# olsonanl/signature_kmers

Hardware: AMD Instinct MI355X
Metric: k-mers/sec (extract+hash+count) at 1/2/4/8 GPUs; achieved HBM GB/s % (higher is better)
Workload: dtype u8

## Files before the change

signature_kmers_amd/__init__.py:

```python
from __future__ import annotations

import ctypes as C
import os
from dataclasses import dataclass

import numpy as np

__all__ = [
    "SkmError", "lib", "K", "UNDEFINED_FUNCTION", "STORED_DTYPE", "CALL_DTYPE",
    "SignatureBuilder", "KeptKmers", "CmphKmerDb", "FunctionCaller", "mph_build",
    "kmer_to_str", "str_to_kmer", "keys_from_strings", "device_count", "MatrixDistance", "SeqIdMap",
    "matrix_tile_rows", "KeptKmerDb", "DeviceKeptKmerDb", "kept_db_plan", "kept_slot",
]

K = 8
UNDEFINED_FUNCTION = 0xFFFF
_HERE = os.path.dirname(os.path.abspath(__file__))
LIB_PATH = os.environ.get("SKM_LIB_PATH") or os.path.join(_HERE, "libskm.so")

STORED_DTYPE = np.dtype([("avg_from_end", "<u2"), ("function_index", "<u2"), ("mean", "<u2"),
                         ("median", "<u2"), ("var", "<u2")])
CALL_DTYPE = np.dtype([("start", "<u4"), ("end", "<u4"), ("count", "<i4"), ("function_index", "<u2"),
                       ("pad", "<u2"), ("protein_length_median", "<u4"),
                       ("protein_length_med_avg_dev", "<f4")])
# ... 159 lines not shown

def debug_chain_bench(n: int, njobs: int, mode: int = 0) -> float:
    ms = C.c_float()
    _check(lib().skm_debug_chain_bench(n, njobs, mode, C.byref(ms)))
    return ms.value


def debug_chain_eval(samples, mode: int):
    x = np.ascontiguousarray(samples, dtype=np.uint32)
    med, var = C.c_double(), C.c_double()
    _check(lib().skm_debug_chain_eval(_ptr(x), len(x), mode, C.byref(med), C.byref(var)))
    return med.value, var.value


def debug_div_check(nm: int, per: int) -> int:
    v = C.c_uint64(0)
    _check(lib().skm_debug_div_check(nm, per, C.byref(v)))
    return v.value


def device_count() -> int:
    n = C.c_int(0)
    _check(lib().skm_device_count(C.byref(n)))
    return n.value


def device_mem_info(device: int = 0) -> tuple:
    fr, tot = C.c_uint64(), C.c_uint64()
    _check(lib().skm_device_mem_info(device, C.byref(fr), C.byref(tot)))
    return fr.value, tot.value


def warm_device(device: int = 0) -> None:
    SignatureBuilder(1, device=device).close()


def kmer_to_str(key: int) -> str:
    return int(key).to_bytes(8, "little").decode("latin-1")


def str_to_kmer(s: str) -> int:
    b = s.encode("latin-1")
    assert len(b) == K
    return int.from_bytes(b, "little")


def keys_from_strings(strs) -> np.ndarray:
    return np.array([str_to_kmer(s) for s in strs], dtype=np.uint64)


@dataclass
class KeptKmers:
    keys: np.ndarray
    data: np.ndarray
    distinct_functions: np.ndarray
    seqs_with_func: np.ndarray
    n_seqs_with_signature: int
    distinct_signatures: int
    n_windows: int

    def stats_lines(self) -> str:
        return (f"Kept {len(self.keys)} kmers\ndistinct_signatures={self.distinct_signatures}\n"
                f"num_seqs_with_a_signature={self.n_seqs_with_signature}\n")

    def final_kmers_lines(self):
        for k, d in zip(self.keys, self.data):
            yield f"{kmer_to_str(k)}\t{int(d['avg_from_end'])}\t{int(d['function_index'])}\t\n"


class _KeptOwner:

    def __init__(self, k):
        self.k = k

    def __del__(self):
        try:
            lib().skm_kept_free(C.byref(self.k))
        except Exception:
            pass


class SignatureBuilder:

    def __init__(self, n_functions: int, max_seqs_per_file: int = 100000, device: int = 0, rank: int = 0,
                 world_size: int = 1):
        self._h = C.c_void_p()
        opts = _BuildOpts(8, max_seqs_per_file, n_functions, 1, rank, world_size)
        self.rank, self.world_size = rank, world_size
        dev = (C.c_int * 1)(device)
        _check(lib().skm_build_create(C.byref(self._h), dev, 1, C.byref(opts)))
        self.n_functions = n_functions
        self.device = device

    def add_batch(self, residues, seq_off, seq_len, seq_func, seq_id=None):
        residues = np.ascontiguousarray(residues, dtype=np.uint8)
        seq_off = np.ascontiguousarray(seq_off, dtype=np.uint64)
        seq_len = np.ascontiguousarray(seq_len, dtype=np.uint32)
        seq_func = np.ascontiguousarray(seq_func, dtype=np.uint16)
        n = len(seq_len)
        assert len(seq_off) == n and len(seq_func) == n
        if n:
            end = seq_off.astype(np.int64) + seq_len.astype(np.int64)
            if end.max() > len(residues):
                raise SkmError("seq_off/seq_len exceed the residue buffer")
        sid = None if seq_id is None else np.ascontiguousarray(seq_id, dtype=np.uint32)
        _check(lib().skm_build_add_batch(self._h, _ptr(residues), _ptr(seq_off), _ptr(seq_len), _ptr(seq_func),
                                         _ptr(sid) if sid is not None else None, n))

    def reserve(self, n_residues: int, n_seqs: int):
        _check(lib().skm_build_reserve(self._h, int(n_residues), int(n_seqs)))

    def set_transport(self, transport: "GlooTransport"):
        self._transport = transport
        _check(lib().skm_build_set_transport(self._h, transport.ptr))

    def set_comm(self, unique_id: bytes):
        buf = (C.c_uint8 * 128).from_buffer_copy(bytes(unique_id))
        _check(lib().skm_build_set_comm(self._h, buf))

    def prepare(self):
        _check(lib().skm_build_prepare(self._h))

    def run(self):
        _check(lib().skm_build_run(self._h))

    def timings(self) -> dict:
        ms = (C.c_float * 15)()
        n = lib().skm_build_last_timings(self._h, ms, 15)
        names = ["extract_count", "scan", "extract_scatter", "bucket_process", "overflow", "chains", "stats", "total",
                 "exchange", "partition", "bucket_kernel", "big_groups", "chain_tail", "giant_start", "giant_end"]
        return {names[i]: float(ms[i]) for i in range(n)}

    def set_kernel_timing(self, enable: bool, only: str | None = None):
        _check(lib().skm_build_set_kernel_timing(self._h, 1 if enable else 0, only.encode() if only else None))

    def kernel_timings(self) -> dict:
        n = lib().skm_build_kernel_timings(self._h, None, 0, None, None, 0)
        if n <= 0:
            return {}
        ms = (C.c_float * n)()
        cnt = (C.c_uint64 * n)()
        buf = C.create_string_buffer(64 * n + 64)
        lib().skm_build_kernel_timings(self._h, buf, len(buf), ms, cnt, n)
        names = buf.value.decode().split("\n")[:n]
        return {names[i]: (float(ms[i]), int(cnt[i])) for i in range(n)}

    def set_option(self, name: str, value: int):
        _check(lib().skm_build_set_option(self._h, name.encode(), int(value)))

    def passes(self) -> int:
        return self.counters()["passes"]

    def counters(self) -> dict:
        v = (C.c_uint64 * 48)()
        n = lib().skm_build_counters(self._h, v, 48)
        names = ["windows", "kept", "overflow_subbuckets", "chain_jobs", "chain_samples", "sequences", "grouped",
                 "overflow_elements", "overflow_kept", "big_groups", "big_kept", "passes", "valid", "giant_chains",
                 "giant_max", "redone", "cap_overflow_scratch", "cap_split", "cap_long_samples", "cap_long_jobs",
                 "demand_overflow_scratch", "demand_split", "demand_long_samples", "demand_long_jobs",
                 "long_samples", "routed", "add_batch_us", "prepare_upload_us", "prepare_plan_us", "prepare_rest_us",
                 "pass_groups", "add_pack_us", "add_dma_wait_us", "finish_us", "finish_wait_us", "finish_copy_us",
                 "finish_chunks", "finish_select_dev_us", "finish_sort_dev_us", "finish_gather_dev_us",
                 "finish_d2h_dev_us", "finish_max_chunk", "finish_wide_index", "kept_cap",
                 "free_after_prepare", "recs_rot", "overflow_light_subbuckets", "overflow_light_elements"]
        return {names[i]: int(v[i]) for i in range(n)}

    def debug_jobs(self, k: int = 64) -> list:
        v = (C.c_uint32 * k)()
        _check(lib().skm_build_debug_jobs(self._h, v, k))
        return [int(x) for x in v]

    def debug_overflow(self, k: int = 4096) -> list:
        v = (C.c_uint32 * k)()
        n = lib().skm_build_debug_overflow(self._h, v, k)
        return [int(x) for x in v[:min(max(n, 0), k)]]

    def debug_stamps(self, enable: bool) -> list:
        v = (C.c_uint64 * 32)()
        _check(lib().skm_build_debug_stamps(self._h, 1 if enable else 0, v, 32))
        return [int(x) for x in v]

    def finish(self) -> KeptKmers:
        k = _Kept()
        _check(lib().skm_build_finish(self._h, C.byref(k)))
        return self._kept(k)

    def finish_slice(self, slice_bits: int, slice_: int) -> KeptKmers:
        k = _Kept()
        _check(lib().skm_build_finish_slice(self._h, int(slice_bits), int(slice_), C.byref(k)))
        return self._kept(k)

    def signature_flags(self) -> np.ndarray:
        n = self.counters()["sequences"]
        out = np.zeros(max(n, 1), np.uint8)
        _check(lib().skm_build_signature_flags(self._h, _ptr(out), n))
        return out[:n]

    def kept_db(self, load_pct: int = 0, slots: int = 0, release_work: bool = False) -> "DeviceKeptKmerDb":
        opts = _KeptDbOpts(int(load_pct), 1 if release_work else 0, int(slots))
        h = C.c_void_p()
        _check(lib().skm_build_kept_db(self._h, C.byref(opts), C.byref(h)))
        return DeviceKeptKmerDb(h, self.device)

    @staticmethod
    def _kept(k) -> KeptKmers:
        owner = _KeptOwner(k)
        n = int(k.n)
        if n:
            kb = (C.c_char * (8 * n)).from_address(C.cast(k.keys, C.c_void_p).value)
            db = (C.c_char * (10 * n)).from_address(C.cast(k.data, C.c_void_p).value)
            kb._owner = db._owner = owner
            keys = np.frombuffer(kb, np.uint64)
            data = np.frombuffer(db, STORED_DTYPE)
        else:
            keys, data = np.zeros(0, np.uint64), np.zeros(0, STORED_DTYPE)
        nf = int(k.n_functions)
        df = np.ctypeslib.as_array(k.distinct_functions, shape=(max(nf, 1),))[:nf].copy()
        sw = np.ctypeslib.as_array(k.seqs_with_func, shape=(max(nf, 1),))[:nf].copy()
        return KeptKmers(keys, data, df, sw, int(k.n_seqs_with_signature), int(k.distinct_signatures),
                         int(k.n_windows))

    def close(self):
        if self._h:
            lib().skm_build_destroy(self._h)
            self._h = C.c_void_p()

    def __del__(self):
        try:
            self.close()
        except Exception:
            pass


class GlooTransport:

    def __init__(self):
        import torch.distributed as dist
        self.dist = dist
        self.rank, self.world = dist.get_rank(), dist.get_world_size()
        self._cbs = (_A2A_T(self._a2a), _RED_T(self._red), _AGV_T(self._agv))
        self.struct = _Transport(None, *self._cbs)
        self.ptr = C.pointer(self.struct)

    @staticmethod
    def _buf(addr, n):
        import torch
        if n == 0:
            return torch.zeros(0, dtype=torch.uint8)
        return torch.frombuffer((C.c_uint8 * n).from_address(addr), dtype=torch.uint8)

    def _a2a(self, ctx, send, scnt, soff, recv, rcnt, roff):
        try:
            W, me = self.world, self.rank
            sc = [int(scnt[i]) for i in range(W)]
            so = [int(soff[i]) for i in range(W)]
            rc = [int(rcnt[i]) for i in range(W)]
            ro = [int(roff[i]) for i in range(W)]
            if sc[me]:
                C.memmove(recv + ro[me], send + so[me], sc[me])
            reqs = []
            for q in range(W):
                if q == me:
                    continue
                if sc[q]:
                    reqs.append(self.dist.isend(self._buf(send + so[q], sc[q]).clone(), q))
                if rc[q]:
                    reqs.append(self.dist.irecv(self._buf(recv + ro[q], rc[q]), q))
            for r in reqs:
                r.wait()
            return 0
        except Exception:
            import traceback
            traceback.print_exc()
            return -1

    def _red(self, ctx, data, count, op):
        try:
            import torch
            n = int(count)
            if op == 0:
                a = np.ctypeslib.as_array(C.cast(data, C.POINTER(C.c_uint32)), shape=(n,))
                t = torch.from_numpy(a.astype(np.int64))
                self.dist.all_reduce(t, op=self.dist.ReduceOp.SUM)
                a[:] = (t.numpy() & 0xFFFFFFFF).astype(np.uint32)
            else:
                a = np.ctypeslib.as_array(C.cast(data, C.POINTER(C.c_uint8)), shape=(n,))
                t = torch.from_numpy(a.astype(np.int32))
                self.dist.all_reduce(t, op=self.dist.ReduceOp.MAX)
                a[:] = t.numpy().astype(np.uint8)
            return 0
        except Exception:
            import traceback
            traceback.print_exc()
            return -1

    def _agv(self, ctx, send, recv, bytes_per_rank):
        try:
            import torch
            W = self.world
            nb = [int(bytes_per_rank[i]) for i in range(W)]
            m = max(1, max(nb))
            mine = torch.zeros(m, dtype=torch.uint8)
            if nb[self.rank]:
                mine[:nb[self.rank]] = self._buf(send, nb[self.rank])
            outs = [torch.zeros(m, dtype=torch.uint8) for _ in range(W)]
            self.dist.all_gather(outs, mine)
            o = 0
            for r in range(W):
                if nb[r]:
                    self._buf(recv + o, nb[r])[:] = outs[r][:nb[r]]
                o += nb[r]
            return 0
        except Exception:
            import traceback
            traceback.print_exc()
            return -1

# ... 456 lines not shown
```

signature_kmers_amd/csrc/skm_build.hip:

```cpp
#include <hip/hip_runtime.h>

#include <algorithm>
#include <type_traits>
#include <chrono>
#include <cmath>
#include <cstdio>
#include <cstdlib>
#include <cstring>
#include <deque>
#include <memory>
#include <numeric>
#include <string>
#include <thread>
#include <vector>

#include "skm_common.h"
#include "skm_keptdb.h"
#include "skm_pool.h"
#include "skm_output.h"
#include "skm_util.h"

#if defined(SKM_WITH_RCCL)
#include <rccl/rccl.h>
#endif
// ... 460 lines not shown
            const int q = __ffsll((long long)m) - 1;
            m &= m - 1;
            const uint32_t pos = base + (uint32_t)q;
            const uint32_t len = pos - run_s;
            if (len > best_c) {
                best_c = len;
                best_f = run_f;
                rb = run_s;
            }
            run_s = pos;
            run_f = (uint32_t)__shfl((int)f, q, 64);
        }
    }
    {
        const uint32_t len = c - run_s;
        if (len > best_c) {
            best_c = len;
            best_f = run_f;
            rb = run_s;
        }
    }
    if ((float)best_c < float(c) * 0.8f) return r;
    r.kept = true;
    r.best_f = best_f;
    r.cbest = best_c;
    r.rb = rb;
    uint32_t vmin = 0xFFFFu, vmax = 0;
    for (uint32_t t = lane; t < c; t += 64) {
        const uint32_t o = (uint32_t)(v.lov(a + t) & 0xFFFFu);
        vmin = min(vmin, o);
        vmax = max(vmax, o);
    }
    vmin = wave_min(vmin);
    vmax = wave_max(vmax);
    const uint32_t k = c / 2;
    while (vmin < vmax) {
        const uint32_t mid = (vmin + vmax) >> 1;
        uint32_t cnt = 0;
        for (uint32_t t = lane; t < c; t += 64) cnt += (uint32_t)(v.lov(a + t) & 0xFFFFu) <= mid;
        cnt = wave_sum(cnt);
        if (cnt >= k + 1)
            vmax = mid;
        else
            vmin = mid + 1;
    }
    r.avg = vmin;
    uint32_t sum = 0;
    for (uint32_t t = lane; t < c; t += 64) {
        const uint32_t s = (uint32_t)(v.lov(a + t) >> 36);
        mark_seq(flags, s);
        if (t >= rb && t < rb + best_c) sum += glen[s];
    }
    sum = wave_sum(sum);
    r.mean = d2u16((double)(uint16_t)sum / (double)best_c);
    r.median = 0;
    r.var = 0;
    return r;
}

__device__ __forceinline__ uint32_t wg_sum(uint32_t x, uint32_t* s_wave) {
    const uint32_t lane = threadIdx.x & 63u, wave = threadIdx.x >> 6, nw = blockDim.x >> 6;
    x = wave_sum(x);
    if (lane == 0) s_wave[wave] = x;
    __syncthreads();
    uint32_t t = 0;
    for (uint32_t w = 0; w < nw; ++w) t += s_wave[w];
    __syncthreads();
    return t;
}

__device__ __forceinline__ uint32_t wg_max(uint32_t x, uint32_t* s_wave) {
    const uint32_t lane = threadIdx.x & 63u, wave = threadIdx.x >> 6, nw = blockDim.x >> 6;
    x = wave_max(x);
    if (lane == 0) s_wave[wave] = x;
    __syncthreads();
    uint32_t t = 0;
    for (uint32_t w = 0; w < nw; ++w) t = max(t, s_wave[w]);
    __syncthreads();
    return t;
}

__device__ __forceinline__ uint32_t wg_min(uint32_t x, uint32_t* s_wave) {
    const uint32_t lane = threadIdx.x & 63u, wave = threadIdx.x >> 6, nw = blockDim.x >> 6;
    x = wave_min(x);
    if (lane == 0) s_wave[wave] = x;
    __syncthreads();
    uint32_t t = 0xFFFFFFFFu;
    for (uint32_t w = 0; w < nw; ++w) t = min(t, s_wave[w]);
    __syncthreads();
    return t;
}

template <class V>
__device__ bool group_block(const V& v, uint64_t a, uint32_t c, const uint32_t* __restrict__ glen,
                            uint32_t* __restrict__ flags, uint32_t* heads, uint32_t hcap, uint32_t* s_wave, GRes& r) {
    const uint32_t tid = threadIdx.x, nt = blockDim.x;
    r.kept = false;
    uint32_t H = 0;
    for (uint32_t t0 = 0; t0 < c; t0 += nt) {
        const uint32_t t = t0 + tid;
        const bool head = t < c && (t == 0 || v.func(a + t) != v.func(a + t - 1));
        uint32_t tot;
        const uint32_t pos = wg_exclusive_scan(head ? 1u : 0u, s_wave, tot);
        if (head && H + pos < hcap) heads[H + pos] = t;
        H += tot;
    }
    if (H > hcap) return false;
    __syncthreads();
    uint32_t lmax = 0;
    for (uint32_t j = tid; j < H; j += nt) lmax = max(lmax, (j + 1 < H ? heads[j + 1] : c) - heads[j]);
    const uint32_t best_c = wg_max(lmax, s_wave);
    uint32_t fmin = 0xFFFFFFFFu;
    for (uint32_t j = tid; j < H; j += nt)
        if ((j + 1 < H ? heads[j + 1] : c) - heads[j] == best_c) fmin = min(fmin, (v.func(a + heads[j]) << 16) | j);
    const uint32_t fj = wg_min(fmin, s_wave);
    if ((float)best_c < float(c) * 0.8f) return true;
    const uint32_t rb = heads[fj & 0xFFFFu];
    r.kept = true;
    r.best_f = fj >> 16;
    r.cbest = best_c;
    r.rb = rb;
    uint32_t k = c / 2, pre = 0;
    for (int b = 15; b >= 0; --b) {
        uint32_t n0 = 0;
        for (uint32_t t = tid; t < c; t += nt) {
            const uint32_t o = (uint32_t)(v.lov(a + t) & 0xFFFFu);
            n0 += (o >> b) == (pre >> b);
        }
        n0 = wg_sum(n0, s_wave);
        if (k >= n0) {
            k -= n0;
            pre |= 1u << b;
        }
    }
    r.avg = pre;
    uint32_t sum = 0;
    for (uint32_t t = tid; t < c; t += nt) {
        const uint32_t s = (uint32_t)(v.lov(a + t) >> 36);
        mark_seq(flags, s);
        if (t >= rb && t < rb + best_c) sum += glen[s];
    }
    sum = wg_sum(sum, s_wave);
    r.mean = d2u16((double)(uint16_t)sum / (double)best_c);
    r.median = 0;
    r.var = 0;
    return true;
}

enum : uint32_t {
    RUN_FLAGS = 0,
    RUN_LONG_CUR = 1,
    RUN_LONG_N = 2,
    RUN_LONG_FLUSHED = 3,
    RUN_SNAP = 28,
    RUN_DEM_TOT = 8,
    RUN_DEM_SPLIT = 9,
    RUN_DEM_LONG = 10,
    RUN_DEM_LJOBS = 11,
    RUN_LONG_WANT = 12,
    RUN_LONG_WANTJ = 13,
    RUN_ACC_LIGHT_SUB = 14,
    RUN_ACC_LIGHT_ELEMS = 15,
    RUN_ACC_NOVF = 16,
    RUN_ACC_JOBS = 17,
    RUN_ACC_LENS = 18,
    RUN_ACC_OVF_ELEMS = 19,
    RUN_ACC_OVF_KEPT = 20,
    RUN_ACC_BIG = 21,
    RUN_ACC_BIG_KEPT = 22,
    RUN_ACC_GROUPED = 23,
    RUN_LAST_NOVF = 24,
    RUN_LAST_JOBS = 25,
    RUN_NLOC = 26,
    RUN_SLOTS = 64
};
constexpr unsigned long long RUN_F_ARENA = 1;
constexpr unsigned long long RUN_F_RERUN = 2;
constexpr unsigned long long RUN_F_CAP = 4;
enum : uint32_t {
    PLAN_NOVF = 0,
    PLAN_NSPLIT = 1,
    PLAN_NHEAVY = 2,
    PLAN_SKIP = 3,
    PLAN_Q_SPLIT = 4,
    PLAN_Q_HEAVY = 5,
    PLAN_Q_REST = 6,
    PLAN_Q_LIGHT = 7,
    PLAN_SLOTS = 8
};

constexpr int JOB_CLASSES = 32;
constexpr int JOB_WG = 256;

__device__ __forceinline__ uint32_t job_class(uint32_t n) { return 31u - (uint32_t)__clz(n | 1u); }

__device__ __forceinline__ void job_chunk(const unsigned long long* nj_p, uint64_t cap, uint64_t& a, uint64_t& e) {
    const uint64_t nj = min((uint64_t)*nj_p, cap);
    const uint64_t chunk = (nj + gridDim.x - 1) / gridDim.x;
    a = min(nj, (uint64_t)blockIdx.x * chunk);
    e = min(nj, a + chunk);
}

__global__ __launch_bounds__(JOB_WG) void k_job_count(const Job* __restrict__ jobs, const unsigned long long* nj_p,
                                                      uint64_t cap, uint32_t* __restrict__ hist) {
    __shared__ uint32_t h[JOB_CLASSES];
    if (threadIdx.x < JOB_CLASSES) h[threadIdx.x] = 0;
    __syncthreads();
    uint64_t a, e;
    job_chunk(nj_p, cap, a, e);
    for (uint64_t j = a + threadIdx.x; j < e; j += blockDim.x) atomicAdd(&h[job_class(jobs[j].n)], 1u);
    __syncthreads();
    if (threadIdx.x < JOB_CLASSES) hist[blockIdx.x * JOB_CLASSES + threadIdx.x] = h[threadIdx.x];
}

constexpr uint32_t LONG_CLASS = 14;

__global__ void k_job_scan(const uint32_t* __restrict__ hist, uint32_t nwg, uint64_t* __restrict__ offs,
                           uint32_t long_class) {
    __shared__ uint64_t tot[JOB_CLASSES];
    const uint32_t c = threadIdx.x;
    if (c < JOB_CLASSES) {
        uint64_t t = 0;
        for (uint32_t w = 0; w < nwg; ++w) t += hist[w * JOB_CLASSES + c];
        tot[c] = t;
    }
    __syncthreads();
    if (c == 0) {
        uint64_t nl = 0;
        for (uint32_t cc = long_class; cc < JOB_CLASSES; ++cc) nl += tot[cc];
        offs[(uint64_t)nwg * JOB_CLASSES] = nl;
    }
    if (c < JOB_CLASSES) {
        uint64_t base = 0;
        for (uint32_t cc = JOB_CLASSES - 1; cc > c; --cc) base += tot[cc];
        for (uint32_t w = 0; w < nwg; ++w) {
            offs[w * JOB_CLASSES + c] = base;
            base += hist[w * JOB_CLASSES + c];
        }
    }
}

__global__ __launch_bounds__(JOB_WG) void k_job_scatter(const Job* __restrict__ jobs, const unsigned long long* nj_p,
                                                        uint64_t cap, const uint64_t* __restrict__ offs,
                                                        Job* __restrict__ sorted) {
    __shared__ unsigned long long cur[JOB_CLASSES];
    if (threadIdx.x < JOB_CLASSES) cur[threadIdx.x] = offs[blockIdx.x * JOB_CLASSES + threadIdx.x];
    __syncthreads();
    uint64_t a, e;
    job_chunk(nj_p, cap, a, e);
    for (uint64_t j = a + threadIdx.x; j < e; j += blockDim.x) {
        const Job jb = jobs[j];
        sorted[atomicAdd(&cur[job_class(jb.n)], 1ull)] = jb;
    }
}

__global__ __launch_bounds__(1024) void k_long_plan(const Job* __restrict__ jobs, const uint64_t* __restrict__ nlong_p,
                                                    uint64_t* __restrict__ off, unsigned long long* __restrict__ run,
                                                    uint64_t arena_cap, uint64_t jobs_cap) {
    __shared__ uint32_t s_wave[17];
    __shared__ unsigned long long s_run;
    const uint64_t nlong = *nlong_p;
    if (threadIdx.x == 0) s_run = 0;
    __syncthreads();
    for (uint64_t b = 0; b < nlong; b += blockDim.x) {
        const uint64_t j = b + threadIdx.x;
        const uint32_t n = j < nlong ? jobs[j].n : 0u;
        uint32_t tot;
        const uint32_t ex = wg_exclusive_scan(n, s_wave, tot);
        const unsigned long long run_ = s_run;
        if (j < nlong) off[j] = run_ + ex;
        __syncthreads();
        if (threadIdx.x == 0) s_run = run_ + tot;
        __syncthreads();
    }
    if (threadIdx.x == 0) {
        const uint64_t total = s_run;
        off[nlong] = total;
        off[nlong + 1] = nlong;
        if (run) {
            uint64_t base = 0, jbase = 0;
            bool ok = true;
            if (nlong) {
                const unsigned long long want = atomicAdd(&run[RUN_LONG_WANT], (unsigned long long)total) + total;
                const unsigned long long wantj = atomicAdd(&run[RUN_LONG_WANTJ], (unsigned long long)nlong) + nlong;
                auto reserve = [&](unsigned long long* c, uint64_t n, uint64_t cap, uint64_t& at) {
                    unsigned long long cur = *(volatile unsigned long long*)c;
                    while (true) {
                        if (cur + n > cap) return false;
                        const unsigned long long seen = atomicCAS(c, cur, cur + n);
                        if (seen == cur) {
                            at = cur;
                            return true;
                        }
                        cur = seen;
                    }
                };
                ok = reserve(&run[RUN_LONG_CUR], total, arena_cap, base);
                ok = ok && reserve(&run[RUN_LONG_N], nlong, jobs_cap, jbase);
                if (!ok) {
                    atomicMax(&run[RUN_DEM_LONG], want);
                    atomicMax(&run[RUN_DEM_LJOBS], wantj);
                    atomicOr(&run[RUN_FLAGS], (unsigned long long)RUN_F_RERUN);
                }
            }
            off[nlong + 2] = base;
            off[nlong + 3] = jbase;
// ... 1766 lines not shown
    SKM_STAMP(6);
    {
        const uint32_t ntask = tstart[6];
        const uint32_t nbig = cstart[7] - cstart[6];
        const uint64_t bbase = *reinterpret_cast<const unsigned long long*>(L.wave + 44);
        const uint32_t wave = tid >> 6, nwaves = nt >> 6, lane = tid & 63u;
        uint64_t* slots = reinterpret_cast<uint64_t*>(L.lens32);
        uint64_t* slots_lo = const_cast<uint64_t*>(src_lo);
        (void)wave;
        (void)nwaves;
        for (;;) {
            uint32_t t = 0;
            if (lane == 0) t = atomicAdd(&ccnt[7], 1u);
            t = (uint32_t)__builtin_amdgcn_readfirstlane((int)t);
            if (t >= nbig + ntask) break;
            if (t < nbig) {
                const uint32_t g = L.big[cstart[6] + t];
                const uint32_t rep = L.glist[g];
                const uint32_t a = L.goff[rep];
                const uint32_t c = g + 1 < G ? L.goff[L.glist[g + 1]] - a : M - a;
                for (uint32_t u = lane; u < c; u += 64) {
                    const uint32_t j = L.order[a + u];
                    const uint64_t hj = L.hi[j], lj = L.lo[j];
                    slots[a + u] = ((hj & 0xFFFFull) << 48) | (lj >> 16);
                    slots_lo[a + u] = elem_len(hj, lj, A.glen);
                }
                const uint64_t q = bbase + t;
                if (lane == 0 && q < A.big_cap) {
                    A.big_desc[2 * q] = key_h43(hprefix, (L.hi[rep] >> 16) & REM_MASK, A.rem_bits, A.pshift) |
                                        ((uint64_t)c << KEY_BITS);
                    A.big_desc[2 * q + 1] = L.lens_sel + 2 * a;
                }
                continue;
            }
            const uint32_t ts = ntask - 1u - (t - nbig);
            uint32_t k = 0;
            while (k < 5 && ts >= tstart[k + 1]) ++k;
            const uint32_t per = 64u >> (k + 1);
            const uint32_t q0 = cstart[k] + (ts - tstart[k]) * per, qe = cstart[k + 1];
            switch (k) {
                case 0: seg_groups<2>(L, q0, qe, G, M, A, hprefix, jobinfo, fmean); break;
                case 1: seg_groups<4>(L, q0, qe, G, M, A, hprefix, jobinfo, fmean); break;
                case 2: seg_groups<8>(L, q0, qe, G, M, A, hprefix, jobinfo, fmean); break;
                case 3: seg_groups<16>(L, q0, qe, G, M, A, hprefix, jobinfo, fmean); break;
                case 4: seg_groups<32>(L, q0, qe, G, M, A, hprefix, jobinfo, fmean); break;
                default: seg_groups<64>(L, q0, qe, G, M, A, hprefix, jobinfo, fmean); break;
            }
        }
    }
    __syncthreads();
    SKM_STAMP(11);
    SKM_STAMP(7);
    constexpr uint32_t EMIT_PER = CAP / BPK_THREADS;
    unsigned long long* s_base = reinterpret_cast<unsigned long long*>(L.wave + 36);
    const uint32_t j0 = tid * EMIT_PER;
    uint32_t cnt = 0;
#pragma unroll
    for (uint32_t u = 0; u < EMIT_PER; ++u) {
        const uint32_t j = j0 + u;
        const uint32_t jb = j < n ? jobinfo[j] : 0u;
        cnt += ((jb & JOB_KEPT) ? 1u : 0u) | ((jb & JOB_COUNT_MASK) ? 0x10000u : 0u);
    }
    uint32_t tot;
    const uint32_t pos = wg_exclusive_scan1(cnt, L.wave, tot);
    unsigned long long rsv = 0;
    if (tid == 0 && (tot & 0xFFFFu)) rsv = atomicAdd(A.kept_ctr, (unsigned long long)(tot & 0xFFFFu));
    if (tid == 64 && (tot >> 16)) rsv = atomicAdd(&A.ctr[3], (unsigned long long)(tot >> 16));
    {
        uint32_t pk = pos & 0xFFFFu, pj = pos >> 16;
#pragma unroll
        for (uint32_t u = 0; u < EMIT_PER; ++u) {
            const uint32_t jb = j0 + u < n ? jobinfo[j0 + u] : 0u;
            if (!(jb & JOB_KEPT)) continue;
            L.slot[pk] = (uint16_t)(j0 + u);
            if (jb & JOB_COUNT_MASK) {
                L.order[pj++] = (uint16_t)(j0 + u);
                L.rank[j0 + u] = (uint16_t)pk;
            }
            ++pk;
        }
    }
    if (tid == 0 || tid == 64) s_base[tid >> 6] = rsv;
    __syncthreads();
    const uint32_t nkept = tot & 0xFFFFu, njob = tot >> 16;
    if (nkept) {
        const uint64_t ob = s_base[0];
#pragma unroll 1
        for (uint32_t t = tid; t < nkept; t += nt) {
            const uint32_t j = L.slot[t];
            const uint32_t jb = jobinfo[j];
            uint64_t lo;
            if (jb & JOB_COUNT_MASK) {
                const uint32_t fm = fmean[j];
                lo = kept_lo(fm & 0xFFFFu, fm >> 16, 0, 0);
            } else {
                lo = L.lo[j];
            }
            write_kept(A, ob + t, L.hi[j], lo);
        }
        const uint64_t jbase = njob ? s_base[1] : 0;
#pragma unroll 1
        for (uint32_t t = tid; t < njob; t += nt) {
            const uint32_t j = L.order[t];
            const uint32_t jb = jobinfo[j];
            Job jbr;
            jbr.lens_off = L.lens_sel + 2 * (jb >> 16);
            jbr.n = jb & JOB_COUNT_MASK;
            jbr.out_idx = (uint32_t)(ob + L.rank[j]);
            A.jobs[jbase + t] = jbr;
        }
    }
    __syncthreads();
    SKM_STAMP(8);
    return nkept;
}

struct SubMem {
    uint64_t hi[CAP];
    uint64_t lo[CAP];
    uint32_t tab[TAB];
    __align__(16) uint16_t slot[CAP];
    __align__(16) uint16_t rank[CAP];
    __align__(16) uint16_t goff[CAP];
    __align__(16) uint16_t glist[CAP];
    __align__(16) uint16_t order[CAP];
    __align__(16) uint16_t big[CAP / 2];
    __align__(16) uint32_t wave[48];
    uint32_t nbig;
    uint64_t tlast;
    uint32_t ccnt[24];
};

__device__ __forceinline__ SubLds sub_lds(SubMem& m) {
    SubLds L;
    L.ccnt = m.ccnt;
    L.tlast = &m.tlast;
    if (threadIdx.x == 0) m.tlast = __builtin_amdgcn_s_memtime();
    L.hi = m.hi;
    L.lo = m.lo;
    L.tab = m.tab;
    L.slot = m.slot;
    L.rank = m.rank;
    L.goff = m.goff;
    L.glist = m.glist;
    L.order = m.order;
    L.big = m.big;
    L.wave = m.wave;
    L.nbig = &m.nbig;
    L.lens32 = nullptr;
    L.lens_sel = 0;
    return L;
}

__global__ __launch_bounds__(BPK_THREADS, BPK_WAVES_EU) void k_bucket_process(BucketArgs A) {
    static_assert(CAP % BPK_THREADS == 0, "emit assigns CAP / BPK_THREADS elements per thread");
    __shared__ SubMem s_mem;
    __shared__ uint32_t s_sub[(1 << MAX_B2) + 1];
    if (A.skip && *A.skip) return;
    SubLds L = sub_lds(s_mem);

    const uint32_t bucket = blockIdx.x;
    if (bucket >= A.nbuckets) return;
    const uint64_t r0 = A.bstart[bucket], r1 = A.bstart[bucket + 1];
    const uint64_t n = r1 - r0;
    if (n == 0) return;
    const uint64_t hprefix = (uint64_t)(A.bucket_base + bucket) << A.rem_bits;
    if (A.prio == 1) __builtin_amdgcn_s_setprio(1);
    if (A.prio == 2) __builtin_amdgcn_s_setprio(2);
    if (A.prio >= 3) __builtin_amdgcn_s_setprio(3);

    const bool direct = n <= (uint64_t)CAP && A.nsrc == 1;
    uint32_t nsub = 1;
    if (!direct) {
        const uint32_t* tab = A.sub_tab + (uint64_t)bucket * SUB_TAB;
        nsub = tab[0];
        for (uint32_t d = threadIdx.x; d <= nsub; d += blockDim.x) s_sub[d] = tab[1 + d];
        __syncthreads();
        SKM_STAMP(9);
    }
    struct Batch {
        uint32_t a, cnt;
    };
    auto next_batch = [&](uint32_t& d) -> Batch {
        if (direct) {
            if (d >= 1) return Batch{0, 0};
            d = 1;
            return Batch{0, (uint32_t)n};
        }
        while (d < nsub) {
            const uint32_t a = s_sub[d];
            if (s_sub[d + 1] - a == 0 || s_sub[d + 1] - a > (uint32_t)CAP) {
                ++d;
                continue;
            }
            uint32_t d2 = d + 1;
            while (d2 < nsub && s_sub[d2 + 1] - a <= (uint32_t)CAP) ++d2;
            d = d2;
            return Batch{a, s_sub[d2] - a};
        }
        return Batch{0, 0};
    };
    const uint64_t* base_hi = direct ? A.recs_hi + r0 : A.tmp_hi + r0;
    const uint64_t* base_lo = direct ? A.recs_lo + r0 : A.tmp_lo + r0;
    const uint64_t sel = direct ? LENS_IN_RECS : LENS_IN_TMP;
    uint32_t d = 0;
    for (Batch cur = next_batch(d); cur.cnt; cur = next_batch(d)) {
        L.lens_sel = (sel << LENS_SEL_SHIFT) | (2 * (r0 + cur.a));
        L.lens32 = reinterpret_cast<uint32_t*>(const_cast<uint64_t*>(base_hi + cur.a));
        process_sub(base_hi + cur.a, base_lo + cur.a, cur.cnt, A, hprefix, L);
        __syncthreads();
        SKM_STAMP(10);
    }
}

struct BigOut {
    uint64_t h43;
    uint64_t lens_off;
    uint32_t n;
    uint16_t avg, func, mean, pad0;
    uint32_t pad1;
};
static_assert(sizeof(BigOut) == 32, "BigOut layout");

struct BigArgs {
    const uint64_t* desc;
    const unsigned long long* ndesc;
    uint32_t cap;
    const uint64_t* recs_hi;
    const uint64_t* tmp_hi;
    const uint64_t* recs_lo;
    const uint64_t* tmp_lo;
    uint32_t* flags;
    BigOut* out;
};

template <int E>
__device__ __forceinline__ uint32_t ballot_count(const bool (&p)[E]) {
    uint32_t n = 0;
#pragma unroll
    for (int e = 0; e < E; ++e) n += (uint32_t)__popcll(__ballot(p[e]));
    return n;
}

template <int E, int D>
__device__ __forceinline__ void bitonic_cross(uint64_t (&ky)[E], bool take_min) {
#pragma unroll
    for (int e = 0; e < E; ++e) {
        const uint64_t o = xshfl64<D>(ky[e]);
        ky[e] = take_min ? (o < ky[e] ? o : ky[e]) : (o > ky[e] ? o : ky[e]);
    }
}

template <int E>
__device__ __forceinline__ void big_group(const BigArgs& B, uint64_t g, uint64_t* mem, const uint64_t* mlen,
                                          uint32_t c, uint64_t h43, uint64_t lens_off) {
    const uint32_t lane = threadIdx.x & 63u;
    uint32_t fo[E];
    uint64_t ky[E];
#pragma unroll
    for (int e = 0; e < E; ++e) {
        const uint32_t t = lane * E + (uint32_t)e;
        fo[e] = 0xFFFFFFFFu;
        ky[e] = ~0ull;
        if (t < c) {
            const uint64_t v = mem[t];
            const uint32_t len = (uint32_t)mlen[t];
            const uint32_t i = (uint32_t)v & ((1u << ELEM_I_BITS) - 1u);
            fo[e] = ((uint32_t)(v >> 48) << 16) | ((len - i) & 0xFFFFu);
            ky[e] = (v << 16) | t;
        }
    }
    uint32_t cand = 0xFFFFFFFFu, cc = 0;
#pragma unroll
    for (int e = 0; e < E; ++e) {
        if (fo[e] != 0xFFFFFFFFu) {
            const uint32_t f = fo[e] >> 16;
            if (cc == 0) {
                cand = f;
                cc = 1;
            } else if (f == cand) {
                ++cc;
            } else {
                --cc;
            }
        }
    }
    bm_combine(cand, cc);
    bool p[E];
#pragma unroll
    for (int e = 0; e < E; ++e) p[e] = (fo[e] >> 16) == cand;
    const uint32_t nb = ballot_count<E>(p);
    BigOut o;
    o.h43 = h43;
    o.lens_off = lens_off;
    o.n = 0;
    o.avg = o.func = o.mean = 0;
    o.pad0 = 0;
    o.pad1 = 0;
    if ((float)nb < float(c) * 0.8f) {
        if (lane == 0) B.out[g] = o;
        return;
    }
    constexpr int MC = E < 8 ? E : 8;
#pragma unroll
    for (int e0 = 0; e0 < E; e0 += MC) {
        uint32_t ms[MC];
#pragma unroll
        for (int u = 0; u < MC; ++u)
            ms[u] = fo[e0 + u] != 0xFFFFFFFFu ? (uint32_t)(ky[e0 + u] >> (16 + ELEM_I_BITS)) : 0xFFFFFFFFu;
        if constexpr (E > 16) {
            Seq8 q;
#pragma unroll
            for (int u = 0; u < 8; ++u) q.s[u] = ms[u];
            mark_seqs8(B.flags, q);
        } else {
            mark_seqs<MC>(B.flags, ms);
        }
    }
    uint32_t sum = 0;
#pragma unroll
    for (int e = 0; e < E; ++e) {
        if (fo[e] != 0xFFFFFFFFu && p[e]) sum += (uint32_t)mlen[ky[e] & 0xFFFFu];
        if (!p[e]) ky[e] = ~0ull;
    }
    sum = wave_sum(sum);
    uint32_t k = c / 2, pre = 0;
#pragma unroll 1
    for (int b = 15; b >= 0; --b) {
#pragma unroll
        for (int e = 0; e < E; ++e) {
            const uint32_t v = fo[e] == 0xFFFFFFFFu ? 0x10000u : (fo[e] & 0xFFFFu);
            p[e] = ((v >> b) ^ (pre >> b)) == 0u;
        }
        const uint32_t n0 = ballot_count<E>(p);
        if (k >= n0) {
            k -= n0;
            pre |= 1u << b;
        }
    }
#pragma unroll 1
    for (uint32_t kk = 2; kk <= 64u * E; kk <<= 1) {
        const bool asc_lane = ((lane * (uint32_t)E) & kk) == 0;
#pragma unroll 1
        for (uint32_t jj = kk >> 1; jj >= (uint32_t)E; jj >>= 1) {
            const uint32_t d = jj / (uint32_t)E;
            const bool take_min = ((lane & d) == 0) == asc_lane;
            switch (d) {
                case 1: bitonic_cross<E, 1>(ky, take_min); break;
                case 2: bitonic_cross<E, 2>(ky, take_min); break;
                case 4: bitonic_cross<E, 4>(ky, take_min); break;
                case 8: bitonic_cross<E, 8>(ky, take_min); break;
                case 16: bitonic_cross<E, 16>(ky, take_min); break;
                default: bitonic_cross<E, 32>(ky, take_min); break;
            }
        }
#pragma unroll
        for (int jj = E / 2; jj > 0; jj >>= 1) {
            if ((uint32_t)jj < kk) {
#pragma unroll
                for (int e = 0; e < E; ++e) {
                    const int l = e ^ jj;
                    if (l > e) {
                        const bool asc = (((lane * (uint32_t)E) + (uint32_t)e) & kk) == 0;
                        const uint64_t x = ky[e], y = ky[l];
                        const bool sw = asc ? (y < x) : (x < y);
                        ky[e] = sw ? y : x;
                        ky[l] = sw ? x : y;
                    }
                }
            }
        }
    }
    uint32_t* lens = reinterpret_cast<uint32_t*>(mem);
#pragma unroll
    for (int e = 0; e < E; ++e) {
        const uint32_t t = lane * E + (uint32_t)e;
        if (t < nb) lens[nb - 1 - t] = (uint32_t)mlen[ky[e] & 0xFFFFu];
    }
    o.n = nb;
    o.avg = (uint16_t)pre;
    o.func = (uint16_t)cand;
    o.mean = d2u16((double)(uint16_t)sum / (double)nb);
    if (lane == 0) B.out[g] = o;
}

constexpr int BIG_WG = 256;

template <bool LARGE>
__global__ __launch_bounds__(BIG_WG, LARGE ? 3 : 4) void k_big_groups(BigArgs B) {
    const uint64_t nd = min((uint64_t)*B.ndesc, (uint64_t)B.cap);
    const uint64_t nw = (uint64_t)gridDim.x * (BIG_WG / 64);
    for (uint64_t g = (uint64_t)blockIdx.x * (BIG_WG / 64) + (threadIdx.x >> 6); g < nd; g += nw) {
        const uint64_t d0 = B.desc[2 * g], d1 = B.desc[2 * g + 1];
        const uint32_t c = (uint32_t)(d0 >> KEY_BITS);
        if (LARGE != (c > 1024u)) continue;
        const uint64_t h43 = d0 & KEY_MASK;
        const uint64_t sel = d1 >> LENS_SEL_SHIFT, off = d1 & LENS_OFF_MASK;
        uint64_t* mem = const_cast<uint64_t*>(sel == LENS_IN_RECS ? B.recs_hi : B.tmp_hi) + off / 2;
        const uint64_t* mlen = (sel == LENS_IN_RECS ? B.recs_lo : B.tmp_lo) + off / 2;
        if constexpr (LARGE) {
            big_group<32>(B, g, mem, mlen, c, h43, d1);
        } else {
            if (c <= 128u) big_group<2>(B, g, mem, mlen, c, h43, d1);
            else if (c <= 256u) big_group<4>(B, g, mem, mlen, c, h43, d1);
            else if (c <= 512u) big_group<8>(B, g, mem, mlen, c, h43, d1);
            else big_group<16>(B, g, mem, mlen, c, h43, d1);
        }
    }
}

__global__ __launch_bounds__(BIG_WG) void k_big_append(const BigOut* __restrict__ out, BigArgs B, BucketArgs A) {
    __shared__ __align__(16) uint32_t s_wave[48];
    __shared__ unsigned long long s_base[2];
    const uint64_t nd = min((uint64_t)*B.ndesc, (uint64_t)B.cap);
    const uint64_t per = (nd + gridDim.x - 1) / gridDim.x;
    const uint64_t g0 = (uint64_t)blockIdx.x * per, g1 = min(nd, g0 + per);
    for (uint64_t r = g0; r < g1; r += BIG_WG) {
        const uint64_t g = r + threadIdx.x;
        const bool kept = g < g1 && out[g].n != 0;
        uint32_t tot;
        const uint32_t pos = wg_exclusive_scan(kept ? 1u : 0u, s_wave, tot);
        if (tot == 0) continue;
        if (threadIdx.x == 0) {
            s_base[0] = atomicAdd(A.kept_ctr, (unsigned long long)tot);
            s_base[1] = atomicAdd(&A.ctr[3], (unsigned long long)tot);
            atomicAdd(&A.ctr[6], (unsigned long long)tot);
        }
        __syncthreads();
        if (kept) {
            const BigOut o = out[g];
            const uint64_t w = s_base[0] + pos;
            write_kept(A, w, kept_hi(o.h43, o.avg), kept_lo(o.func, o.mean, 0, 0));
            Job jb;
            jb.lens_off = o.lens_off;
            jb.n = o.n;
            jb.out_idx = (uint32_t)w;
            A.jobs[s_base[1] + pos] = jb;
        }
        __syncthreads();
    }
}

__global__ __launch_bounds__(1024) void k_part_order(const uint64_t* __restrict__ bstart, uint32_t nb,
                                                     uint32_t* __restrict__ order) {
    __shared__ uint32_t s_wave[48];
    const uint64_t total = bstart[nb] - bstart[0];
    const uint64_t thr = 2 * (total / max(nb, 1u));
    const uint32_t per = (nb + blockDim.x - 1) / blockDim.x;
    const uint32_t b0 = min(nb, threadIdx.x * per), b1 = min(nb, b0 + per);
    uint32_t loc = 0;
    for (uint32_t b = b0; b < b1; ++b) loc += bstart[b + 1] - bstart[b] > thr ? 1u : 0u;
    uint32_t nbig;
    uint32_t pos = wg_exclusive_scan(loc, s_wave, nbig);
    uint32_t sp = b0 - pos;
    for (uint32_t b = b0; b < b1; ++b) {
        if (bstart[b + 1] - bstart[b] > thr)
            order[pos++] = b;
        else
            order[nbig + sp++] = b;
    }
    if (threadIdx.x == 0) order[nb] = nbig;
}

constexpr uint32_t PT_ROUND = 2048, PT_THREADS = BP_THREADS;

__global__ __launch_bounds__(PT_THREADS, 3) void k_partition(BucketArgs A) {
    __shared__ uint32_t s_cur[(1 << MAX_B2) + 1];
    __shared__ uint32_t s_rc[1 << MAX_B2];
    __shared__ uint16_t s_ro[(1 << MAX_B2) + 1];
    __shared__ uint64_t s_sh[PT_ROUND];
    __shared__ uint64_t s_sl[PT_ROUND];
    __shared__ __align__(16) uint32_t s_wave[48];
    if (blockIdx.x >= A.nbuckets) return;
    const uint32_t bucket = A.order ? A.order[blockIdx.x] : blockIdx.x;
    const uint64_t r0 = A.bstart[bucket], r1 = A.bstart[bucket + 1];
    const uint64_t n = r1 - r0;
    uint32_t* tab = A.sub_tab + (uint64_t)bucket * SUB_TAB;
    if (n == 0 || (n <= (uint64_t)CAP && A.nsrc == 1)) {
        if (threadIdx.x == 0) tab[0] = 0;
        return;
    }
    const uint64_t rem_mask = (1ull << A.rem_bits) - 1;
    int b2 = 0;
    const uint64_t target = A.sub_target ? A.sub_target : (uint32_t)SUB_TARGET;
    while (b2 < MAX_B2 && (n >> b2) > target) ++b2;
    const uint32_t nsub = 1u << b2;
    const int shift = A.rem_bits - b2;
    for (uint32_t d = threadIdx.x; d <= nsub; d += blockDim.x) s_cur[d] = 0;
    __syncthreads();
    const uint32_t nseg = A.nsrc;
    auto seg = [&](uint32_t p, uint64_t& base, uint64_t& len) {
        if (nseg == 1) {
            base = r0;
            len = n;
        } else {
            base = A.seg_start[(uint64_t)p * A.nbuckets + bucket];
            len = A.seg_len[(uint64_t)p * A.nbuckets + bucket];
        }
    };
    for (uint32_t p = 0; p < nseg; ++p) {
        uint64_t base, len;
        seg(p, base, len);
        for (uint64_t j0 = 0; j0 < len; j0 += blockDim.x) {
            const uint64_t j = j0 + threadIdx.x;
            const bool v = j < len;
            const uint64_t h = v ? A.recs_hi[base + j] : 0ull;
            agg_count(s_cur, (uint32_t)(((h >> 16) & rem_mask) >> shift), v);
        }
    }
    __syncthreads();
    {
        const uint32_t per = (nsub + blockDim.x - 1) / blockDim.x;
        const uint32_t d0 = threadIdx.x * per;
        uint32_t local = 0;
        for (uint32_t d = d0; d < min(nsub, d0 + per); ++d) local += s_cur[d];
        uint32_t tot;
        uint32_t run = wg_exclusive_scan(local, s_wave, tot);
        for (uint32_t d = d0; d < min(nsub, d0 + per); ++d) {
            const uint32_t t = s_cur[d];
            s_cur[d] = run;
            run += t;
        }
        __syncthreads();
        if (threadIdx.x == 0) s_cur[nsub] = tot;
        __syncthreads();
    }
    if (threadIdx.x == 0) tab[0] = nsub;
    for (uint32_t d = threadIdx.x; d <= nsub; d += blockDim.x) tab[1 + d] = s_cur[d];
    __syncthreads();
    constexpr uint32_t PER = PT_ROUND / PT_THREADS;
    for (uint32_t p = 0; p < nseg; ++p) {
        uint64_t base, len;
        seg(p, base, len);
        uint64_t nh[PER], nl[PER];
#pragma unroll
        for (uint32_t u = 0; u < PER; ++u) {
            const uint64_t j = threadIdx.x + (uint64_t)u * PT_THREADS;
            if (j < len) {
                nh[u] = A.recs_hi[base + j];
                nl[u] = A.recs_lo[base + j];
            }
        }
        for (uint64_t rb = 0; rb < len; rb += PT_ROUND) {
            for (uint32_t d = threadIdx.x; d < nsub; d += blockDim.x) s_rc[d] = 0;
            uint64_t eh[PER], el[PER];
            uint32_t sb[PER], rk[PER];
#pragma unroll
            for (uint32_t u = 0; u < PER; ++u) {
                sb[u] = 0xFFFFFFFFu;
                eh[u] = nh[u];
                el[u] = nl[u];
                const uint64_t j = rb + PT_ROUND + threadIdx.x + (uint64_t)u * PT_THREADS;
                if (j < len) {
                    nh[u] = A.recs_hi[base + j];
                    nl[u] = A.recs_lo[base + j];
                }
            }
            __syncthreads();
#pragma unroll
            for (uint32_t u = 0; u < PER; ++u) {
                const uint64_t j = rb + threadIdx.x + (uint64_t)u * PT_THREADS;
                const bool v = j < len;
                if (v) sb[u] = (uint32_t)(((eh[u] >> 16) & rem_mask) >> shift);
                rk[u] = agg_rank(s_rc, v ? sb[u] : 0u, v);
            }
            __syncthreads();
            {
                const uint32_t per = (nsub + blockDim.x - 1) / blockDim.x;
                const uint32_t d0 = threadIdx.x * per;
                uint32_t local = 0;
                for (uint32_t d = d0; d < min(nsub, d0 + per); ++d) local += s_rc[d];
                uint32_t tot;
                uint32_t run = wg_exclusive_scan(local, s_wave, tot);
                for (uint32_t d = d0; d < min(nsub, d0 + per); ++d) {
                    s_ro[d] = (uint16_t)run;
                    run += s_rc[d];
                }
                if (threadIdx.x == 0) s_ro[nsub] = (uint16_t)tot;
                __syncthreads();
            }
#pragma unroll
            for (uint32_t u = 0; u < PER; ++u)
                if (sb[u] != 0xFFFFFFFFu) {
                    const uint32_t slot = s_ro[sb[u]] + rk[u];
                    s_sh[slot] = eh[u];
                    s_sl[slot] = el[u];
                }
            __syncthreads();
            const uint32_t tot = s_ro[nsub];
            for (uint32_t k = threadIdx.x; k < tot; k += blockDim.x) {
                const uint64_t h = s_sh[k];
                const uint32_t d = (uint32_t)(((h >> 16) & rem_mask) >> shift);
                const uint64_t o = r0 + s_cur[d] + (k - s_ro[d]);
                A.tmp_hi[o] = h;
                A.tmp_lo[o] = s_sl[k];
            }
            __syncthreads();
            for (uint32_t d = threadIdx.x; d < nsub; d += blockDim.x) s_cur[d] += s_rc[d];
            __syncthreads();
        }
    }
    for (uint32_t d = threadIdx.x; d < nsub; d += blockDim.x) {
        const uint32_t beg = d ? s_cur[d - 1] : 0u;
        const uint32_t cnt = s_cur[d] - beg;
        if (cnt > (uint32_t)CAP) {
            const unsigned int en = atomicAdd(reinterpret_cast<unsigned int*>(&A.ctr[1]), 1u);
            if (en < A.ovf_cap) {
                OvfEntry o;
                o.off = r0 + beg;
                o.n = cnt;
                o.bucket = bucket;
                o.scratch = 0;
                o.npad = 0;
                o.src = 1;
                A.ovf[en] = o;
            }
        }
    }
}

struct OvfScratch {
    uint64_t* hi;
    uint64_t* lo;
    uint32_t* heads;
    uint64_t* jobinfo;
    uint32_t* fmean;
};

constexpr uint32_t OVF_INLINE_CAP = 32;
constexpr uint32_t OVF_BLOCK_GROUP = 1024;

__global__ __launch_bounds__(BP_THREADS) void k_overflow(BucketArgs A, OvfScratch S, uint32_t* plan, int lo_slot,
// ... 974 lines not shown
                        mark_seq(A.flags, sv[u]);
                    }
                }
            }
        }
        if (tid == 0) {
            const uint64_t h43 = key_h43((uint64_t)(A.bucket_base + K.bucket) << A.rem_bits, K.rem, A.rem_bits, A.pshift);
            write_kept(A, o, kept_hi(h43, pre), kept_lo(best_f, mean, 0, 0));
            Job jbr;
            jbr.n = cb;
            jbr.out_idx = o;
            if (giant) {
                jbr.lens_off = reinterpret_cast<uint64_t>(H.gsamples + loff);
                H.gjobs[jb] = jbr;
            } else {
                jbr.lens_off = loff;
                A.jobs[jb] = jbr;
            }
        }
        __syncthreads();
    }
}

struct PlanArgs {
    const OvfEntry* in;
    OvfEntry* out;
    const unsigned long long* ctr;
    const unsigned long long* kept;
    const unsigned long long* nloc;
    unsigned long long* run;
    uint32_t* plan;
    uint32_t ovf_cap, split_min, heavy_min;
    uint64_t kept_cap, tot_cap, split_cap;
};

constexpr uint32_t PLAN_BINS = 3 * 32;

__device__ __forceinline__ uint32_t plan_bin(uint32_t n, uint32_t split_min, uint32_t heavy_min) {
    const uint32_t tier = (n >= split_min ? 1u : 0u) + (n >= heavy_min ? 1u : 0u);
    return PLAN_BINS - 1u - (tier * 32u + (31u - (uint32_t)__clz(n | 1u)));
}

__global__ __launch_bounds__(1024) void k_ovf_plan(PlanArgs P) {
    __shared__ uint32_t s_cnt[PLAN_BINS];
    __shared__ unsigned long long s_part[1024];
    __shared__ unsigned long long s_tot, s_elems, s_split;
    __shared__ uint32_t s_nsplit, s_nheavy;
    const uint32_t tid = threadIdx.x, nt = blockDim.x;
    const uint64_t raw = P.ctr[1] & 0xFFFFFFFFull;
    const uint32_t n = (uint32_t)min<uint64_t>(raw, P.ovf_cap);
    for (uint32_t i = tid; i < PLAN_BINS; i += nt) s_cnt[i] = 0;
    if (tid == 0) {
        s_tot = s_elems = s_split = 0;
        s_nsplit = s_nheavy = 0;
    }
    __syncthreads();
    for (uint32_t i = tid; i < n; i += nt) atomicAdd(&s_cnt[plan_bin(P.in[i].n, P.split_min, P.heavy_min)], 1u);
    __syncthreads();
    if (tid == 0) {
        uint32_t r = 0;
        for (uint32_t b = 0; b < PLAN_BINS; ++b) {
            const uint32_t c = s_cnt[b];
            s_cnt[b] = r;
            r += c;
        }
    }
    __syncthreads();
    unsigned long long lt = 0, le = 0, ls = 0;
    uint32_t lns = 0, lnh = 0;
    for (uint32_t i = tid; i < n; i += nt) {
        OvfEntry e = P.in[i];
        const uint32_t pos = atomicAdd(&s_cnt[plan_bin(e.n, P.split_min, P.heavy_min)], 1u);
        uint64_t np = 1;
        while (np < e.n) np <<= 1;
        e.npad = (uint32_t)np;
        P.out[pos] = e;
        lt += np;
        le += e.n;
        if (e.n >= P.split_min) {
            ls += e.n;
            ++lns;
        }
        if (e.n >= P.heavy_min) ++lnh;
    }
    atomicAdd(&s_tot, lt);
    atomicAdd(&s_elems, le);
    atomicAdd(&s_split, ls);
    atomicAdd(&s_nsplit, lns);
    atomicAdd(&s_nheavy, lnh);
    __threadfence_block();
    __syncthreads();
    const uint32_t per = (n + nt - 1) / nt;
    const uint32_t a = min(n, tid * per), e_ = min(n, a + per);
    unsigned long long sum = 0;
    for (uint32_t i = a; i < e_; ++i) sum += P.out[i].npad;
    s_part[tid] = sum;
    __syncthreads();
    if (tid == 0) {
        unsigned long long r = 0;
        for (uint32_t t = 0; t < nt; ++t) {
            const unsigned long long v = s_part[t];
            s_part[t] = r;
            r += v;
        }
    }
    __syncthreads();
    unsigned long long o = s_part[tid];
    for (uint32_t i = a; i < e_; ++i) {
        P.out[i].scratch = o;
        o += P.out[i].npad;
    }
    if (tid == 0) {
        unsigned long long* R = P.run;
        const uint64_t tot = s_tot, split = s_split, nl = *P.nloc;
        atomicMax(&R[RUN_DEM_TOT], (unsigned long long)tot);
        atomicMax(&R[RUN_DEM_SPLIT], (unsigned long long)split);
        if (raw > P.ovf_cap) atomicOr(&R[RUN_FLAGS], RUN_F_CAP);
        const bool over = tot > P.tot_cap || split > P.split_cap;
        if (over) atomicOr(&R[RUN_FLAGS], RUN_F_RERUN);
        if (P.kept[0] + nl > P.kept_cap) atomicOr(&R[RUN_FLAGS], RUN_F_ARENA);
        const bool skip = over || (atomicAdd(&R[RUN_FLAGS], 0ull) & (RUN_F_ARENA | RUN_F_CAP)) != 0;
        P.plan[PLAN_NOVF] = skip ? 0u : n;
        P.plan[PLAN_NSPLIT] = skip ? 0u : s_nsplit;
        P.plan[PLAN_NHEAVY] = skip ? 0u : s_nheavy;
        P.plan[PLAN_SKIP] = skip ? 1u : 0u;
        P.plan[PLAN_Q_SPLIT] = 0;
        P.plan[PLAN_Q_HEAVY] = 0;
        P.plan[PLAN_Q_REST] = 0;
        P.plan[PLAN_Q_LIGHT] = 0;
        R[RUN_ACC_NOVF] += n;
        R[RUN_ACC_OVF_ELEMS] += s_elems;
        R[RUN_ACC_GROUPED] += nl;
        R[RUN_LAST_NOVF] = n;
    }
}

__global__ void k_poison_jobs(Job* __restrict__ jobs, uint64_t n, uint64_t samples, uint32_t idx,
                             skm_stored_kmer_data* __restrict__ out) {
    const uint64_t t = (uint64_t)blockIdx.x * blockDim.x + threadIdx.x;
    for (uint64_t j = t; j < n; j += (uint64_t)gridDim.x * blockDim.x) jobs[j] = Job{samples, 8u, idx};
    if (t == 0) out[idx] = skm_stored_kmer_data{0xC0DE, 0xC0DE, 0xC0DE, 0xC0DE, 0xC0DE};
}

__global__ void k_pass_account(const unsigned long long* __restrict__ ctr, unsigned long long* __restrict__ run,
                               uint64_t jobs_cap, uint64_t jobs2_cap, uint64_t big_cap, uint64_t lens_cap) {
    const unsigned long long j = ctr[3] + ctr[8 + 3];
    run[RUN_ACC_JOBS] += j;
    run[RUN_ACC_LENS] += ctr[8 + 4];
    run[RUN_ACC_OVF_KEPT] += ctr[8];
    run[RUN_ACC_BIG] += ctr[5];
    run[RUN_ACC_BIG_KEPT] += ctr[6];
    run[RUN_ACC_LIGHT_SUB] += ctr[21];
    run[RUN_ACC_LIGHT_ELEMS] += ctr[22];
    run[RUN_LAST_JOBS] = j;
    if (ctr[3] > jobs_cap || ctr[8 + 3] > jobs2_cap || ctr[5] > big_cap || ctr[8 + 4] > lens_cap)
        atomicOr(&run[RUN_FLAGS], RUN_F_CAP);
}

__global__ void k_kept_finalize(uint64_t* __restrict__ keys, const skm_stored_kmer_data* __restrict__ data,
                                const unsigned long long* __restrict__ n_p, uint32_t nf, uint32_t* __restrict__ dfunc) {
    extern __shared__ uint32_t s_h[];
    const uint64_t n = *n_p;
    const bool lds = nf <= 16384;
    if (lds)
        for (uint32_t f = threadIdx.x; f < nf; f += blockDim.x) s_h[f] = 0;
    __syncthreads();
    for (uint64_t i = (uint64_t)blockIdx.x * blockDim.x + threadIdx.x; i < n; i += (uint64_t)gridDim.x * blockDim.x) {
        keys[i] = decode_key(unmix43(keys[i]));
        uint32_t f = data[i].function_index;
        if (f < nf) {
            if (lds)
                atomicAdd(&s_h[f], 1u);
            else
                atomicAdd(&dfunc[f], 1u);
        }
    }
    __syncthreads();
    if (lds)
        for (uint32_t f = threadIdx.x; f < nf; f += blockDim.x)
            if (s_h[f]) atomicAdd(&dfunc[f], s_h[f]);
}

__global__ void k_func_hist_seqs(const SeqMeta* __restrict__ meta, uint32_t nseq, uint32_t nf, uint32_t* __restrict__ swf) {
    extern __shared__ uint32_t s_h[];
    const bool lds = nf <= 16384;
    if (lds)
        for (uint32_t f = threadIdx.x; f < nf; f += blockDim.x) s_h[f] = 0;
    __syncthreads();
    for (uint32_t s = blockIdx.x * blockDim.x + threadIdx.x; s < nseq; s += gridDim.x * blockDim.x) {
        uint32_t f = meta[s].func;
        if (f < nf) {
            if (lds)
                atomicAdd(&s_h[f], 1u);
            else
                atomicAdd(&swf[f], 1u);
        }
    }
    __syncthreads();
    if (lds)
        for (uint32_t f = threadIdx.x; f < nf; f += blockDim.x)
            if (s_h[f]) atomicAdd(&swf[f], s_h[f]);
}

__global__ void k_flags_from_bits(const uint32_t* __restrict__ bits, uint32_t nseq, uint8_t* __restrict__ flags) {
    for (uint32_t w = blockIdx.x * blockDim.x + threadIdx.x; w < (nseq + 31) / 32; w += gridDim.x * blockDim.x) {
        const uint32_t v = bits[w];
        const uint32_t n = min(32u, nseq - 32 * w);
        uint8_t* o = flags + 32 * (uint64_t)w;
        for (uint32_t t = 0; t < n; ++t) o[t] = (uint8_t)((v >> t) & 1u);
    }
}

__global__ void k_count_flags(const uint8_t* __restrict__ flags, uint32_t nseq, unsigned long long* __restrict__ out) {
    uint32_t local = 0;
    for (uint32_t s = blockIdx.x * blockDim.x + threadIdx.x; s < nseq; s += gridDim.x * blockDim.x) local += flags[s] ? 1u : 0u;
#pragma unroll
    for (int d = 32; d > 0; d >>= 1) local += __shfl_down(local, d, 64);
    if ((threadIdx.x & 63) == 0 && local) atomicAdd(out, (unsigned long long)local);
}

__global__ void k_send_counts(const uint64_t* __restrict__ bstart, uint32_t NB, uint32_t NB1, uint32_t W,
                              const unsigned long long* __restrict__ expect, unsigned long long* __restrict__ run,
                              uint32_t* __restrict__ out) {
    const uint32_t t = blockIdx.x * blockDim.x + threadIdx.x;
    if (t < NB) out[t] = (uint32_t)(bstart[t + 1] - bstart[t]);
    if (t < W && bstart[(uint64_t)(t + 1) * NB1] - bstart[(uint64_t)t * NB1] != expect[t])
        atomicOr(&run[RUN_FLAGS], (unsigned long long)RUN_F_CAP);
}

__global__ __launch_bounds__(1024) void k_recv_plan(const uint32_t* __restrict__ cnt, uint32_t W, uint32_t NB1,
                                                    const unsigned long long* __restrict__ expect,
                                                    unsigned long long* __restrict__ run,
                                                    uint64_t* __restrict__ seg_start, uint32_t* __restrict__ seg_len,
                                                    uint64_t* __restrict__ vstart) {
    __shared__ uint32_t s_wave[17];
    __shared__ unsigned long long s_tot[64];
    const uint32_t tid = threadIdx.x, nt = blockDim.x;
    const uint32_t N = W * NB1;
    {
        const uint32_t per = (N + nt - 1) / nt, a = min(N, tid * per), e = min(N, a + per);
        uint32_t loc = 0;
        for (uint32_t i = a; i < e; ++i) loc += cnt[i];
        uint32_t tot;
        uint64_t run_ = wg_exclusive_scan(loc, s_wave, tot);
        for (uint32_t i = a; i < e; ++i) {
            seg_start[i] = run_;
            seg_len[i] = cnt[i];
            run_ += cnt[i];
        }
    }
    if (tid < 64) s_tot[tid] = 0;
    __syncthreads();
    for (uint32_t i = tid; i < N; i += nt) atomicAdd(&s_tot[i / NB1], (unsigned long long)cnt[i]);
    __syncthreads();
    if (tid < W && s_tot[tid] != expect[tid]) atomicOr(&run[RUN_FLAGS], (unsigned long long)RUN_F_CAP);
    {
        const uint32_t per = (NB1 + nt - 1) / nt, a = min(NB1, tid * per), e = min(NB1, a + per);
        uint32_t loc = 0;
        for (uint32_t k = a; k < e; ++k)
            for (uint32_t p = 0; p < W; ++p) loc += cnt[(uint64_t)p * NB1 + k];
        uint32_t tot;
        uint64_t run_ = wg_exclusive_scan(loc, s_wave, tot);
        for (uint32_t k = a; k < e; ++k) {
            vstart[k] = run_;
            for (uint32_t p = 0; p < W; ++p) run_ += cnt[(uint64_t)p * NB1 + k];
        }
        if (tid == 0) vstart[NB1] = tot;
    }
}

__global__ __launch_bounds__(256) void k_slice_select(const uint64_t* __restrict__ keys,
                                                      const skm_stored_kmer_data* __restrict__ data, uint64_t n,
                                                      int bits, uint64_t slice, unsigned long long* __restrict__ cursor,
                                                      uint64_t* __restrict__ out_keys,
                                                      skm_stored_kmer_data* __restrict__ out_data) {
    const uint32_t lane = threadIdx.x & 63u;
    const uint64_t stride = (uint64_t)gridDim.x * blockDim.x;
    for (uint64_t b0 = (uint64_t)blockIdx.x * blockDim.x; b0 < n; b0 += stride) {
        const uint64_t j = b0 + threadIdx.x;
        const uint64_t k = j < n ? keys[j] : 0ull;
        const bool in = j < n && (bits == 0 || (slice_hash(k) >> (64 - bits)) == slice);
        const uint64_t m = __ballot(in);
        if (!m) continue;
        unsigned long long base = 0;
        if (lane == 0) base = atomicAdd(cursor, (unsigned long long)__popcll(m));
        base = __shfl(base, 0, 64);
        if (in && out_keys) {
            const uint64_t o = base + (uint64_t)__popcll(m & ((1ull << lane) - 1ull));
            out_keys[o] = k;
            out_data[o] = data[j];
        }
    }
}

struct Tune {
    int passes = 0;
    int64_t mem_budget_mb = 0;
    int ovf_heavy = 8192;
    int ovf_inline_min = 0x7FFFFFFF;
    int inline_prio = 3;
    int ovf_long_class = 14;
    int main_long_class = 14;
    int ovf_chain_wgs = 0;
    int chain_prio = 0;
    int bucket_prio = 0;
    int chain_lds_kb = 0;
    int host_timing = 0;
    int heavy_min = (int)HEAVY_MIN;
    int split_min = (int)SPLIT_MIN;
    int ovf_light = 1;
    int giant_class = -1;
    int giant_passes = 0;
    int prefetch = 1;
    int heavy_grid = (int)HEAVY_GRID;
    int ovf_grid = 1024;
    int split_grid = 512;
    int chain_grid = 4096;
    int stream_prio = 0;
    int chain_batches = 2;
    int chain_streams = 1;
    int poison_jobs = 0;
    int route_vacate = 0;
    int tail_async = 1;
    int big_grid = 2048;
    int big_grid_large = 512;
    int big_split = 0;
    int part_order = 1;
    int emit_group = 0;
    int route_first = -1;
    int route_first_min = 1 << 17;
    int route_heavy_min = 1 << 14;
    int chain_cus = 0;
    int side_cus = 0;
    int serial_overflow = 0;
    int stage_round = 1;
    int lane_long = 1 << 20;
    int lane_grid = 256;
    int lane_streams = 1;
    int lane_tail = 1 << 16;
    int sub_target = 0;
    int heavy_lsd = 0;
    int handoff_index_limit = 0;
    int handoff_max_chunk = 0;
};

}

using namespace skm;

struct ChainSet {
    DevBuf hist, offs, sorted, long_off;
};

struct skm_build {
    skm_build_opts opts{};
    int device = 0;
    hipStream_t stream = nullptr;
    struct EvSet {
        hipEvent_t ev[13] = {}, o[3] = {}, o3[3] = {};
    };
    std::deque<EvSet> evsets;
    hipEvent_t* ev = nullptr;
    hipEvent_t* ev_o = nullptr;
    hipEvent_t* ev_o3 = nullptr;
    float last_ms[15] = {};
    uint64_t ovf_elems = 0, ovf_kept = 0, ovf_light_sub = 0, ovf_light_elems = 0;

    uint8_t* st_pin[2] = {};
    size_t st_fill[2] = {};
    hipEvent_t st_ev[2] = {};
    bool st_busy[2] = {};
    int st_cur = 0;
    uint64_t rp_total = 0;
    uint64_t rp_dev = 0;
    uint64_t res_cap = 0;
    std::vector<SeqMeta> h_meta;
    std::vector<uint32_t> h_seqid;
    std::unique_ptr<HostPool> pool;
    HandoffStats handoff;
    std::vector<uint32_t> h_keep;
    std::vector<uint64_t> h_cum;
    double add_s = 0, add_pack_s = 0, add_wait_s = 0, prep_upload_s = 0, prep_plan_s = 0, prep_rest_s = 0;
    uint64_t n_windows = 0;
    bool seqid_strict = true;
    bool prepared = false, ran = false;
    bool work_released = false;

    DevBuf d_res, d_meta, d_blk2seq, d_glen;
    uint64_t rp = 0;
    uint32_t nseq = 0;
    int world = 1, rank = 0;
    int owner_bits = 0, b1_bits = 12;
    uint32_t s_base = 0;
    uint32_t n_total = 0;
    std::vector<uint32_t> g_seqid;
    bool g_strict = true;
    DevBuf d_hist, d_offs, d_partial, d_rbbase, d_bstart32, d_bstart, d_owner_start;
    DevBuf d_recs_hi, d_recs_lo, d_tmp_hi, d_tmp_lo;
    DevBuf d_stg_hi, d_stg_lo;
    DevBuf d_part_order;
    DevBuf d_cur0, d_cur1, d_slices;
    DevBuf d_flagbits;
    DevBuf d_keys, d_data, d_ctr, d_flags, d_dfunc, d_swf, d_ovf, d_ovf_hi, d_ovf_lo, d_ovf_heads, d_ovf_job, d_ovf_fm;
    DevBuf d_jobs, d_lens, d_stamps, d_big_desc, d_big_out;
    uint64_t big_cap = 0, n_big = 0, big_kept = 0;
    bool stamps = false;
    uint64_t jobs_cap = 0, lens_cap = 0, n_jobs = 0, n_lens = 0;
    uint32_t n_overflow = 0, n_overflow_last = 0;
    uint32_t nwg = 0;
    uint64_t span = 0;
    uint64_t n_kept = 0;
    uint64_t ovf_cap = 0;

    DevBuf d_rhi, d_rlo;
    DevBuf d_cnt_send, d_cnt_recv;
    DevBuf d_seg_start, d_seg_len, d_vstart;
    std::vector<uint64_t> xs_send, xs_recv;
    DevBuf d_xs;
    uint64_t n_local_max = 0;
    uint64_t n_local = 0;
    uint64_t cap_local = 0;

#if defined(SKM_WITH_RCCL)
    ncclComm_t comm = nullptr;
#endif
    std::vector<skm_build*> group;
    skm_transport tp{};

    hipStream_t stream2 = nullptr, stream3 = nullptr;
    hipStream_t stream_tail = nullptr;
    hipStream_t stream_tail2 = nullptr;
    hipEvent_t ev_tail_bp = nullptr, ev_tail_done = nullptr, ev_tail2 = nullptr;
    bool tail_pending = false;
    uint64_t free_after_prepare = 0;
    hipEvent_t ev_part = nullptr, ev_split = nullptr, ev_light = nullptr;
    DevBuf d_hv_keys, d_hv_rec, d_hv_len, d_hv_s0, d_hv_s1;
    DevBuf d_sub_tab, d_jobs2, d_jobs3;

    unsigned long long* h_pin = nullptr;
    OvfEntry* h_ovf = nullptr;
    size_t h_ovf_cap = 0;
    unsigned long long* pinned_ctr() {
        if (!h_pin) SKM_HIP(hipHostMalloc(reinterpret_cast<void**>(&h_pin), 128 * 8, hipHostMallocDefault));
        return h_pin;
    }
    OvfEntry* pinned_ovf(size_t n) {
        if (n > h_ovf_cap) {
            if (h_ovf) SKM_HIP(hipHostFree(h_ovf));
            h_ovf = nullptr;
            h_ovf_cap = std::max<size_t>(n, 1024);
            SKM_HIP(hipHostMalloc(reinterpret_cast<void**>(&h_ovf), sizeof(OvfEntry) * h_ovf_cap, hipHostMallocDefault));
        }
        return h_ovf;
    }

    uint64_t jobs2_cap = 0;
    ChainSet cs_main, cs_ovf, cs_ovf3;
    uint32_t n_ovf_heavy = 0;

    int pass_bits = 0;
    uint64_t pass_max = 0;
    uint64_t valid_total = 0;
    DevBuf d_ids;
    DevBuf d_bloom;
    std::vector<uint64_t> cnt64;
    bool route = false;
    bool route_first = false;
    uint64_t routed = 0;
    DevBuf d_posg, d_histg, d_npos;
    uint32_t emit_g = 1;
    DevBuf d_selrows, d_seloff;
    uint64_t sel_span = 0;
    uint32_t sel_wg = SEL_WG;
    hipStream_t stx = nullptr;
    hipEvent_t ev_staged = nullptr, ev_emit = nullptr;
    int64_t emit_q = -1;
    uint32_t pf_nwg = 1;
    uint64_t pf_span = 0;
    uint64_t kept_cap = 0;
    hipEvent_t ev_start = nullptr;
    struct Acc {
        uint64_t novf, jobs, lens, ovf_elems, ovf_kept, big, big_kept, grouped;
    } acc{};
    float pass_ms[12] = {};
    skm::Tune tune;
    hipStream_t chain_st = nullptr;
    hipEvent_t chain_ev[3] = {};
    static constexpr int LANE_ST = 4;
    hipStream_t lane_st[LANE_ST] = {};
    hipEvent_t lane_ev[LANE_ST] = {};
    bool lane_used[LANE_ST] = {};
    static constexpr int GSLOTS = 3;
    hipStream_t gst[GSLOTS] = {};
    hipEvent_t gev_ready[GSLOTS] = {}, gev_done[GSLOTS] = {};
    std::deque<DevBuf> gsamples, gjobs, gcount;
    bool gused[GSLOTS] = {};
    bool chain_used[GSLOTS + 1] = {};
    DevBuf d_gstat;
    uint64_t giant_jobs = 0, giant_max = 0;
    DevBuf d_long_arena;
    DevBuf d_long_jobs;
    uint64_t long_jobs_cap = 0;
    DevBuf d_ovf2, d_plan, d_run;
    uint64_t tot_cap = 0, split_cap = 0, long_cap = 0;
    uint64_t run_flags = 0, demand[4] = {}, n_jobs_last = 0, n_redo = 0;
    uint64_t long_samples = 0;
    int kt_mode = 0;
    std::string kt_only;
    std::vector<hipEvent_t> kt_pool;
    size_t kt_used = 0;
    struct KtRec {
        const char* name;
        size_t e0;
    };
    std::vector<KtRec> kt_recs;
    std::vector<std::string> kt_names;
    std::vector<double> kt_ms;
    std::vector<uint64_t> kt_n;
    hipEvent_t ev_tail[2] = {};
    hipEvent_t ev_giant[2] = {};
    bool giant_timed = false;
};

namespace {

int kt_begin(skm_build* b, const char* name, hipStream_t st) {
    if (!b->kt_mode || (!b->kt_only.empty() && b->kt_only != name)) return -1;
    while (b->kt_pool.size() < b->kt_used + 2) {
        hipEvent_t e;
        SKM_HIP(hipEventCreate(&e));
        b->kt_pool.push_back(e);
    }
    const size_t e0 = b->kt_used;
    b->kt_used += 2;
    SKM_HIP(hipEventRecord(b->kt_pool[e0], st));
    b->kt_recs.push_back({name, e0});
    return (int)e0;
}
void kt_end(skm_build* b, int e0, hipStream_t st) {
    if (e0 >= 0) SKM_HIP(hipEventRecord(b->kt_pool[(size_t)e0 + 1], st));
}
#define SKM_LAUNCH(B, K, G, BL, LDS, ST, ...)                   \
    do {                                                        \
        const int _kt = kt_begin((B), #K, (ST));                \
        hipLaunchKernelGGL(K, G, BL, LDS, ST, __VA_ARGS__);     \
        kt_end((B), _kt, (ST));                                 \
    } while (0)
#define SKM_LAUNCH_AS(B, NAME, K, G, BL, LDS, ST, ...)          \
    do {                                                        \
        const int _kt = kt_begin((B), NAME, (ST));              \
        hipLaunchKernelGGL(K, G, BL, LDS, ST, __VA_ARGS__);     \
        kt_end((B), _kt, (ST));                                 \
    } while (0)

void kt_collect(skm_build* b) {
    b->kt_names.clear();
    b->kt_ms.clear();
    b->kt_n.clear();
    for (const auto& r : b->kt_recs) {
// ... 154 lines not shown
}

enum class Red { SumU32, MaxU8 };

void allreduce(const Ranks& bs, const std::vector<void*>& ptr, size_t count, Red op) {
    if (count == 0) return;
    if (has_tp(bs)) {
        skm_build* b = bs[0];
        const size_t es = op == Red::SumU32 ? 4 : 1;
        std::vector<uint8_t> h(count * es);
        SKM_HIP(hipStreamSynchronize(b->stream));
        SKM_HIP(hipMemcpy(h.data(), ptr[0], count * es, hipMemcpyDeviceToHost));
        tp_check(b->tp.allreduce(b->tp.ctx, h.data(), count, op == Red::SumU32 ? 0 : 1), "allreduce");
        SKM_HIP(hipMemcpy(ptr[0], h.data(), count * es, hipMemcpyHostToDevice));
        return;
    }
    if (is_group(bs)) {
        sync_all(bs);
        const size_t es = op == Red::SumU32 ? 4 : 1;
        std::vector<uint8_t> acc(count * es, 0), tmp(count * es);
        for (size_t r = 0; r < bs.size(); ++r) {
            SKM_HIP(hipMemcpy(tmp.data(), ptr[r], count * es, hipMemcpyDeviceToHost));
            if (op == Red::SumU32) {
                auto* a = reinterpret_cast<uint32_t*>(acc.data());
                auto* t = reinterpret_cast<const uint32_t*>(tmp.data());
                for (size_t i = 0; i < count; ++i) a[i] += t[i];
            } else {
                for (size_t i = 0; i < count; ++i) acc[i] = std::max(acc[i], tmp[i]);
            }
        }
        for (size_t r = 0; r < bs.size(); ++r) SKM_HIP(hipMemcpy(ptr[r], acc.data(), count * es, hipMemcpyHostToDevice));
        return;
    }
#if defined(SKM_WITH_RCCL)
    skm_build* b = bs[0];
    if (op == Red::SumU32)
        SKM_NCCL(ncclAllReduce(ptr[0], ptr[0], count, ncclUint32, ncclSum, b->comm, b->stream));
    else
        SKM_NCCL(ncclAllReduce(ptr[0], ptr[0], count, ncclUint8, ncclMax, b->comm, b->stream));
#else
    throw Error(SKM_E_COMM, "libskm was built without RCCL");
#endif
}

std::vector<uint64_t> allgather_u64(const Ranks& bs, const std::vector<uint64_t>& mine) {
    if (has_tp(bs)) {
        skm_build* b = bs[0];
        std::vector<uint64_t> out(b->world), bytes(b->world, 8);
        tp_check(b->tp.allgatherv(b->tp.ctx, &mine[0], out.data(), bytes.data()), "allgatherv");
        return out;
    }
    if (is_group(bs)) return mine;
#if defined(SKM_WITH_RCCL)
    skm_build* b = bs[0];
    DevBuf d;
    d.ensure(8 * (b->world + 1));
    SKM_HIP(hipMemcpyAsync(d.as<uint64_t>() + b->rank, &mine[0], 8, hipMemcpyHostToDevice, b->stream));
    SKM_NCCL(ncclAllGather(d.as<uint64_t>() + b->rank, d.p, 1, ncclUint64, b->comm, b->stream));
    std::vector<uint64_t> out(b->world);
    SKM_HIP(hipMemcpyAsync(out.data(), d.p, 8 * b->world, hipMemcpyDeviceToHost, b->stream));
    SKM_HIP(hipStreamSynchronize(b->stream));
    return out;
#else
    throw Error(SKM_E_COMM, "libskm was built without RCCL");
#endif
}

void allgatherv(const Ranks& bs, const std::vector<const void*>& src, const std::vector<void*>& dst,
                const std::vector<uint64_t>& bytes_per_rank) {
    const size_t W = bytes_per_rank.size();
    std::vector<uint64_t> off(W + 1, 0);
    for (size_t r = 0; r < W; ++r) off[r + 1] = off[r] + bytes_per_rank[r];
    if (has_tp(bs)) {
        skm_build* b = bs[0];
        std::vector<uint8_t> hs(std::max<uint64_t>(bytes_per_rank[b->rank], 1)), hr(std::max<uint64_t>(off[W], 1));
        SKM_HIP(hipStreamSynchronize(b->stream));
        if (bytes_per_rank[b->rank])
            SKM_HIP(hipMemcpy(hs.data(), src[0], bytes_per_rank[b->rank], hipMemcpyDeviceToHost));
        tp_check(b->tp.allgatherv(b->tp.ctx, hs.data(), hr.data(), bytes_per_rank.data()), "allgatherv");
        if (off[W]) SKM_HIP(hipMemcpy(dst[0], hr.data(), off[W], hipMemcpyHostToDevice));
        return;
    }
    if (is_group(bs)) {
        sync_all(bs);
        for (size_t q = 0; q < bs.size(); ++q)
            for (size_t r = 0; r < W; ++r)
                if (bytes_per_rank[r])
                    SKM_HIP(hipMemcpy(static_cast<uint8_t*>(dst[q]) + off[r], src[r], bytes_per_rank[r],
                                      hipMemcpyDeviceToDevice));
        return;
    }
#if defined(SKM_WITH_RCCL)
    skm_build* b = bs[0];
    SKM_NCCL(ncclGroupStart());
    for (int r = 0; r < b->world; ++r)
        if (bytes_per_rank[r])
            SKM_NCCL(ncclBroadcast(r == b->rank ? src[0] : nullptr, static_cast<uint8_t*>(dst[0]) + off[r],
                                   bytes_per_rank[r], ncclUint8, r, b->comm, b->stream));
    SKM_NCCL(ncclGroupEnd());
#else
    throw Error(SKM_E_COMM, "libskm was built without RCCL");
#endif
}

void set_geometry(skm_build* b) {
    b->world = std::max(1, b->opts.world_size);
    b->rank = b->opts.rank;
    int ob = 0;
    while ((1 << ob) < b->world) ++ob;
    b->owner_bits = ob;
    const int total = 12 + (ob >= 2 ? 1 : 0);
    b->b1_bits = total - ob;
}

constexpr size_t STAGE_BYTES = 64ull << 20;

void res_reserve(skm_build* b, uint64_t need) {
    if (need <= b->res_cap && b->d_res.p) return;
    const uint64_t cap = std::max<uint64_t>({need, b->res_cap + b->res_cap / 2, STAGE_BYTES});
    void* np = nullptr;
    SKM_HIP(hipMalloc(&np, cap));
    if (b->rp_dev) SKM_HIP(hipMemcpyAsync(np, b->d_res.p, b->rp_dev, hipMemcpyDeviceToDevice, b->stream));
    SKM_HIP(hipStreamSynchronize(b->stream));
    if (b->d_res.p) SKM_HIP(hipFree(b->d_res.p));
    b->d_res.p = np;
    b->d_res.bytes = cap;
    b->res_cap = cap;
}

void stage_flush(skm_build* b) {
    const int c = b->st_cur;
    if (b->st_fill[c]) {
        res_reserve(b, b->rp_dev + b->st_fill[c] + 64);
        SKM_HIP(hipMemcpyAsync(b->d_res.as<uint8_t>() + b->rp_dev, b->st_pin[c], b->st_fill[c], hipMemcpyHostToDevice,
                               b->stream));
        SKM_HIP(hipEventRecord(b->st_ev[c], b->stream));
        b->st_busy[c] = true;
        b->rp_dev += b->st_fill[c];
        b->st_fill[c] = 0;
    }
    b->st_cur ^= 1;
    const int n = b->st_cur;
    if (b->st_busy[n]) {
        const auto t0 = std::chrono::steady_clock::now();
        SKM_HIP(hipEventSynchronize(b->st_ev[n]));
        b->add_wait_s += std::chrono::duration<double>(std::chrono::steady_clock::now() - t0).count();
        b->st_busy[n] = false;
    }
    b->st_fill[n] = 0;
}

void prepare_local(skm_build* b) {
    SKM_HIP(hipSetDevice(b->device));
    set_geometry(b);
    stage_flush(b);
    const uint64_t rp = b->rp_total;
    b->rp = rp;
    b->nseq = (uint32_t)b->h_meta.size();
    SKM_CHECK(b->h_meta.size() < (1ull << ELEM_S_BITS), SKM_E_ARG, "too many sequences in one build shard");
    res_reserve(b, rp + 64);
    SKM_HIP(hipMemsetAsync(b->d_res.as<uint8_t>() + rp, 0, 64, b->stream));
    b->d_meta.ensure(sizeof(SeqMeta) * (b->nseq + 1));
    const SeqMeta sentinel{rp, 0, 0xFFFF, 0};
    if (b->nseq) SKM_HIP(hipMemcpy(b->d_meta.p, b->h_meta.data(), sizeof(SeqMeta) * b->nseq, hipMemcpyHostToDevice));
    SKM_HIP(hipMemcpy(b->d_meta.as<SeqMeta>() + b->nseq, &sentinel, sizeof(SeqMeta), hipMemcpyHostToDevice));
    const uint64_t nblk = (rp >> 6) + 1;
    b->d_blk2seq.ensure(sizeof(uint32_t) * nblk);
    SKM_HIP(hipMemsetAsync(b->d_blk2seq.p, 0, sizeof(uint32_t) * nblk, b->stream));
    if (b->nseq)
        hipLaunchKernelGGL(k_blk2seq, dim3((b->nseq + 255) / 256), dim3(256), 0, b->stream, b->d_meta.as<SeqMeta>(), b->nseq,
                           b->d_blk2seq.as<uint32_t>(), nblk);
    SKM_HIP(hipGetLastError());
    const uint32_t NB = 1u << (b->owner_bits + b->b1_bits);
    uint64_t step = (uint64_t)EX_THREADS * EX_POS_PER_THREAD;
    uint64_t nwg = std::max<uint64_t>(1, std::min<uint64_t>(EX_MAX_WG, ceil_div(rp ? rp : 1, step)));
    b->span = ceil_div(ceil_div(rp ? rp : 1, nwg), step) * step;
    b->nwg = (uint32_t)ceil_div(rp ? rp : 1, b->span);
    const uint32_t nrb = (uint32_t)ceil_div(b->nwg, SCAN_ROWS);
    b->d_hist.ensure(sizeof(uint32_t) * (uint64_t)b->nwg * NB);
    b->d_offs.ensure(sizeof(uint32_t) * (uint64_t)b->nwg * NB);
    b->d_partial.ensure(sizeof(uint32_t) * (uint64_t)nrb * NB);
    b->d_rbbase.ensure(sizeof(uint32_t) * (uint64_t)nrb * NB);
    b->d_bstart32.ensure(sizeof(uint32_t) * (NB + 1));
    b->d_bstart.ensure(sizeof(uint64_t) * (NB + 1));
    b->d_owner_start.ensure(sizeof(uint64_t) * 80);
    b->d_ctr.ensure(2 * 256);
    b->d_dfunc.ensure(sizeof(uint32_t) * std::max<uint32_t>(b->opts.n_functions, 1));
    b->d_swf.ensure(sizeof(uint32_t) * std::max<uint32_t>(b->opts.n_functions, 1));
}

constexpr uint64_t PASS_BYTES = 104;
inline uint64_t pass_work(uint64_t m, int pb, uint64_t rp, bool giant = false) {
    const uint64_t G = pb ? std::min<uint64_t>(1ull << pb, 4) : 0;
    const uint64_t gcap = std::min<uint64_t>(m / 16 * 5 + (1u << 15), 1ull << 28);
    const uint64_t gw = giant ? (1ull << pb) * (4 * gcap + sizeof(Job) * (gcap >> 10) + 4096) : 0;
    return m * (PASS_BYTES + 8 * G) + (pb ? rp : 0) + gw;
}
inline bool work_fits(uint64_t work, uint64_t budget) { return work <= budget / 8 * 5; }
void size_passes(skm_build* b, int forced_pb = -1) {
    DevBuf d_cnt;
    d_cnt.ensure(8 * 64);
    SKM_HIP(hipMemsetAsync(d_cnt.p, 0, 8 * 64, b->stream));
    if (b->rp)
        hipLaunchKernelGGL(k_pass_ids, dim3(1024), dim3(256), 4u * 64, b->stream, b->d_res.as<uint8_t>(), b->rp, 0, 0,
                           nullptr, d_cnt.as<unsigned long long>(), nullptr, 64u);
    SKM_HIP(hipGetLastError());
    uint64_t cnt[64];
    SKM_HIP(hipMemcpyAsync(cnt, d_cnt.p, sizeof(cnt), hipMemcpyDeviceToHost, b->stream));
    SKM_HIP(hipStreamSynchronize(b->stream));
    b->valid_total = 0;
    for (int i = 0; i < 64; ++i) b->valid_total += cnt[i];
    auto pass_max = [&](int pb) {
        uint64_t m = 0;
        const int per = 64 >> pb;
        for (int p = 0; p < (1 << pb); ++p) {
            uint64_t t = 0;
            for (int i = 0; i < per; ++i) t += cnt[p * per + i];
            m = std::max(m, t);
        }
        return m;
    };
    size_t fr = 0, tot = 0;
    SKM_HIP(hipMemGetInfo(&fr, &tot));
    const uint64_t budget = b->tune.mem_budget_mb > 0 ? (uint64_t)b->tune.mem_budget_mb << 20 : (uint64_t)fr;
    int pb = 0;
    if (forced_pb >= 0) {
        pb = forced_pb;
    } else if (b->tune.passes > 0) {
        while ((1 << pb) < b->tune.passes) ++pb;
    } else {
        while (pb < 6) {
            const uint64_t m = pass_max(pb);
            const bool giant = b->tune.giant_class > 0 || (b->tune.giant_class < 0 && (pb == 0 || b->world > 1));
            if (m < (1ull << 32) - (1ull << 28) && work_fits(pass_work(m, pb, b->rp, giant), budget)) break;
            ++pb;
        }
    }
    SKM_CHECK(pb <= 6, SKM_E_ARG, "key_range_passes must be a power of two <= 64");
    b->pass_bits = pb;
    b->pass_max = pass_max(pb);
    b->route = false;
    b->routed = 0;
    b->cnt64.assign(cnt, cnt + 64);
    SKM_CHECK(b->pass_max < (1ull << 32), SKM_E_ARG, "more than 2^32 occurrences in one pass of one GPU shard");
}

bool tail_async_on(const skm_build* b) { return b->tune.tail_async && b->world == 1 && b->pass_bits; }

void ensure_local(skm_build* b, uint64_t n) {
    if (tail_async_on(b)) {
        const uint64_t cs = std::max<uint64_t>(n + n / 16, 1);
        b->d_stg_hi.ensure(8 * cs);
        b->d_stg_lo.ensure(8 * cs);
    }
    if (n <= b->cap_local && b->cap_local) return;
    const uint64_t c = std::max<uint64_t>(n + n / 16, 1);
    if (b->world > 1) {
        b->d_rhi.ensure(8 * c);
        b->d_rlo.ensure(8 * c);
    }
    b->d_tmp_hi.ensure(8 * c);
    b->d_tmp_lo.ensure(8 * c);
    if (b->pass_bits == 0) {
        b->d_keys.ensure(8 * c);
        b->d_data.ensure(sizeof(skm_stored_kmer_data) * c + 16);
        b->kept_cap = c;
    }
    const uint32_t NB1 = 1u << b->b1_bits;
    b->ovf_cap = c / CAP + NB1 + 16;
    b->jobs_cap = c / 3 + 16;
    b->lens_cap = c + 16;
    b->d_jobs.ensure(sizeof(Job) * b->jobs_cap);
    b->d_lens.ensure(sizeof(uint32_t) * b->lens_cap);
    b->d_ovf.ensure(sizeof(OvfEntry) * b->ovf_cap);
    b->big_cap = c / 65 + 64;
    b->d_big_desc.ensure(16 * b->big_cap);
    b->d_big_out.ensure(sizeof(BigOut) * b->big_cap);
    b->cap_local = c;
}

void size_local(skm_build* b) {
    const uint64_t W = std::max<uint64_t>(b->pass_max, 1);
    b->d_recs_hi.ensure(8 * W);
    b->d_recs_lo.ensure(8 * W);
    if (b->pass_bits > 0) {
        const uint32_t NB = 1u << (b->owner_bits + b->b1_bits);
        const uint32_t P = 1u << b->pass_bits;
        const uint32_t eg = b->tune.emit_group > 0 ? (uint32_t)b->tune.emit_group : 4u;
        b->emit_g = std::max<uint32_t>(1, std::min<uint32_t>(P, eg));
        b->d_posg.ensure(8 * W * b->emit_g);
        b->d_ids.ensure(((b->rp + 15) & ~15ull) + 64);
        SKM_HIP(hipMemsetAsync(b->d_ids.p, 0xFF, ((b->rp + 15) & ~15ull) + 64, b->stream));
        b->d_histg.ensure(sizeof(uint32_t) * (uint64_t)NB * b->emit_g);
        b->d_npos.ensure(8ull * P);
        const uint64_t rmax = (1ull << REL_BITS) - 16;
        b->sel_wg = (uint32_t)std::max<uint64_t>(SEL_WG, ceil_div(std::max<uint64_t>(b->rp, 1), rmax));
        b->d_selrows.ensure(4ull * b->sel_wg * P);
        b->d_seloff.ensure(8ull * P * (b->sel_wg + 1));
        b->sel_span = ceil_div(ceil_div(std::max<uint64_t>(b->rp, 1), b->sel_wg), 16) * 16;
        SKM_CHECK(b->sel_span < (1ull << REL_BITS), SKM_E_STATE, "pass entry row span exceeds REL_BITS");
        const uint64_t stage_wg = b->tune.stage_round == 1 ? 4ull * EX_MAX_WG : EX_MAX_WG;
        uint32_t nwg = (uint32_t)std::max<uint64_t>(1, std::min<uint64_t>(stage_wg, ceil_div(W, (uint64_t)SC_ROUND * 4)));
        b->pf_span = ceil_div(ceil_div(W, nwg), (uint64_t)SC_ROUND) * SC_ROUND;
        b->pf_nwg = (uint32_t)std::max<uint64_t>(1, ceil_div(W, b->pf_span));
        b->d_hist.ensure(sizeof(uint32_t) * (uint64_t)EX_MAX_WG * NB);
        b->d_offs.ensure(sizeof(uint32_t) * (uint64_t)EX_MAX_WG * NB);
        b->d_partial.ensure(sizeof(uint32_t) * (uint64_t)ceil_div(EX_MAX_WG, SCAN_ROWS) * NB);
        b->d_rbbase.ensure(sizeof(uint32_t) * (uint64_t)ceil_div(EX_MAX_WG, SCAN_ROWS) * NB);
    }
}

void size_arena(skm_build* b) {
    if (b->pass_bits == 0) return;
    size_t fr = 0, tot = 0;
    SKM_HIP(hipMemGetInfo(&fr, &tot));
    const uint64_t reserve = b->pass_max * 32 + (1ull << 30);
    const uint64_t held = (uint64_t)b->d_keys.bytes + (uint64_t)b->d_data.bytes;
    const uint64_t avail = fr + held > reserve ? fr + held - reserve : 0;
    uint64_t cap = std::min<uint64_t>(b->valid_total + 16, avail / (8 + sizeof(skm_stored_kmer_data)));
    if (b->tune.mem_budget_mb > 0) {
        const uint64_t budget = (uint64_t)b->tune.mem_budget_mb << 20;
        const bool giant = b->tune.giant_class > 0 || (b->tune.giant_class < 0 && (b->pass_bits == 0 || b->world > 1));
        const uint64_t used = pass_work(b->pass_max, b->pass_bits, b->rp, giant);
        cap = std::min<uint64_t>(cap, budget > used ? (budget - used) / 18 : 0);
    }
    cap = std::max<uint64_t>(cap, b->pass_max + 16);
    b->d_keys.ensure(8 * cap);
    b->d_data.ensure(sizeof(skm_stored_kmer_data) * cap + 16);
    b->kept_cap = cap;
}

void alloc_caps(skm_build* b);
void pass_peer_counts(const Ranks& bs);

bool route_first_on(const skm_build* b) {
    return b->tune.route_first > 0 || (b->tune.route_first < 0 && b->world > 1);
}
uint32_t route_arg(const skm_build* b) {
    return b->route_first ? ROUTE_FIRST : (uint32_t)std::max(0, b->tune.route_vacate);
}

void route_plan(const Ranks& bs) {
    skm_build* b0 = bs[0];
    int pb = b0->pass_bits;
    const int W = b0->world;
    for (auto* b : bs) {
        b->route = false;
        b->route_first = false;
        b->routed = 0;
    }
    auto wish = [&](const skm_build* b) -> uint64_t {
        const bool first = route_first_on(b);
        if (b->tune.route_heavy_min <= 0 || pb < (first ? (W > 1 ? 1 : 0) : (W > 1 ? 1 : 2))) return 0u;
        return first ? 3u : 1u;
    };
    uint64_t want = 3u;
    {
        std::vector<uint64_t> mine(bs.size());
        for (size_t k = 0; k < bs.size(); ++k) mine[k] = wish(bs[k]);
        const std::vector<uint64_t> all = W > 1 ? allgather_u64(bs, mine) : mine;
        for (auto v : all) want &= v;
    }
    if (!(want & 1u)) return;
    const bool first = (want & 2u) != 0;
    const size_t ncms = 2ull << CMS_BITS, nbl = 1ull << BLOOM_BITS;
    std::vector<DevBuf> cms(bs.size()), bl8(bs.size());
    std::vector<void*> pc, pb8;
    for (size_t k = 0; k < bs.size(); ++k) {
        skm_build* b = bs[k];
        cms[k].ensure(4 * ncms);
        bl8[k].ensure(nbl);
        SKM_HIP(hipMemsetAsync(cms[k].p, 0, 4 * ncms, b->stream));
        SKM_HIP(hipMemsetAsync(bl8[k].p, 0, nbl, b->stream));
        if (b->rp)
            hipLaunchKernelGGL(k_route_sketch, dim3(2048), dim3(256), 0, b->stream, b->d_res.as<uint8_t>(), b->rp,
                               cms[k].as<uint32_t>(), 0u, nullptr);
        SKM_HIP(hipGetLastError());
        pc.push_back(cms[k].p);
        pb8.push_back(bl8[k].p);
    }
    if (W > 1) allreduce(bs, pc, ncms, Red::SumU32);
    for (size_t k = 0; k < bs.size(); ++k) {
        skm_build* b = bs[k];
        const uint64_t hmin = first ? (uint64_t)std::max(1, b->tune.route_first_min) : (uint64_t)b->tune.route_heavy_min;
        const uint32_t thresh = std::max<uint32_t>(8, (uint32_t)((hmin >> ROUTE_SAMPLE) * 85 / 100));
        if (b->rp)
            hipLaunchKernelGGL(k_route_sketch, dim3(2048), dim3(256), 0, b->stream, b->d_res.as<uint8_t>(), b->rp,
                               cms[k].as<uint32_t>(), thresh, bl8[k].as<uint8_t>());
        SKM_HIP(hipGetLastError());
    }
    if (W > 1) allreduce(bs, pb8, nbl, Red::MaxU8);
    for (size_t k = 0; k < bs.size(); ++k) {
        skm_build* b = bs[k];
        b->route_first = first;
        b->d_bloom.ensure(nbl / 8);
        hipLaunchKernelGGL(k_bloom_pack, dim3((uint32_t)(nbl / 32 + 255) / 256), dim3(256), 0, b->stream,
                           bl8[k].as<uint8_t>(), b->d_bloom.as<uint32_t>());
        SKM_HIP(hipGetLastError());
    }
    std::vector<uint64_t> ok(bs.size(), 1), heavy(bs.size(), 0);
    std::vector<uint64_t> routed_m(bs.size()), routed_n(bs.size());
    auto count_routed = [&]() {
        for (size_t k = 0; k < bs.size(); ++k) {
            skm_build* b = bs[k];
            const uint32_t P = 1u << pb;
            DevBuf d_cnt;
            d_cnt.ensure(8 * 64);
            SKM_HIP(hipMemsetAsync(d_cnt.p, 0, 8 * 64, b->stream));
            if (b->rp)
                hipLaunchKernelGGL(k_pass_ids, dim3(1024), dim3(256), 4u * 64 + (uint32_t)(nbl / 8), b->stream,
                                   b->d_res.as<uint8_t>(), b->rp, pb, 0, nullptr, d_cnt.as<unsigned long long>(),
                                   b->d_bloom.as<uint32_t>(), 64u, nullptr, 0, route_arg(b));
            SKM_HIP(hipGetLastError());
            uint64_t cnt[64];
            SKM_HIP(hipMemcpyAsync(cnt, d_cnt.p, sizeof(cnt), hipMemcpyDeviceToHost, b->stream));
            SKM_HIP(hipStreamSynchronize(b->stream));
            const int R = b->tune.route_vacate > 0 ? std::min(b->tune.route_vacate, (int)P - 1) : (int)(P >> 1);
            uint64_t natural_late = 0, late = 0, m = 0;
            if (first) {
                natural_late = cnt[0];
            } else {
                for (int p = (int)P - R; p < (int)P; ++p) {
                    for (int i = 0; i < (64 >> pb); ++i) natural_late += b->cnt64[p * (64 >> pb) + i];
                    late += cnt[p];
                }
            }
            for (uint32_t p = 0; p < P; ++p) m = std::max<uint64_t>(m, cnt[p]);
            size_t fr = 0, tot = 0;
            SKM_HIP(hipMemGetInfo(&fr, &tot));
            const uint64_t budget = b->tune.mem_budget_mb > 0 ? (uint64_t)b->tune.mem_budget_mb << 20 : (uint64_t)fr;
            const bool forced = b->tune.passes > 0;
            const bool giant = b->tune.giant_class > 0 || (b->tune.giant_class < 0 && (pb == 0 || b->world > 1));
            ok[k] = m < (1ull << 32) - (1ull << 28) &&
                    (forced || m <= b->pass_max || work_fits(pass_work(m, pb, b->rp, giant), budget));
            routed_m[k] = m;
            routed_n[k] = natural_late - late;
            heavy[k] = first ? cnt[0] : 0;
        }
    };
    auto turn_off = [&]() {
        for (auto* b : bs) b->route_first = false;
    };
    count_routed();
    if (first) {
        const std::vector<uint64_t> all = W > 1 ? allgather_u64(bs, heavy) : heavy;
        uint64_t any = 0;
        for (auto v : all) any |= v;
        if (!any) return turn_off();
        if (pb < 2 && b0->tune.passes <= 0 && pb < 6) {
            ++pb;
            for (auto* b : bs) {
                size_passes(b, pb);
                b->route_first = true;
            }
            count_routed();
        }
        if (pb == 0) return turn_off();
    }
    {
        const std::vector<uint64_t> all = W > 1 ? allgather_u64(bs, ok) : ok;
        for (auto v : all)
            if (!v) return turn_off();
    }
    for (size_t k = 0; k < bs.size(); ++k) {
        bs[k]->pass_max = routed_m[k];
        bs[k]->routed = routed_n[k];
        bs[k]->route = true;
    }
}

void check_not_released(const Ranks& bs) {
    for (auto* b : bs)
        SKM_CHECK(!b->work_released, SKM_E_STATE,
                  "the build's work buffers were released (skm_build_kept_db release_work): the handle can only be "
                  "read out and destroyed");
}

void prepare(const Ranks& bs) {
    check_not_released(bs);
    bool need = false;
    for (auto* b : bs) need |= !b->prepared;
    if (!need) return;
    using clk = std::chrono::steady_clock;
    const auto t0 = clk::now();
    for (auto* b : bs) prepare_local(b);
    for (auto* b : bs) SKM_HIP(hipStreamSynchronize(b->stream));
    const auto t1 = clk::now();
    for (auto* b : bs) size_passes(b);
    {
        std::vector<uint64_t> mine;
        for (auto* b : bs) mine.push_back((uint64_t)b->pass_bits);
        const std::vector<uint64_t> all = bs[0]->world > 1 ? allgather_u64(bs, mine) : mine;
        uint64_t pb = 0;
        for (auto v : all) pb = std::max(pb, v);
        for (auto* b : bs)
            if ((uint64_t)b->pass_bits != pb) size_passes(b, (int)pb);
        route_plan(bs);
        for (auto* b : bs) SKM_HIP(hipStreamSynchronize(b->stream));
    }
    const auto t2 = clk::now();
    for (auto* b : bs) {
        b->prep_upload_s = std::chrono::duration<double>(t1 - t0).count();
        b->prep_plan_s = std::chrono::duration<double>(t2 - t1).count();
    }
    for (auto* b : bs) size_local(b);
    skm_build* b0 = bs[0];
    if (b0->world == 1) {
        b0->s_base = 0;
        b0->n_total = b0->nseq;
        b0->d_glen.ensure(4 * (b0->nseq + 1));
        std::vector<uint32_t> len(b0->nseq);
        for (uint32_t s = 0; s < b0->nseq; ++s) len[s] = b0->h_meta[s].len;
        if (b0->nseq) SKM_HIP(hipMemcpyAsync(b0->d_glen.p, len.data(), 4 * b0->nseq, hipMemcpyHostToDevice, b0->stream));
        ensure_local(b0, b0->pass_max);
    } else {
        std::vector<uint64_t> mine;
        for (auto* b : bs) mine.push_back(b->nseq);
        const std::vector<uint64_t> ns = allgather_u64(bs, mine);
        uint64_t tot = 0;
        for (auto v : ns) tot += v;
        SKM_CHECK(tot < (1ull << ELEM_S_BITS), SKM_E_ARG, "too many sequences in one build");
        std::vector<uint64_t> bytes(ns.size());
        for (size_t r = 0; r < ns.size(); ++r) bytes[r] = 4 * ns[r];
        std::vector<DevBuf> lens_src(bs.size()), ids_src(bs.size()), ids_all(bs.size());
        std::vector<const void*> src_l, src_i;
        std::vector<void*> dst_l, dst_i;
        for (size_t k = 0; k < bs.size(); ++k) {
            skm_build* b = bs[k];
            uint64_t base = 0;
            for (int r = 0; r < b->rank; ++r) base += ns[r];
            b->s_base = (uint32_t)base;
            b->n_total = (uint32_t)tot;
            std::vector<uint32_t> len(b->nseq);
            for (uint32_t s = 0; s < b->nseq; ++s) len[s] = b->h_meta[s].len;
            lens_src[k].ensure(4 * (b->nseq + 1));
            ids_src[k].ensure(4 * (b->nseq + 1));
            ids_all[k].ensure(4 * (tot + 1));
            b->d_glen.ensure(4 * (tot + 1));
            SKM_HIP(hipMemcpy(lens_src[k].p, len.data(), 4 * b->nseq, hipMemcpyHostToDevice));
            SKM_HIP(hipMemcpy(ids_src[k].p, b->h_seqid.data(), 4 * b->nseq, hipMemcpyHostToDevice));
            src_l.push_back(lens_src[k].p);
            src_i.push_back(ids_src[k].p);
            dst_l.push_back(b->d_glen.p);
            dst_i.push_back(ids_all[k].p);
        }
        if (is_group(bs)) {
            allgatherv(bs, src_l, dst_l, bytes);
            allgatherv(bs, src_i, dst_i, bytes);
        } else {
            allgatherv(bs, {src_l[0]}, {dst_l[0]}, bytes);
            allgatherv(bs, {src_i[0]}, {dst_i[0]}, bytes);
        }
        sync_all(bs);
        pass_peer_counts(bs);
        for (size_t k = 0; k < bs.size(); ++k) {
            skm_build* b = bs[k];
            b->g_seqid.resize(tot);
            if (tot) SKM_HIP(hipMemcpy(b->g_seqid.data(), ids_all[k].p, 4 * tot, hipMemcpyDeviceToHost));
            b->g_strict = true;
            for (uint64_t s = 1; s < tot; ++s)
                if (b->g_seqid[s] <= b->g_seqid[s - 1]) b->g_strict = false;
            ensure_local(b, std::max(b->pass_max, b->n_local_max));
        }
    }
    for (auto* b : bs) {
        if (!b->tot_cap) {
            b->tot_cap = b->cap_local / 8 * 5 + (1u << 16);
            b->split_cap = b->tot_cap / 2;
            b->long_cap = b->pass_bits ? b->valid_total / 8 + (1u << 16) : 0;
        }
        alloc_caps(b);
        size_arena(b);
        b->d_flags.ensure(std::max<uint64_t>(b->n_total, 1));
        b->d_flagbits.ensure(4 * ((b->n_total + 31) / 32 + 1));
        {
            size_t fr = 0, tot = 0;
            SKM_HIP(hipMemGetInfo(&fr, &tot));
            b->free_after_prepare = fr;
        }
        SKM_HIP(hipStreamSynchronize(b->stream));
        b->prepared = true;
        b->ran = false;
    }
    for (auto* b : bs) b->prep_rest_s = std::chrono::duration<double>(clk::now() - t2).count();
}

void emit_group(skm_build* b, uint32_t g, hipStream_t st) {
    const uint32_t G = b->emit_g;
    const uint32_t NB = 1u << (b->owner_bits + b->b1_bits);
    const int rem_bits = KEY_BITS - b->pass_bits - b->owner_bits - b->b1_bits;
    const uint64_t cap = std::max<uint64_t>(b->pass_max, 1);
#define SKM_EMIT(GG)                                                                                                    \
    SKM_LAUNCH_AS(b, "k_pass_emit", k_pass_emit<GG>, dim3(b->sel_wg), dim3(EMIT_THREADS), 0, st, b->d_res.as<uint8_t>(), \
                  b->d_ids.as<uint8_t>(), b->rp, g * G, b->sel_span, b->d_seloff.as<uint64_t>(), b->sel_wg, \
                  b->d_posg.as<uint64_t>(), cap)
    if (G == 16)
        SKM_EMIT(16);
    else if (G == 8)
        SKM_EMIT(8);
    else if (G == 4)
        SKM_EMIT(4);
    else if (G == 2)
        SKM_EMIT(2);
    else
        SKM_EMIT(1);
#undef SKM_EMIT
    SKM_HIP(hipMemsetAsync(b->d_histg.p, 0, sizeof(uint32_t) * NB * G, st));
    SKM_LAUNCH(b, k_pass_hist, dim3(256, G), dim3(PH_THREADS), 4u * NB, st, b->d_posg.as<uint64_t>(), cap,
               b->d_npos.as<unsigned long long>() + (uint64_t)g * G, NB, rem_bits, b->d_histg.as<uint32_t>());
    SKM_HIP(hipGetLastError());
    if (st != b->stream) SKM_HIP(hipEventRecord(b->ev_emit, st));
}

inline unsigned long long* pass_ctr(skm_build* b) { return b->d_ctr.as<unsigned long long>() + 32; }

void join_tail(skm_build* b) {
    if (!b->tail_pending) return;
    SKM_HIP(hipStreamWaitEvent(b->stream, b->ev_tail_done, 0));
    b->tail_pending = false;
}

void phase_extract(skm_build* b, uint32_t pass) {
    hipStream_t st = b->stream;
    const int nbits = b->owner_bits + b->b1_bits;
    const uint32_t NB = 1u << nbits;
    const uint32_t nowners = 1u << b->owner_bits;
    SKM_HIP(hipEventRecord(b->ev[0], st));
    const size_t lds_cnt = sizeof(uint32_t) * NB;
    ExtractArgs X;
    X.res = b->d_res.as<uint8_t>();
    X.rp = b->rp;
    X.span = b->span;
    X.owner_bits = b->owner_bits;
    X.b1_bits = b->b1_bits;
    X.pass_bits = b->pass_bits;
    X.pass_id = pass;
    X.pos_cap = b->pass_max;
    X.ids = nullptr;
    X.hist = b->d_hist.as<uint32_t>();
    X.offs = b->d_offs.as<uint32_t>();
    X.owner_start = b->d_owner_start.as<uint64_t>();
    X.blk2seq = b->d_blk2seq.as<uint32_t>();
    X.meta = b->d_meta.as<SeqMeta>();
    X.s_base = b->s_base;
    X.out_hi = b->d_recs_hi.as<uint64_t>();
    X.out_lo = b->d_recs_lo.as<uint64_t>();
    uint32_t nwg = b->nwg, hist_rows = b->nwg;
    if (b->pass_bits) {
        const uint32_t G = b->emit_g, q = pass % G;
        if (q == 0) {
            if (b->emit_q == (int64_t)(pass / G))
                SKM_HIP(hipStreamWaitEvent(st, b->ev_emit, 0));
            else
                emit_group(b, pass / G, st);
            b->emit_q = -1;
        }
        X.hist = b->d_histg.as<uint32_t>() + (uint64_t)q * NB;
        X.span = b->pf_span;
        nwg = b->pf_nwg;
        hist_rows = 1;
        (void)lds_cnt;
    } else {
        SKM_LAUNCH(b, k_extract, dim3(nwg), dim3(EX_THREADS), lds_cnt, st, X);
    }
    SKM_HIP(hipGetLastError());
    SKM_HIP(hipEventRecord(b->ev[1], st));
    const uint32_t nrb = (uint32_t)ceil_div(hist_rows, SCAN_ROWS);
    dim3 gsc((NB + 255) / 256, nrb);
    SKM_LAUNCH(b, k_colsum, gsc, dim3(256), 0, st, X.hist, hist_rows, NB, b->d_partial.as<uint32_t>());
    SKM_LAUNCH(b, k_bstart, dim3(1), dim3(1024), 0, st, b->d_partial.as<uint32_t>(), nrb, NB, b->b1_bits,
                       b->d_rbbase.as<uint32_t>(), b->d_bstart32.as<uint32_t>(), b->d_owner_start.as<uint64_t>(), nowners);
    SKM_LAUNCH(b, k_coloffs, gsc, dim3(256), 0, st, X.hist, b->d_rbbase.as<uint32_t>(), hist_rows,
                       NB, b->d_offs.as<uint32_t>());
    SKM_LAUNCH(b, k_abs_starts, dim3((NB + 1 + 255) / 256), dim3(256), 0, st, b->d_bstart32.as<uint32_t>(),
                       b->d_owner_start.as<uint64_t>(), NB, b->b1_bits, nowners, b->d_bstart.as<uint64_t>());
    SKM_HIP(hipGetLastError());
    SKM_HIP(hipEventRecord(b->ev[2], st));
    const int l0_shift = nbits - SC_L0_BITS;
    b->d_cur0.ensure(8ull * 64 * CUR_STRIDE);
    b->d_cur1.ensure(8ull * NB * CUR_STRIDE);
    b->d_slices.ensure(4 * 80);
    SKM_LAUNCH(b, k_stage_init, dim3((NB + 255) / 256), dim3(256), 0, st, b->d_bstart.as<uint64_t>(), NB, l0_shift,
                       b->d_cur0.as<unsigned long long>(), b->d_cur1.as<unsigned long long>(), b->d_slices.as<uint32_t>());
    const bool sep = tail_async_on(b);
    uint64_t* stg_hi = (sep ? b->d_stg_hi : b->d_tmp_hi).as<uint64_t>();
    uint64_t* stg_lo = (sep ? b->d_stg_lo : b->d_tmp_lo).as<uint64_t>();
    if (!sep) join_tail(b);
    if (b->pass_bits && b->tune.stage_round == 1)
        SKM_LAUNCH_AS(b, "k_extract_stage_pos", (k_extract_stage_pos<SC_ROUND_HALF, 4>), dim3(nwg), dim3(EX_THREADS), 0, st, X,
                   b->d_posg.as<uint64_t>() + (uint64_t)(pass % b->emit_g) * std::max<uint64_t>(b->pass_max, 1),
                   b->d_npos.as<unsigned long long>() + pass,
                   b->d_seloff.as<uint64_t>() + (uint64_t)pass * (b->sel_wg + 1), b->sel_wg, b->sel_span,
                   b->d_cur0.as<unsigned long long>(), stg_hi, stg_lo);
    else if (b->pass_bits)
        SKM_LAUNCH_AS(b, "k_extract_stage_pos", (k_extract_stage_pos<SC_ROUND, 2>), dim3(nwg), dim3(EX_THREADS), 0, st, X,
                   b->d_posg.as<uint64_t>() + (uint64_t)(pass % b->emit_g) * std::max<uint64_t>(b->pass_max, 1),
                   b->d_npos.as<unsigned long long>() + pass,
                   b->d_seloff.as<uint64_t>() + (uint64_t)pass * (b->sel_wg + 1), b->sel_wg, b->sel_span,
                   b->d_cur0.as<unsigned long long>(), stg_hi, stg_lo);
    else
        SKM_LAUNCH(b, k_extract_stage, dim3(nwg), dim3(EX_THREADS), 0, st, X, b->d_cur0.as<unsigned long long>(),
                           stg_hi, stg_lo);
    join_tail(b);
    const uint32_t nsl = (uint32_t)(ceil_div(b->pass_max, SC_SLICE) + (1u << SC_L0_BITS));
    SKM_LAUNCH(b, k_split_stage, dim3(nsl), dim3(EX_THREADS), 0, st, stg_hi,
                       stg_lo, b->d_bstart.as<uint64_t>(), nbits, b->d_slices.as<uint32_t>(),
                       b->d_cur1.as<unsigned long long>(), b->d_recs_hi.as<uint64_t>(), b->d_recs_lo.as<uint64_t>());
    SKM_HIP(hipGetLastError());
    SKM_HIP(hipEventRecord(b->ev[3], st));
}

void exchange(const Ranks& bs, uint32_t pass) {
    const int W = bs[0]->world;
    const uint32_t NB1 = 1u << bs[0]->b1_bits;
    const uint32_t NB = NB1 * (uint32_t)W;
    A2A cx, ex_hi, ex_lo;
    for (auto* b : bs) {
        b->d_cnt_send.ensure(4ull * NB);
        b->d_cnt_recv.ensure(4ull * NB);
        SKM_LAUNCH(b, k_send_counts, dim3((NB + 255) / 256), dim3(256), 0, b->stream, b->d_bstart.as<uint64_t>(), NB, NB1,
                   (uint32_t)W, b->d_xs.as<unsigned long long>() + (uint64_t)pass * W, b->d_run.as<unsigned long long>(),
                   b->d_cnt_send.as<uint32_t>());
        cx.send.push_back(b->d_cnt_send.as<uint8_t>());
        cx.recv.push_back(b->d_cnt_recv.as<uint8_t>());
        std::vector<uint64_t> off(W), c(W, 4ull * NB1);
        for (int q = 0; q < W; ++q) off[q] = 4ull * NB1 * q;
        cx.soff.push_back(off);
        cx.scnt.push_back(c);
        cx.roff.push_back(off);
        cx.rcnt.push_back(c);
        std::vector<uint64_t> so(W), sc(W), ro(W), rcn(W);
        uint64_t s0 = 0, r0 = 0;
        for (int q = 0; q < W; ++q) {
            const uint64_t ns = b->xs_send[(uint64_t)pass * W + q], nr = b->xs_recv[(uint64_t)pass * W + q];
            so[q] = 8 * s0;
            sc[q] = 8 * ns;
            ro[q] = 8 * r0;
            rcn[q] = 8 * nr;
            s0 += ns;
            r0 += nr;
        }
        ex_hi.send.push_back(b->d_recs_hi.as<uint8_t>());
        ex_hi.recv.push_back(b->d_rhi.as<uint8_t>());
        ex_lo.send.push_back(b->d_recs_lo.as<uint8_t>());
        ex_lo.recv.push_back(b->d_rlo.as<uint8_t>());
        for (A2A* e : {&ex_hi, &ex_lo}) {
            e->soff.push_back(so);
            e->scnt.push_back(sc);
            e->roff.push_back(ro);
            e->rcnt.push_back(rcn);
        }
    }
    alltoallv(bs, cx);
    alltoallv(bs, ex_hi);
    alltoallv(bs, ex_lo);
    for (auto* b : bs) {
        b->d_seg_start.ensure(8ull * NB);
        b->d_seg_len.ensure(4ull * NB);
        b->d_vstart.ensure(8ull * (NB1 + 1));
        SKM_LAUNCH(b, k_recv_plan, dim3(1), dim3(1024), 0, b->stream, b->d_cnt_recv.as<uint32_t>(), (uint32_t)W, NB1,
                   b->d_xs.as<unsigned long long>() + (uint64_t)(b->xs_recv.size() / W + pass) * W,
                   b->d_run.as<unsigned long long>(), b->d_seg_start.as<uint64_t>(), b->d_seg_len.as<uint32_t>(),
                   b->d_vstart.as<uint64_t>());
        SKM_HIP(hipGetLastError());
    }
}

void pass_peer_counts(const Ranks& bs) {
    const int W = bs[0]->world;
    const uint32_t P = 1u << bs[0]->pass_bits;
    A2A x;
    std::vector<DevBuf> snd(bs.size()), rcv(bs.size());
    for (size_t k = 0; k < bs.size(); ++k) {
        skm_build* b = bs[k];
        DevBuf cnt;
        cnt.ensure(8ull * P * W);
        SKM_HIP(hipMemsetAsync(cnt.p, 0, 8ull * P * W, b->stream));
        if (b->rp)
            hipLaunchKernelGGL(k_pass_ids, dim3(1024), dim3(256), 4u * P * W + (b->route ? (1u << BLOOM_BITS) / 8 : 0u),
                               b->stream, b->d_res.as<uint8_t>(), b->rp, b->pass_bits, b->owner_bits, nullptr,
                               cnt.as<unsigned long long>(), b->route ? b->d_bloom.as<uint32_t>() : nullptr, P * W,
                               nullptr, 0, route_arg(b));
        SKM_HIP(hipGetLastError());
        std::vector<uint64_t> c(P * W), t(P * W);
        SKM_HIP(hipMemcpyAsync(c.data(), cnt.p, 8ull * P * W, hipMemcpyDeviceToHost, b->stream));
        SKM_HIP(hipStreamSynchronize(b->stream));
        b->xs_send = c;
        for (uint32_t p = 0; p < P; ++p)
            for (int q = 0; q < W; ++q) t[(uint64_t)q * P + p] = c[(uint64_t)p * W + q];
        snd[k].ensure(8ull * P * W);
        rcv[k].ensure(8ull * P * W);
        SKM_HIP(hipMemcpy(snd[k].p, t.data(), 8ull * P * W, hipMemcpyHostToDevice));
        x.send.push_back(snd[k].as<uint8_t>());
        x.recv.push_back(rcv[k].as<uint8_t>());
        std::vector<uint64_t> off(W), n(W, 8ull * P);
        for (int q = 0; q < W; ++q) off[q] = 8ull * P * q;
        x.soff.push_back(off);
        x.scnt.push_back(n);
        x.roff.push_back(off);
        x.rcnt.push_back(n);
    }
    alltoallv(bs, x);
    sync_all(bs);
    for (size_t k = 0; k < bs.size(); ++k) {
        skm_build* b = bs[k];
        std::vector<uint64_t> t(P * W);
        SKM_HIP(hipMemcpy(t.data(), rcv[k].p, 8ull * P * W, hipMemcpyDeviceToHost));
        b->xs_recv.assign((uint64_t)P * W, 0);
        uint64_t most = 0;
        for (uint32_t p = 0; p < P; ++p) {
            uint64_t tot = 0;
            for (int q = 0; q < W; ++q) {
                b->xs_recv[(uint64_t)p * W + q] = t[(uint64_t)q * P + p];
                tot += t[(uint64_t)q * P + p];
            }
            most = std::max(most, tot);
        }
        SKM_CHECK(most < (1ull << 32) - (1ull << 28), SKM_E_ARG, "more than 2^32 occurrences in one pass of one GPU");
        b->n_local_max = most;
        b->d_xs.ensure(16ull * P * W);
        SKM_HIP(hipMemcpy(b->d_xs.p, b->xs_send.data(), 8ull * P * W, hipMemcpyHostToDevice));
        SKM_HIP(hipMemcpy(b->d_xs.as<uint64_t>() + (uint64_t)P * W, b->xs_recv.data(), 8ull * P * W, hipMemcpyHostToDevice));
    }
}

uint64_t giant_cap(const skm_build* b) { return std::min<uint64_t>(std::max<uint64_t>(b->split_cap, 1), 1ull << 28); }

int giant_class(const skm_build* b) {
    return b->tune.giant_class >= 0 ? b->tune.giant_class : (b->pass_bits == 0 || b->world > 1 ? 14 : 0);
}

constexpr uint32_t JOB_NWG = 256;
constexpr uint32_t LONG_GRID = 2048;

void launch_chains(skm_build* b, hipStream_t st, const Job* jobs, const unsigned long long* nj_d, uint64_t cap,
                   ChainSet& cs, const uint32_t* lens, const uint32_t* recs32, const uint32_t* tmp32,
                   const uint32_t* big32, skm_stored_kmer_data* out, uint32_t long_class,
                   hipStream_t st_short = nullptr, hipEvent_t ev_sorted = nullptr, uint32_t max_wgs = 0) {
    const Tune& tn = b->tune;
    SKM_LAUNCH(b, k_job_count, dim3(JOB_NWG), dim3(JOB_WG), 0, st, jobs, nj_d, cap, cs.hist.as<uint32_t>());
    SKM_LAUNCH(b, k_job_scan, dim3(1), dim3(64), 0, st, cs.hist.as<uint32_t>(), JOB_NWG, cs.offs.as<uint64_t>(),
                       long_class);
    SKM_LAUNCH(b, k_job_scatter, dim3(JOB_NWG), dim3(JOB_WG), 0, st, jobs, nj_d, cap, cs.offs.as<uint64_t>(),
                       cs.sorted.as<Job>());
    if (st_short && ev_sorted) SKM_HIP(hipEventRecord(ev_sorted, st));
    const uint64_t* nlong_d = cs.offs.as<uint64_t>() + (uint64_t)JOB_NWG * JOB_CLASSES;
    const auto* nlong_u = reinterpret_cast<const unsigned long long*>(nlong_d);
    if (b->pass_bits == 0) {
        const uint32_t lds = (uint32_t)tn.chain_lds_kb * 1024u;
        static bool attr = false;
        if (lds > 65536 && !attr) {
            SKM_HIP(hipFuncSetAttribute(reinterpret_cast<const void*>(k_chain_long),
                                        hipFuncAttributeMaxDynamicSharedMemorySize, (int)lds));
            attr = true;
        }
        SKM_LAUNCH(b, k_chain_long, dim3(LONG_GRID), dim3(128), lds, st, cs.sorted.as<Job>(), nullptr, nlong_u,
                   lens, recs32, tmp32, big32, out, tn.chain_prio);
    } else {
        SKM_LAUNCH(b, k_long_plan, dim3(1), dim3(1024), 0, st, cs.sorted.as<Job>(), nlong_d,
                           cs.long_off.as<uint64_t>(), b->d_run.as<unsigned long long>(), b->long_cap,
                           b->long_jobs_cap);
        SKM_LAUNCH(b, k_long_stash, dim3(LONG_GRID), dim3(256), 0, st, cs.sorted.as<Job>(), nlong_d,
                           cs.long_off.as<uint64_t>(), lens, recs32, tmp32, big32, b->d_long_arena.as<uint32_t>(),
                           b->d_long_jobs.as<Job>());
    }
    hipStream_t ss = st;
    if (st_short && ev_sorted) {
        SKM_HIP(hipStreamWaitEvent(st_short, ev_sorted, 0));
        ss = st_short;
    }
    SKM_LAUNCH(b, k_chains, dim3(max_wgs ? max_wgs : (uint32_t)std::max(1, tn.chain_grid)), dim3(256), 0, ss,
               cs.sorted.as<Job>(), nlong_u, nj_d, cap, lens, recs32, tmp32, big32, out, 0u);
    SKM_HIP(hipGetLastError());
}

void phase_group(skm_build* b, uint32_t pass) {
    hipStream_t st = b->stream, st2 = b->stream2, st3 = b->stream3;
    const bool multi = b->world > 1;
    const uint32_t NB1 = 1u << b->b1_bits;
    join_tail(b);
    SKM_HIP(hipEventRecord(b->ev[4], st));
    unsigned long long* ctr_d = pass_ctr(b);
    SKM_HIP(hipMemsetAsync(ctr_d, 0, 256, st));
    unsigned long long* run_d = b->d_run.as<unsigned long long>();
    uint32_t* plan_d = b->d_plan.as<uint32_t>();
    OvfEntry* ovf2_d = b->d_ovf2.as<OvfEntry>();
    BucketArgs A;
    A.recs_hi = (multi ? b->d_rhi : b->d_recs_hi).as<uint64_t>();
    A.recs_lo = (multi ? b->d_rlo : b->d_recs_lo).as<uint64_t>();
    A.tmp_hi = b->d_tmp_hi.as<uint64_t>();
    A.tmp_lo = b->d_tmp_lo.as<uint64_t>();
    A.bstart = multi ? b->d_vstart.as<uint64_t>() : b->d_bstart.as<uint64_t>();
    A.seg_start = multi ? b->d_seg_start.as<uint64_t>() : nullptr;
    A.seg_len = multi ? b->d_seg_len.as<uint32_t>() : nullptr;
    A.nsrc = multi ? (uint32_t)b->world : 1u;
    A.sub_tab = b->d_sub_tab.as<uint32_t>();
    A.kept_ctr = b->d_ctr.as<unsigned long long>();
    A.nbuckets = NB1;
    A.bucket_base = (pass << (b->owner_bits + b->b1_bits)) | ((uint32_t)b->rank << b->b1_bits);
    A.rem_bits = KEY_BITS - b->pass_bits - b->owner_bits - b->b1_bits;
    A.pshift = KEY_BITS - b->pass_bits;
    A.glen = b->d_glen.as<uint32_t>();
    A.flags = b->d_flagbits.as<uint32_t>();
    A.ctr = ctr_d;
    A.out_keys = b->d_keys.as<uint64_t>();
    A.out_data = b->d_data.as<skm_stored_kmer_data>();
    A.jobs = b->d_jobs.as<Job>();
    A.lens = b->d_lens.as<uint32_t>();
    A.ovf = b->d_ovf.as<OvfEntry>();
    A.ovf_cap = (uint32_t)b->ovf_cap;
    A.prio = b->tune.bucket_prio;
    A.stamps = nullptr;
    A.big_desc = b->d_big_desc.as<uint64_t>();
    A.big_cap = (uint32_t)std::min<uint64_t>(b->big_cap, 0xFFFFFFFFull);
    A.big_ctr = ctr_d + 5;
    A.skip = nullptr;
    A.sub_target = (uint32_t)std::max(0, b->tune.sub_target);
    if (b->stamps) {
        SKM_HIP(hipMemsetAsync(b->d_stamps.p, 0, 32 * 8, st));
        A.stamps = b->d_stamps.as<unsigned long long>();
    }
    A.order = nullptr;
    if (b->tune.part_order) {
        b->d_part_order.ensure(4ull * (NB1 + 1));
        SKM_LAUNCH(b, k_part_order, dim3(1), dim3(1024), 0, st, A.bstart, NB1, b->d_part_order.as<uint32_t>());
        A.order = b->d_part_order.as<uint32_t>();
    }
    SKM_LAUNCH(b, k_partition, dim3(NB1), dim3(BP_THREADS), 0, st, A);
    SKM_HIP(hipGetLastError());
    SKM_HIP(hipEventRecord(b->ev[10], st));
    if (b->pass_bits && pass % b->emit_g == b->emit_g - 1) SKM_HIP(hipEventRecord(b->ev_staged, st));
    const unsigned long long* nloc_d;
    if (multi) {
        nloc_d = reinterpret_cast<const unsigned long long*>(b->d_vstart.as<uint64_t>() + NB1);
    } else {
        nloc_d = reinterpret_cast<const unsigned long long*>(b->d_bstart.as<uint64_t>() + NB1);
    }
    const uint32_t split_min = (uint32_t)std::max(b->tune.split_min, CAP + 1);
    const uint32_t key_min = (uint32_t)std::max(b->tune.heavy_min, 2);
    PlanArgs P;
    P.in = b->d_ovf.as<OvfEntry>();
    P.out = ovf2_d;
    P.ctr = ctr_d;
    P.kept = b->d_ctr.as<unsigned long long>();
    P.nloc = nloc_d;
    P.run = run_d;
    P.plan = plan_d;
    P.ovf_cap = (uint32_t)b->ovf_cap;
    P.split_min = split_min;
    P.heavy_min = (uint32_t)b->tune.ovf_heavy;
    P.kept_cap = b->kept_cap;
    P.tot_cap = b->tot_cap;
    P.split_cap = b->split_cap;
    SKM_LAUNCH(b, k_ovf_plan, dim3(1), dim3(1024), 0, st, P);
    SKM_HIP(hipGetLastError());
    A.skip = plan_d + PLAN_SKIP;
    BucketArgs A2 = A, A3 = A;
    OvfScratch S;
    S.hi = b->d_ovf_hi.as<uint64_t>();
    S.lo = b->d_ovf_lo.as<uint64_t>();
    S.heads = b->d_ovf_heads.as<uint32_t>();
    S.jobinfo = b->d_ovf_job.as<uint64_t>();
    S.fmean = b->d_ovf_fm.as<uint32_t>();
    A2.ovf = ovf2_d;
    A2.ctr = ctr_d + 8;
    A2.jobs = b->d_jobs2.as<Job>();
    A2.lens = b->d_lens.as<uint32_t>();
    A3.ovf = A2.ovf;
    A3.ctr = A2.ctr;
    A3.jobs = A2.jobs;
    A3.lens = A2.lens;
    const uint32_t inline_min = (uint32_t)b->tune.ovf_inline_min;
    const int prio = b->tune.inline_prio;
    HeavyArgs H;
    H.keys = b->d_hv_keys.as<HeavyKey>();
    H.nkeys = ctr_d + 18;
    H.cursor = ctr_d + 19;
    H.queue = ctr_d + 20;
    H.rec = b->d_hv_rec.as<uint64_t>();
    H.len = b->d_hv_len.as<uint32_t>();
    H.s0 = b->d_hv_s0.as<uint32_t>();
    H.s1 = b->d_hv_s1.as<uint32_t>();
    H.fast = b->opts.n_functions <= HV_FT && !b->tune.heavy_lsd ? 1u : 0u;
    H.n_total = std::max<uint32_t>(b->n_total, 1);
    const int gs = (int)(pass % skm_build::GSLOTS);
    const uint32_t NP = 1u << b->pass_bits;
    const bool late = b->tune.giant_passes <= 0 || pass + (uint32_t)b->tune.giant_passes >= NP;
    const int gcls = giant_class(b);
    H.giant_min = gcls > 0 && late && pass < b->gsamples.size() ? 1u << gcls : 0u;
    H.gsamples = nullptr;
    H.gjobs = nullptr;
    H.gcount = nullptr;
    H.gcap = 0;
    H.gstat = nullptr;
    if (H.giant_min) {
        H.gsamples = b->gsamples[pass].as<uint32_t>();
        H.gjobs = b->gjobs[pass].as<Job>();
        H.gcount = b->gcount[pass].as<unsigned long long>();
        H.gcap = giant_cap(b);
        H.gstat = b->d_gstat.as<unsigned long long>();
    }
    const bool light = b->tune.ovf_light != 0;
    auto launch_overflow = [&]() {
    SKM_HIP(hipEventRecord(b->ev_part, st));
    SKM_HIP(hipStreamWaitEvent(st2, b->ev_part, 0));
    SKM_HIP(hipStreamWaitEvent(st3, b->ev_part, 0));
    SKM_HIP(hipEventRecord(b->ev_o[0], st2));
    SKM_HIP(hipEventRecord(b->ev_o3[0], st3));
    if (H.giant_min) SKM_HIP(hipMemsetAsync(b->gcount[pass].p, 0, 16, st2));
    SKM_LAUNCH(b, k_ovf_split, dim3((uint32_t)std::max(1, b->tune.split_grid)), dim3(BP_THREADS), 0, st2, A2, H, key_min, plan_d);
    SKM_HIP(hipEventRecord(b->ev_split, st2));
    SKM_HIP(hipStreamWaitEvent(st3, b->ev_split, 0));
    if (light) {
        SKM_LAUNCH(b, k_ovf_light, dim3(LIGHT_GRID), dim3(BPK_THREADS), 0, st3, A3, plan_d,
                   ctr_d + 21);
        SKM_HIP(hipEventRecord(b->ev_light, st3));
    }
    SKM_LAUNCH(b, k_heavy, dim3((uint32_t)std::max(1, b->tune.heavy_grid)), dim3(HEAVY_WG), 0, st2, A2, H);
    SKM_HIP(hipGetLastError());
    if (H.giant_min) {
        SKM_HIP(hipEventRecord(b->gev_ready[gs], st2));
        SKM_HIP(hipStreamWaitEvent(b->gst[gs], b->gev_ready[gs], 0));
        SKM_LAUNCH(b, k_giant_order, dim3(1), dim3(1024), 0, b->gst[gs], H.gjobs, H.gcount);
        if (!b->giant_timed) SKM_HIP(hipEventRecord(b->ev_giant[0], b->gst[gs]));
        SKM_LAUNCH(b, k_chain_dyn, dim3(1024), dim3(128), 0, b->gst[gs], H.gjobs, H.gcount, A.out_data,
                           b->tune.chain_prio);
        SKM_HIP(hipGetLastError());
        if (!b->giant_timed) SKM_HIP(hipEventRecord(b->ev_giant[1], b->gst[gs]));
        b->giant_timed = true;
        SKM_HIP(hipEventRecord(b->gev_done[gs], b->gst[gs]));
        b->gused[gs] = true;
    }
    if (light) SKM_HIP(hipStreamWaitEvent(st2, b->ev_light, 0));
    SKM_LAUNCH(b, k_overflow, dim3((uint32_t)std::max(1, b->tune.ovf_grid)), dim3(BP_THREADS), 0, st2, A2, S, plan_d, -1, (int)PLAN_NHEAVY,
                       (int)PLAN_Q_HEAVY, inline_min, prio);
    SKM_HIP(hipEventRecord(b->ev_o[1], st2));
    SKM_LAUNCH(b, k_overflow, dim3((uint32_t)std::max(1, b->tune.ovf_grid)), dim3(BP_THREADS), 0, st3, A3, S, plan_d, (int)PLAN_NHEAVY,
                       (int)PLAN_NOVF, (int)PLAN_Q_REST, inline_min, prio);
    SKM_HIP(hipGetLastError());
    };
    if (!b->tune.serial_overflow) launch_overflow();
    BigArgs BA;
    BA.desc = A.big_desc;
    BA.ndesc = ctr_d + 5;
    BA.cap = A.big_cap;
    BA.recs_hi = A.recs_hi;
    BA.tmp_hi = A.tmp_hi;
    BA.recs_lo = A.recs_lo;
    BA.tmp_lo = A.tmp_lo;
    BA.flags = A.flags;
    BA.out = b->d_big_out.as<BigOut>();
    SKM_HIP(hipEventRecord(b->ev[11], st));
    SKM_LAUNCH(b, k_bucket_process, dim3(NB1), dim3(BPK_THREADS), 0, st, A);
    SKM_HIP(hipGetLastError());
    SKM_HIP(hipEventRecord(b->ev[5], st));
    if (b->tune.serial_overflow) launch_overflow();
    if (b->pass_bits && pass + 1 < NP && (pass + 1) % b->emit_g == 0 && b->tune.prefetch) {
        SKM_HIP(hipStreamWaitEvent(b->stx, b->ev_staged, 0));
        emit_group(b, (pass + 1) / b->emit_g, b->stx);
        b->emit_q = (pass + 1) / b->emit_g;
    }
    const bool tail_async = tail_async_on(b);
    hipStream_t tt = tail_async ? b->stream_tail : st;
    if (tail_async) {
        SKM_HIP(hipEventRecord(b->ev_tail_bp, st));
        SKM_HIP(hipStreamWaitEvent(tt, b->ev_tail_bp, 0));
    }
    SKM_HIP(hipEventRecord(b->ev_o3[0], st3));
    SKM_HIP(hipStreamWaitEvent(st2, b->ev_o3[0], 0));
    launch_chains(b, st2, A2.jobs, ctr_d + 8 + 3, b->jobs2_cap, b->cs_ovf, A2.lens, reinterpret_cast<const uint32_t*>(A.recs_hi),
                  reinterpret_cast<const uint32_t*>(A.tmp_hi), nullptr, A.out_data, (uint32_t)b->tune.ovf_long_class, st3, b->ev_o3[2], (uint32_t)b->tune.ovf_chain_wgs);
    SKM_HIP(hipEventRecord(b->ev_o[2], st2));
    SKM_HIP(hipEventRecord(b->ev_o3[1], st3));
    if (light) SKM_HIP(hipStreamWaitEvent(tt, b->ev_light, 0));
    if (tail_async && b->tune.big_split) {
        SKM_HIP(hipStreamWaitEvent(b->stream_tail2, b->ev_tail_bp, 0));
        if (light) SKM_HIP(hipStreamWaitEvent(b->stream_tail2, b->ev_light, 0));
        SKM_LAUNCH(b, k_big_groups<true>, dim3((uint32_t)std::max(1, b->tune.big_grid_large)), dim3(BIG_WG), 0,
                   b->stream_tail2, BA);
        SKM_HIP(hipEventRecord(b->ev_tail2, b->stream_tail2));
        SKM_LAUNCH(b, k_big_groups<false>, dim3((uint32_t)std::max(1, b->tune.big_grid)), dim3(BIG_WG), 0, tt, BA);
        SKM_HIP(hipStreamWaitEvent(tt, b->ev_tail2, 0));
    } else {
        SKM_LAUNCH(b, k_big_groups<false>, dim3((uint32_t)std::max(1, b->tune.big_grid)), dim3(BIG_WG), 0, tt, BA);
        SKM_LAUNCH(b, k_big_groups<true>, dim3((uint32_t)std::max(1, b->tune.big_grid_large)), dim3(BIG_WG), 0, tt, BA);
    }
    SKM_LAUNCH(b, k_big_append, dim3(256), dim3(BIG_WG), 0, tt, BA.out, BA, A);
    SKM_HIP(hipGetLastError());
    SKM_HIP(hipEventRecord(b->ev[12], tt));
    launch_chains(b, tt, A.jobs, ctr_d + 3, b->jobs_cap, b->cs_main, A.lens, reinterpret_cast<const uint32_t*>(A.recs_hi),
                  reinterpret_cast<const uint32_t*>(A.tmp_hi), nullptr, A.out_data, (uint32_t)b->tune.main_long_class);
    SKM_HIP(hipStreamWaitEvent(tt, b->ev_o[2], 0));
    SKM_HIP(hipStreamWaitEvent(tt, b->ev_o3[1], 0));
    SKM_HIP(hipEventRecord(b->ev[6], tt));
    SKM_LAUNCH(b, k_pass_account, dim3(1), dim3(1), 0, tt, ctr_d, run_d, b->jobs_cap, b->jobs2_cap, b->big_cap,
                       b->lens_cap);
    SKM_HIP(hipGetLastError());
    SKM_HIP(hipEventRecord(b->ev[7], tt));
    if (tail_async) {
        SKM_HIP(hipEventRecord(b->ev_tail_done, tt));
        b->tail_pending = true;
    }
}

void alloc_caps(skm_build* b) {
    const uint64_t T = std::max<uint64_t>(b->tot_cap, 1), Sp = std::max<uint64_t>(b->split_cap, 1);
    b->d_ovf_hi.ensure(8 * T);
    b->d_ovf_lo.ensure(8 * T);
    b->d_ovf_heads.ensure(4 * T);
    b->d_ovf_job.ensure(8 * T);
    b->d_ovf_fm.ensure(4 * T);
    b->jobs2_cap = T / 3 + 16;
    b->d_jobs2.ensure(sizeof(Job) * b->jobs2_cap);
    const uint32_t key_min = (uint32_t)std::max(b->tune.heavy_min, 2);
    b->d_hv_keys.ensure(sizeof(HeavyKey) * (Sp / key_min + 16));
    b->d_hv_rec.ensure(8 * Sp);
    b->d_hv_len.ensure(4 * Sp);
    b->d_hv_s0.ensure(4 * Sp);
    b->d_hv_s1.ensure(4 * Sp);
    b->d_ovf2.ensure(sizeof(OvfEntry) * std::max<uint64_t>(b->ovf_cap, 1));
    b->d_plan.ensure(4 * PLAN_SLOTS);
    b->d_run.ensure(8 * RUN_SLOTS);
    b->d_sub_tab.ensure(4ull * (1u << b->b1_bits) * SUB_TAB);
    b->d_stamps.ensure(32 * 8);
    const int cls = std::max(1, std::min(b->tune.main_long_class, b->tune.ovf_long_class));
    struct {
        ChainSet* cs;
        uint64_t cap, elems;
    } sets[2] = {{&b->cs_main, b->jobs_cap, b->cap_local}, {&b->cs_ovf, b->jobs2_cap, T}};
    for (auto& c : sets) {
        c.cs->hist.ensure(4ull * JOB_NWG * JOB_CLASSES);
        c.cs->offs.ensure(8ull * JOB_NWG * JOB_CLASSES + 16);
        c.cs->sorted.ensure(sizeof(Job) * c.cap);
        c.cs->long_off.ensure(8ull * (std::min(c.cap, (c.elems >> cls) + 16) + 8));
    }
    if (b->pass_bits) {
        b->long_jobs_cap = std::max<uint64_t>(b->long_jobs_cap, b->world * (b->valid_total >> cls) + 4096);
        b->d_long_jobs.ensure(sizeof(Job) * b->long_jobs_cap);
        b->d_long_arena.ensure(4 * std::max<uint64_t>(b->long_cap, 1));
    }
    const uint32_t NP = 1u << b->pass_bits;
    if (giant_class(b) > 0) {
        while (b->gsamples.size() < NP) {
            b->gsamples.emplace_back();
            b->gjobs.emplace_back();
            b->gcount.emplace_back();
        }
        for (uint32_t p = 0; p < NP; ++p) {
            b->gsamples[p].ensure(4 * giant_cap(b));
            b->gjobs[p].ensure(sizeof(Job) * (giant_cap(b) / (1u << giant_class(b)) + 16));
            b->gcount[p].ensure(16);
        }
    }
}

void begin_run(skm_build* b) {
    hipStream_t st = b->stream;
    alloc_caps(b);
    b->emit_q = -1;
    b->giant_timed = false;
    b->tail_pending = false;
    SKM_HIP(hipEventRecord(b->ev_start, st));
    SKM_HIP(hipMemsetAsync(b->d_ctr.p, 0, 2 * 256, st));
    SKM_HIP(hipMemsetAsync(b->d_run.p, 0, 8 * RUN_SLOTS, st));
    SKM_HIP(hipMemsetAsync(b->d_flags.p, 0, b->n_total ? b->n_total : 1, st));
    SKM_HIP(hipMemsetAsync(b->d_flagbits.p, 0, 4 * ((b->n_total + 31) / 32 + 1), st));
    b->d_gstat.ensure(16);
    SKM_HIP(hipMemsetAsync(b->d_gstat.p, 0, 16, st));
    if (b->tune.poison_jobs && b->pass_bits && b->long_jobs_cap)
        hipLaunchKernelGGL(k_poison_jobs, dim3(256), dim3(256), 0, st, b->d_long_jobs.as<Job>(), b->long_jobs_cap,
                           reinterpret_cast<uint64_t>(b->d_long_arena.p), (uint32_t)b->kept_cap,
                           b->d_data.as<skm_stored_kmer_data>());
    if (b->pass_bits) {
        const uint32_t P = 1u << b->pass_bits;
        SKM_LAUNCH(b, k_pass_ids, dim3(b->sel_wg), dim3(256), 4u * P + (b->route ? (1u << BLOOM_BITS) / 8 : 0u), st,
                   b->d_res.as<uint8_t>(), b->rp, b->pass_bits, 0, b->d_ids.as<uint8_t>(), nullptr,
                   b->route ? b->d_bloom.as<uint32_t>() : nullptr, P, b->d_selrows.as<uint32_t>(), b->sel_span,
                   route_arg(b));
        SKM_LAUNCH(b, k_sel_scan, dim3(P), dim3(1024), 0, st, b->d_selrows.as<uint32_t>(), b->sel_wg, P,
                   b->d_seloff.as<uint64_t>(), b->d_npos.as<unsigned long long>(), b->pass_max,
                   b->d_run.as<unsigned long long>());
    }
    SKM_HIP(hipGetLastError());
    b->acc = skm_build::Acc{};
    b->kt_used = 0;
    b->kt_recs.clear();
    std::memset(b->pass_ms, 0, sizeof(b->pass_ms));
    for (bool& g : b->gused) g = false;
    for (bool& g : b->chain_used) g = false;
    b->n_kept = 0;
}

void use_evset(skm_build* b, uint32_t pass) {
    while (b->evsets.size() <= pass) {
        b->evsets.emplace_back();
        skm_build::EvSet& e = b->evsets.back();
        for (auto& x : e.ev) SKM_HIP(hipEventCreate(&x));
        for (auto& x : e.o) SKM_HIP(hipEventCreate(&x));
        for (auto& x : e.o3) SKM_HIP(hipEventCreate(&x));
    }
    b->ev = b->evsets[pass].ev;
    b->ev_o = b->evsets[pass].o;
    b->ev_o3 = b->evsets[pass].o3;
}

void pass_times(skm_build* b, uint32_t npass) {
    const int idx[9] = {0, 1, 2, 3, 5, 8, 9, 10, 11};
    const int from[9] = {0, 1, 2, 4, 12, 3, 4, 11, 5}, to[9] = {1, 2, 3, 12, 6, 4, 10, 5, 12};
    for (uint32_t p = 0; p < npass && p < b->evsets.size(); ++p) {
        const skm_build::EvSet& e = b->evsets[p];
        for (int i = 0; i < 9; ++i) {
            float t = 0.f;
            SKM_HIP(hipEventElapsedTime(&t, e.ev[from[i]], e.ev[to[i]]));
            b->pass_ms[idx[i]] += t;
        }
        float t2 = 0.f, t3 = 0.f;
        SKM_HIP(hipEventElapsedTime(&t2, e.o[0], e.o[2]));
        SKM_HIP(hipEventElapsedTime(&t3, e.o[0], e.o3[1]));
        b->pass_ms[4] += std::max(t2, t3);
    }
}

hipStream_t chain_stream(skm_build* b, int slot) {
    const int k = slot % std::max(1, std::min(b->tune.chain_streams, 1 + skm_build::GSLOTS));
    return k == 0 ? b->chain_st : b->gst[k - 1];
}

void flush_long_chains(skm_build* b, int slot) {
    join_tail(b);
    unsigned long long* run_d = b->d_run.as<unsigned long long>();
    unsigned long long* rng = run_d + RUN_SNAP + 2 * slot;
    SKM_LAUNCH(b, k_long_snap, dim3(1), dim3(1), 0, b->stream, run_d, rng, b->long_jobs_cap);
    SKM_HIP(hipEventRecord(b->chain_ev[0], b->stream));
    hipStream_t cs = chain_stream(b, slot);
    SKM_HIP(hipStreamWaitEvent(cs, b->chain_ev[0], 0));
    b->chain_used[slot % std::max(1, std::min(b->tune.chain_streams, 1 + skm_build::GSLOTS))] = true;
    const bool few = (1 << b->pass_bits) < 8;
    const int lmax = slot < 16 && !few ? b->tune.lane_long : std::min(b->tune.lane_long, b->tune.lane_tail);
    const uint32_t lane_max = lmax > 0 ? (uint32_t)lmax : 0u;
    SKM_LAUNCH(b, k_chain_long, dim3(LONG_GRID), dim3(128), 0, cs, b->d_long_jobs.as<Job>(), rng, rng + 1,
               nullptr, nullptr, nullptr, nullptr, b->d_data.as<skm_stored_kmer_data>(), b->tune.chain_prio,
               lane_max);
    if (lane_max) {
        const int ls = slot % std::max(1, std::min(b->tune.lane_streams, (int)skm_build::LANE_ST));
        hipStream_t lst = b->lane_st[ls];
        SKM_HIP(hipStreamWaitEvent(lst, b->chain_ev[0], 0));
        SKM_LAUNCH(b, k_chains_stash, dim3((uint32_t)std::max(1, b->tune.lane_grid)), dim3(256), 0, lst,
                   b->d_long_jobs.as<Job>(), rng, rng + 1, b->long_jobs_cap, b->d_data.as<skm_stored_kmer_data>(),
                   lane_max);
        b->lane_used[ls] = true;
    }
    SKM_HIP(hipGetLastError());
}

void phase_stats(skm_build* b) {
    hipStream_t st = b->stream;
    const uint32_t F = b->opts.n_functions;
    SKM_HIP(hipEventRecord(b->ev_tail[0], st));
    join_tail(b);
    if (b->n_total)
        SKM_LAUNCH(b, k_flags_from_bits, dim3(1024), dim3(256), 0, st, b->d_flagbits.as<uint32_t>(),
                   (uint32_t)b->n_total, b->d_flags.as<uint8_t>());
    SKM_HIP(hipMemsetAsync(b->d_dfunc.p, 0, sizeof(uint32_t) * (F ? F : 1), st));
    SKM_HIP(hipMemsetAsync(b->d_swf.p, 0, sizeof(uint32_t) * (F ? F : 1), st));
    const size_t lds_f = F <= 16384 ? sizeof(uint32_t) * F : 0;
    if (b->pass_bits) flush_long_chains(b, 16);
    SKM_LAUNCH(b, k_kept_finalize, dim3(2048), dim3(256), lds_f, st, b->d_keys.as<uint64_t>(),
                       b->d_data.as<skm_stored_kmer_data>(), b->d_ctr.as<unsigned long long>(), F,
                       b->d_dfunc.as<uint32_t>());
    if (b->nseq)
        SKM_LAUNCH(b, k_func_hist_seqs, dim3(256), dim3(256), lds_f, st, b->d_meta.as<SeqMeta>(), b->nseq, F,
                           b->d_swf.as<uint32_t>());
    if (b->pass_bits) {
        for (int k = 0; k < skm_build::LANE_ST; ++k) {
            if (!b->lane_used[k]) continue;
            SKM_HIP(hipEventRecord(b->lane_ev[k], b->lane_st[k]));
            SKM_HIP(hipStreamWaitEvent(st, b->lane_ev[k], 0));
            b->lane_used[k] = false;
        }
        for (int k = 0; k <= skm_build::GSLOTS; ++k) {
            if (!b->chain_used[k]) continue;
            const hipStream_t cs = chain_stream(b, k);
            hipEvent_t e = k == 0 ? b->chain_ev[2] : b->gev_done[k - 1];
            SKM_HIP(hipEventRecord(e, cs));
            SKM_HIP(hipStreamWaitEvent(st, e, 0));
        }
    }
    for (int g = 0; g < skm_build::GSLOTS; ++g)
        if (b->gused[g]) SKM_HIP(hipStreamWaitEvent(st, b->gev_done[g], 0));
    SKM_HIP(hipEventRecord(b->ev_tail[1], st));
    SKM_HIP(hipEventRecord(b->ev[7], st));
    SKM_HIP(hipGetLastError());
}

void phase_final(skm_build* b) {
    hipStream_t st = b->stream;
    SKM_LAUNCH(b, k_count_flags, dim3(256), dim3(256), 0, st, b->d_flags.as<uint8_t>(), b->n_total,
                       b->d_ctr.as<unsigned long long>() + 2);
    SKM_HIP(hipGetLastError());
    unsigned long long* pin = b->pinned_ctr();
    SKM_HIP(hipMemcpyAsync(pin + 48, b->d_gstat.p, 16, hipMemcpyDeviceToHost, st));
    SKM_HIP(hipMemcpyAsync(pin + 56, b->d_ctr.p, 8, hipMemcpyDeviceToHost, st));
    SKM_HIP(hipMemcpyAsync(pin + 64, b->d_run.p, 8 * RUN_SLOTS, hipMemcpyDeviceToHost, st));
    const bool canary = b->tune.poison_jobs && b->pass_bits && b->long_jobs_cap;
    if (canary)
        SKM_HIP(hipMemcpyAsync(pin + 42, b->d_data.as<skm_stored_kmer_data>() + b->kept_cap,
                               sizeof(skm_stored_kmer_data), hipMemcpyDeviceToHost, st));
    SKM_HIP(hipEventRecord(b->ev[8], st));
    SKM_HIP(hipEventSynchronize(b->ev[8]));
    const unsigned long long* R = pin + 64;
    b->giant_jobs = pin[48];
    b->giant_max = pin[49];
    b->n_kept = pin[56];
    b->run_flags = R[RUN_FLAGS];
    if (canary) {
        const auto* c = reinterpret_cast<const skm_stored_kmer_data*>(pin + 42);
        if (c->median != 0xC0DE || c->var != 0xC0DE) b->run_flags |= RUN_F_CAP;
    }
    for (int i = 0; i < 4; ++i) b->demand[i] = R[RUN_DEM_TOT + i];
    b->demand[2] = std::max<uint64_t>(b->demand[2], R[RUN_LONG_WANT]);
    b->demand[3] = std::max<uint64_t>(b->demand[3], R[RUN_LONG_WANTJ]);
    pass_times(b, 1u << b->pass_bits);
    for (int i = 0; i < 12; ++i) b->last_ms[i] = b->pass_ms[i];
    SKM_HIP(hipEventElapsedTime(&b->last_ms[6], b->ev[7], b->ev[8]));
    SKM_HIP(hipEventElapsedTime(&b->last_ms[7], b->ev_start, b->ev[8]));
    SKM_HIP(hipEventElapsedTime(&b->last_ms[12], b->ev_tail[0], b->ev_tail[1]));
    b->last_ms[13] = b->last_ms[14] = -1.0f;
    if (b->giant_timed) {
        SKM_HIP(hipEventElapsedTime(&b->last_ms[13], b->ev_start, b->ev_giant[0]));
        SKM_HIP(hipEventElapsedTime(&b->last_ms[14], b->ev_start, b->ev_giant[1]));
    }
    b->long_samples = R[RUN_LONG_CUR];
    kt_collect(b);
    b->n_overflow = (uint32_t)R[RUN_ACC_NOVF];
    b->n_overflow_last = (uint32_t)R[RUN_LAST_NOVF];
    b->n_jobs = R[RUN_ACC_JOBS];
    b->n_jobs_last = R[RUN_LAST_JOBS];
    b->n_lens = R[RUN_ACC_LENS];
    b->ovf_elems = R[RUN_ACC_OVF_ELEMS];
    b->ovf_kept = R[RUN_ACC_OVF_KEPT];
    b->n_big = R[RUN_ACC_BIG];
    b->big_kept = R[RUN_ACC_BIG_KEPT];
    b->ovf_light_sub = R[RUN_ACC_LIGHT_SUB];
    b->ovf_light_elems = R[RUN_ACC_LIGHT_ELEMS];
    b->n_local = R[RUN_ACC_GROUPED];
    b->ran = true;
}

void grow_caps(skm_build* b) {
    auto grow = [](uint64_t& cap, uint64_t dem) {
        if (dem > cap) cap = dem + dem / 8 + 1024;
    };
    grow(b->tot_cap, b->demand[0]);
    grow(b->split_cap, b->demand[1]);
    grow(b->long_cap, b->demand[2]);
    grow(b->long_jobs_cap, b->demand[3]);
    SKM_HIP(hipDeviceSynchronize());
    alloc_caps(b);
}

void run_once(const Ranks& bs) {
    for (auto* b : bs) begin_run(b);
    const uint32_t P = 1u << bs[0]->pass_bits;
    for (uint32_t pass = 0; pass < P; ++pass) {
        for (auto* b : bs) {
            use_evset(b, pass);
            phase_extract(b, pass);
        }
        if (bs[0]->world > 1) exchange(bs, pass);
        for (auto* b : bs) {
            phase_group(b, pass);
            const uint32_t nb = std::min<uint32_t>(P >= 2 ? std::min<uint32_t>(P, (uint32_t)std::max(1, b->tune.chain_batches)) : 1u, 16u);
            const uint32_t per = std::max<uint32_t>(1u, P / nb);
            if (nb > 1 && (pass + 1) % per == 0 && pass + 1 < P) {
                flush_long_chains(b, (int)((pass + 1) / per - 1));
            }
        }
    }
    for (auto* b : bs) phase_stats(b);
    if (bs[0]->world > 1) {
        std::vector<void*> df, sw, fl;
        for (auto* b : bs) {
            df.push_back(b->d_dfunc.p);
            sw.push_back(b->d_swf.p);
            fl.push_back(b->d_flags.p);
        }
        const uint32_t F = bs[0]->opts.n_functions;
        allreduce(bs, df, F, Red::SumU32);
        allreduce(bs, sw, F, Red::SumU32);
        allreduce(bs, fl, bs[0]->n_total, Red::MaxU8);
    }
    for (auto* b : bs) phase_final(b);
}

void run_ranks(const Ranks& bs) {
    check_not_released(bs);
    prepare(bs);
    for (int attempt = 0;; ++attempt) {
        run_once(bs);
        std::vector<uint64_t> mine;
        for (auto* b : bs) mine.push_back((b->run_flags & RUN_F_RERUN) ? 1u : 0u);
        const std::vector<uint64_t> all = bs[0]->world > 1 ? allgather_u64(bs, mine) : mine;
        bool redo = false;
        for (auto v : all) redo |= v != 0;
        if (!redo) break;
        SKM_CHECK(attempt < 3, SKM_E_STATE, "build work buffers did not converge");
        for (auto* b : bs) {
            grow_caps(b);
            ++b->n_redo;
        }
    }
    for (auto* b : bs) {
        SKM_CHECK(!(b->run_flags & RUN_F_ARENA), SKM_E_OOM,
                  "kept k-mer arena exhausted (raise the device memory budget or the key-range passes)");
        SKM_CHECK(!(b->run_flags & RUN_F_CAP), SKM_E_STATE, "build work list capacity exceeded");
    }
}

Ranks ranks_of(skm_build* b) {
    if (!b->group.empty()) return b->group;
    return Ranks{b};
}

}

__attribute__((constructor)) static void skm_hw_queues() {
    const char* q = getenv("GPU_MAX_HW_QUEUES");
    if (!q || atoi(q) < 16) setenv("GPU_MAX_HW_QUEUES", "16", 1);
}

extern "C" {

int skm_build_create(skm_build** out, const int* devices, int n_devices, const skm_build_opts* opts) {
    SKM_API_BEGIN
    SKM_CHECK(out && opts, SKM_E_ARG, "null argument");
    SKM_CHECK(opts->k == 8, SKM_E_ARG, "only k = 8 is supported (kmers-build-signatures.cc:17)");
    SKM_CHECK(opts->n_functions < 0xFFFFu, SKM_E_ARG, "n_functions must be < 65535");
    SKM_CHECK(n_devices == 1, SKM_E_ARG, "one device per process (multi-GPU: one process per GPU)");
    const int ws = std::max(1, opts->world_size);
    SKM_CHECK(ws <= 64 && (ws & (ws - 1)) == 0, SKM_E_ARG, "world_size must be a power of two <= 64");
    SKM_CHECK(opts->rank >= 0 && opts->rank < ws, SKM_E_ARG, "rank out of range");
    int ndev = 0;
    SKM_HIP(hipGetDeviceCount(&ndev));
    SKM_CHECK(ndev > 0, SKM_E_HIP, "no HIP device");
    auto* b = new skm_build();
    b->opts = *opts;
    b->opts.world_size = ws;
    b->device = devices ? devices[0] : 0;
    SKM_HIP(hipSetDevice(b->device));
    SKM_HIP(hipStreamCreateWithFlags(&b->stream, hipStreamNonBlocking));
    SKM_HIP(hipStreamCreateWithFlags(&b->stream2, hipStreamNonBlocking));
    SKM_HIP(hipStreamCreateWithFlags(&b->stream3, hipStreamNonBlocking));
    SKM_HIP(hipStreamCreateWithFlags(&b->stream_tail, hipStreamNonBlocking));
    SKM_HIP(hipStreamCreateWithFlags(&b->stream_tail2, hipStreamNonBlocking));
    SKM_HIP(hipEventCreateWithFlags(&b->ev_tail2, hipEventDisableTiming));
    SKM_HIP(hipEventCreateWithFlags(&b->ev_tail_bp, hipEventDisableTiming));
    SKM_HIP(hipEventCreateWithFlags(&b->ev_tail_done, hipEventDisableTiming));
    use_evset(b, 0);
    SKM_HIP(hipEventCreate(&b->ev_start));
    SKM_HIP(hipStreamCreateWithFlags(&b->chain_st, hipStreamNonBlocking));
    for (int k = 0; k < skm_build::LANE_ST; ++k) {
        SKM_HIP(hipStreamCreateWithFlags(&b->lane_st[k], hipStreamNonBlocking));
        SKM_HIP(hipEventCreateWithFlags(&b->lane_ev[k], hipEventDisableTiming));
    }
    SKM_HIP(hipStreamCreateWithFlags(&b->stx, hipStreamNonBlocking));
    SKM_HIP(hipEventCreateWithFlags(&b->ev_staged, hipEventDisableTiming));
    SKM_HIP(hipEventCreateWithFlags(&b->ev_emit, hipEventDisableTiming));
    for (int g = 0; g < skm_build::GSLOTS; ++g) {
        SKM_HIP(hipStreamCreateWithFlags(&b->gst[g], hipStreamNonBlocking));
        SKM_HIP(hipEventCreateWithFlags(&b->gev_ready[g], hipEventDisableTiming));
        SKM_HIP(hipEventCreateWithFlags(&b->gev_done[g], hipEventDisableTiming));
    }
    for (auto& e : b->chain_ev) SKM_HIP(hipEventCreateWithFlags(&e, hipEventDisableTiming));
    SKM_HIP(hipEventCreateWithFlags(&b->ev_part, hipEventDisableTiming));
    for (auto& e : b->ev_tail) SKM_HIP(hipEventCreate(&e));
    for (auto& e : b->ev_giant) SKM_HIP(hipEventCreate(&e));
    for (int i = 0; i < 2; ++i) {
        SKM_HIP(hipHostMalloc(reinterpret_cast<void**>(&b->st_pin[i]), STAGE_BYTES, hipHostMallocDefault));
        SKM_HIP(hipEventCreateWithFlags(&b->st_ev[i], hipEventDisableTiming));
    }
    SKM_HIP(hipEventCreateWithFlags(&b->ev_split, hipEventDisableTiming));
    SKM_HIP(hipEventCreateWithFlags(&b->ev_light, hipEventDisableTiming));
    set_geometry(b);
    *out = b;
    SKM_API_END
}

int skm_build_add_batch(skm_build* b, const uint8_t* residues, const uint64_t* seq_off, const uint32_t* seq_len,
                        const uint16_t* seq_func, const uint32_t* seq_id, size_t n_seqs) {
    SKM_API_BEGIN
    SKM_CHECK(b, SKM_E_ARG, "null build");
    SKM_CHECK(n_seqs == 0 || (residues && seq_off && seq_len && seq_func), SKM_E_ARG, "null array");
    check_not_released(Ranks{b});
    SKM_HIP(hipSetDevice(b->device));
    const auto t0 = std::chrono::steady_clock::now();
    std::vector<uint32_t>& ks = b->h_keep;
    ks.clear();
// ... 316 lines not shown
               : n == "chain_batches" ? &t.chain_batches
               : n == "chain_streams" ? &t.chain_streams
               : n == "poison_jobs" ? &t.poison_jobs
               : n == "route_heavy_min" ? &t.route_heavy_min
               : n == "stage_round" ? &t.stage_round
               : n == "serial_overflow" ? &t.serial_overflow
               : n == "big_split" ? &t.big_split
               : n == "sub_target" ? &t.sub_target
               : n == "lane_long" ? &t.lane_long
               : n == "lane_grid" ? &t.lane_grid
               : n == "lane_tail" ? &t.lane_tail
               : n == "lane_streams" ? &t.lane_streams
               : n == "heavy_grid" ? &t.heavy_grid
               : n == "route_vacate" ? &t.route_vacate
               : n == "route_first" ? &t.route_first
               : n == "tail_async" ? &t.tail_async
               : n == "big_grid" ? &t.big_grid
               : n == "big_grid_large" ? &t.big_grid_large
               : n == "part_order" ? &t.part_order
               : n == "emit_group" ? &t.emit_group
               : n == "handoff_index_limit" ? &t.handoff_index_limit
               : n == "handoff_max_chunk" ? &t.handoff_max_chunk
               : n == "route_first_min" ? &t.route_first_min : nullptr;
        SKM_CHECK(f != nullptr, SKM_E_ARG, "unknown build option: " + n);
        SKM_CHECK(value >= 0 && value <= 0x7FFFFFFF, SKM_E_ARG, "option value out of range");
        if (n == "overflow_long_class" || n == "main_long_class")
            SKM_CHECK(value >= 1 && value < 32, SKM_E_ARG, "long chain classes in [1, 32)");
        if (n == "giant_class") SKM_CHECK(value < 32, SKM_E_ARG, "giant_class in [0, 32)");
        if (n == "emit_group")
            SKM_CHECK(value == 0 || value == 1 || value == 2 || value == 4 || value == 8 || value == 16, SKM_E_ARG,
                      "emit_group must be 0, 1, 2, 4, 8 or 16");
        *f = (int)value;
    }
    b->prepared = false;
    b->ran = false;
    SKM_API_END
}

int skm_build_debug_stamps(skm_build* b, int enable, uint64_t* out, int cap) {
    SKM_API_BEGIN
    SKM_CHECK(b, SKM_E_ARG, "null build");
    if (out && cap > 0 && b->stamps && b->d_stamps.p) {
        uint64_t tmp[32];
        SKM_HIP(hipMemcpy(tmp, b->d_stamps.p, sizeof(tmp), hipMemcpyDeviceToHost));
        for (int i = 0; i < cap && i < 32; ++i) out[i] = tmp[i];
    }
    b->stamps = enable != 0;
    SKM_API_END
}

int skm_build_debug_jobs(skm_build* b, uint32_t* out, int cap) {
    SKM_API_BEGIN
    SKM_CHECK(b && out, SKM_E_ARG, "null argument");
    SKM_HIP(hipDeviceSynchronize());
    const uint64_t n = std::min<uint64_t>((uint64_t)cap, b->n_jobs_last);
    std::vector<Job> j(n);
    const bool ovf = b->n_overflow_last && b->cs_ovf.sorted.p;
    const DevBuf& src = ovf ? b->cs_ovf.sorted : b->cs_main.sorted;
    const uint64_t m = std::min<uint64_t>(n, src.bytes / sizeof(Job));
    if (m) SKM_HIP(hipMemcpy(j.data(), src.p, sizeof(Job) * m, hipMemcpyDeviceToHost));
    for (uint64_t i = 0; i < (uint64_t)cap; ++i) out[i] = i < m ? j[i].n : 0u;
    SKM_API_END
}

int skm_build_debug_overflow(skm_build* b, uint32_t* out, int cap) {
    if (!b || !out) return SKM_E_ARG;
    if (hipSetDevice(b->device) != hipSuccess || hipDeviceSynchronize() != hipSuccess) return SKM_E_HIP;
    const uint32_t n = b->d_ovf.p ? (uint32_t)std::min<uint64_t>(b->n_overflow_last, b->d_ovf.bytes / sizeof(OvfEntry)) : 0u;
    std::vector<OvfEntry> e(n);
    if (n && hipMemcpy(e.data(), b->d_ovf.p, sizeof(OvfEntry) * n, hipMemcpyDeviceToHost) != hipSuccess) return SKM_E_HIP;
    for (int i = 0; i < cap; ++i) out[i] = (uint32_t)i < n ? e[i].n : 0u;
    return (int)n;
}

int skm_debug_chain_bench(uint32_t n, uint32_t njobs, int mode, float* ms) {
    SKM_API_BEGIN
    SKM_CHECK(ms && n && njobs, SKM_E_ARG, "bad argument");
    std::vector<uint32_t> lens((size_t)n * njobs);
    uint32_t x = 12345;
    for (auto& v : lens) {
        x = x * 1664525u + 1013904223u;
        v = 240 + (x >> 16) % 121;
    }
    std::vector<Job> jobs(njobs);
    for (uint32_t i = 0; i < njobs; ++i) jobs[i] = Job{(uint64_t)i * n, n, i};
    DevBuf dl, dj, dout;
    dl.ensure(4 * lens.size());
    dj.ensure(sizeof(Job) * njobs);
    dout.ensure(std::max(sizeof(skm_stored_kmer_data), sizeof(double)) * njobs);
    SKM_HIP(hipMemcpy(dl.p, lens.data(), 4 * lens.size(), hipMemcpyHostToDevice));
    SKM_HIP(hipMemcpy(dj.p, jobs.data(), sizeof(Job) * njobs, hipMemcpyHostToDevice));
    DevBuf dn;
    dn.ensure(8);
    const unsigned long long nj64 = njobs;
    SKM_HIP(hipMemcpy(dn.p, &nj64, 8, hipMemcpyHostToDevice));
    hipEvent_t e0, e1;
    SKM_HIP(hipEventCreate(&e0));
    SKM_HIP(hipEventCreate(&e1));
    const uint64_t threads = ceil_div(njobs, 64) * 128;
    for (int it = 0; it < 2; ++it) {
        SKM_HIP(hipEventRecord(e0, 0));
        if (mode == 3 || mode == 4 || mode == 5)
            hipLaunchKernelGGL(k_chain_long_half, dim3(njobs), dim3(64), 0, 0, dj.as<Job>(), dl.as<uint32_t>(),
                               mode - 3, reinterpret_cast<double*>(dout.p));
        else if (mode == 2 || (mode == 0 && n >= (1u << LONG_CLASS)))
            hipLaunchKernelGGL(k_chain_long, dim3(njobs), dim3(128), 0, 0, dj.as<Job>(), nullptr, dn.as<unsigned long long>(),
                               dl.as<uint32_t>(), dl.as<uint32_t>(), dl.as<uint32_t>(), dl.as<uint32_t>(),
                               dout.as<skm_stored_kmer_data>(), 0);
        else
            hipLaunchKernelGGL(k_chains, dim3((uint32_t)ceil_div(threads, 256)), dim3(256), 0, 0, dj.as<Job>(), nullptr,
                               dn.as<unsigned long long>(), (uint64_t)njobs, dl.as<uint32_t>(), dl.as<uint32_t>(),
                               dl.as<uint32_t>(), dl.as<uint32_t>(), dout.as<skm_stored_kmer_data>());
        SKM_HIP(hipEventRecord(e1, 0));
        SKM_HIP(hipEventSynchronize(e1));
        SKM_HIP(hipEventElapsedTime(ms, e0, e1));
    }
    (void)hipEventDestroy(e0);
    (void)hipEventDestroy(e1);
    SKM_API_END
}

int skm_debug_chain_eval(const uint32_t* samples, uint32_t n, int mode, double* median, double* var) {
    SKM_API_BEGIN
    SKM_CHECK(samples && n && median && var && (mode == 1 || mode == 2), SKM_E_ARG, "bad argument");
    DevBuf dx, dout;
    dx.ensure(4ull * n);
    dout.ensure(16);
    SKM_HIP(hipMemcpy(dx.p, samples, 4ull * n, hipMemcpyHostToDevice));
    hipLaunchKernelGGL(k_chain_eval, dim3(1), dim3(128), 0, 0, dx.as<uint32_t>(), n, mode, dout.as<double>());
    SKM_HIP(hipGetLastError());
    double r[2];
    SKM_HIP(hipMemcpy(r, dout.p, 16, hipMemcpyDeviceToHost));
    *median = r[0];
    *var = r[1];
    SKM_API_END
}

int skm_debug_div_check(uint64_t nm, uint32_t per, uint64_t* mismatches) {
    SKM_API_BEGIN
    SKM_CHECK(mismatches && nm, SKM_E_ARG, "bad argument");
    DevBuf d;
    d.ensure(8);
    SKM_HIP(hipMemset(d.p, 0, 8));
    hipLaunchKernelGGL(k_div_check, dim3((uint32_t)ceil_div(nm, 256)), dim3(256), 0, 0, nm, per,
                       d.as<unsigned long long>());
    SKM_HIP(hipGetLastError());
    SKM_HIP(hipMemcpy(mismatches, d.p, 8, hipMemcpyDeviceToHost));
    SKM_API_END
}

int skm_build_counters(skm_build* b, uint64_t* out, int cap) {
    if (!b || !out) return SKM_E_ARG;
    auto us = [](double sec) { return (uint64_t)(sec * 1e6); };
    const uint64_t v[48] = {b->n_windows, b->n_kept, b->n_overflow, b->n_jobs, b->n_lens, b->nseq, b->n_local,
                            b->ovf_elems, b->ovf_kept, b->n_big, b->big_kept, 1ull << b->pass_bits, b->valid_total,
                            b->giant_jobs, b->giant_max, b->n_redo, b->tot_cap, b->split_cap, b->long_cap,
                            b->long_jobs_cap, b->demand[0], b->demand[1], b->demand[2], b->demand[3],
                            b->long_samples, b->routed, us(b->add_s), us(b->prep_upload_s), us(b->prep_plan_s),
                            us(b->prep_rest_s), b->pass_bits ? (1ull << b->pass_bits) / b->emit_g : 0ull, us(b->add_pack_s),
                            us(b->add_wait_s), us(b->handoff.total_s), us(b->handoff.wait_s),
                            us(b->handoff.copy_s), b->handoff.chunks, (uint64_t)(1e3 * b->handoff.select_ms),
                            (uint64_t)(1e3 * b->handoff.sort_ms), (uint64_t)(1e3 * b->handoff.gather_ms),
                            (uint64_t)(1e3 * b->handoff.d2h_ms), b->handoff.max_chunk,
                            (uint64_t)b->handoff.wide_index, b->kept_cap, b->free_after_prepare,
                            0ull , b->ovf_light_sub, b->ovf_light_elems};
    int n = std::min(cap, 48);
    for (int i = 0; i < n; ++i) out[i] = v[i];
    return n;
}

int skm_build_set_kernel_timing(skm_build* b, int enable, const char* only) {
    SKM_API_BEGIN
    SKM_CHECK(b, SKM_E_ARG, "null build");
    b->kt_mode = enable ? 1 : 0;
    b->kt_only = only ? std::string(only) : std::string();
    SKM_API_END
}

int skm_build_kernel_timings(skm_build* b, char* names, size_t names_cap, float* ms, uint64_t* launches, int cap) {
    if (!b) return SKM_E_ARG;
    const int n = (int)b->kt_names.size();
    std::string all;
    for (int k = 0; k < n; ++k) {
        if (k < cap) {
            if (ms) ms[k] = (float)b->kt_ms[k];
            if (launches) launches[k] = b->kt_n[k];
        }
        all += b->kt_names[k];
        all += '\n';
    }
    if (names && names_cap) {
        const size_t c = std::min(names_cap - 1, all.size());
        std::memcpy(names, all.data(), c);
        names[c] = 0;
    }
    return n;
}

int skm_build_last_timings(skm_build* b, float* ms, int cap) {
    if (!b || !ms) return SKM_E_ARG;
    int n = std::min(cap, 15);
    for (int i = 0; i < n; ++i) ms[i] = b->last_ms[i];
    return n;
}

int skm_build_finish(skm_build* b, skm_kept* out) {
    SKM_API_BEGIN
    SKM_CHECK(b && out, SKM_E_ARG, "null argument");
    check_transport(b);
    SKM_HIP(hipSetDevice(b->device));
    const Ranks bs = ranks_of(b);
    bool need = false;
    for (auto* x : bs) need |= !x->prepared || !x->ran;
    if (need) run_ranks(bs);
    std::memset(out, 0, sizeof(*out));
    const uint32_t F = b->opts.n_functions;
    std::vector<uint64_t> mine;
    for (auto* x : bs) mine.push_back(x->n_kept);
    const std::vector<uint64_t> nk = b->world > 1 ? allgather_u64(bs, mine) : mine;
    uint64_t total = 0;
    for (auto v : nk) total += v;
    const bool gather = b->world > 1 && b->rank == 0;
    const uint64_t n = gather ? total : b->n_kept;
    DevBuf gk, gd;
    const uint64_t* src_k = b->d_keys.as<uint64_t>();
    const skm_stored_kmer_data* src_d = b->d_data.as<skm_stored_kmer_data>();
    if (b->world > 1 && bs.size() > 1) {
        if (gather) {
            gk.ensure(8 * (total + 1));
            gd.ensure(sizeof(skm_stored_kmer_data) * (total + 1));
            uint64_t o = 0;
            for (auto* x : bs) {
                if (x->n_kept) {
                    SKM_HIP(hipMemcpy(gk.as<uint64_t>() + o, x->d_keys.p, 8 * x->n_kept, hipMemcpyDeviceToDevice));
                    SKM_HIP(hipMemcpy(gd.as<skm_stored_kmer_data>() + o, x->d_data.p,
                                      sizeof(skm_stored_kmer_data) * x->n_kept, hipMemcpyDeviceToDevice));
                }
                o += x->n_kept;
            }
            src_k = gk.as<uint64_t>();
            src_d = gd.as<skm_stored_kmer_data>();
        }
    } else if (b->world > 1) {
        const int W = b->world;
        A2A xk, xd;
        std::vector<uint64_t> so(W, 0), sck(W, 0), scd(W, 0), rok(W, 0), rod(W, 0), rck(W, 0), rcd(W, 0);
        sck[0] = 8 * b->n_kept;
        scd[0] = sizeof(skm_stored_kmer_data) * b->n_kept;
        if (gather) {
            gk.ensure(8 * (total + 1));
            gd.ensure(sizeof(skm_stored_kmer_data) * (total + 1));
            uint64_t o = 0;
            for (int r = 0; r < W; ++r) {
                rok[r] = 8 * o;
                rod[r] = sizeof(skm_stored_kmer_data) * o;
                rck[r] = 8 * nk[r];
                rcd[r] = sizeof(skm_stored_kmer_data) * nk[r];
                o += nk[r];
            }
        }
        xk.send = {b->d_keys.as<uint8_t>()};
        xk.recv = {gather ? gk.as<uint8_t>() : nullptr};
        xk.soff = {so};
        xk.scnt = {sck};
        xk.roff = {rok};
        xk.rcnt = {rck};
        xd.send = {b->d_data.as<uint8_t>()};
        xd.recv = {gather ? gd.as<uint8_t>() : nullptr};
        xd.soff = {so};
        xd.scnt = {scd};
        xd.roff = {rod};
        xd.rcnt = {rcd};
        alltoallv(bs, xk);
        alltoallv(bs, xd);
        SKM_HIP(hipStreamSynchronize(b->stream));
        if (gather) {
            src_k = gk.as<uint64_t>();
            src_d = gd.as<skm_stored_kmer_data>();
        }
    }
    out->distinct_functions = (uint32_t*)std::malloc(sizeof(uint32_t) * std::max<uint32_t>(F, 1));
    out->seqs_with_func = (uint32_t*)std::malloc(sizeof(uint32_t) * std::max<uint32_t>(F, 1));
    SKM_CHECK(out->distinct_functions && out->seqs_with_func, SKM_E_OOM, "host allocation failed");
    if (F) {
        SKM_HIP(hipMemcpyAsync(out->distinct_functions, b->d_dfunc.p, sizeof(uint32_t) * F, hipMemcpyDeviceToHost, b->stream));
        SKM_HIP(hipMemcpyAsync(out->seqs_with_func, b->d_swf.p, sizeof(uint32_t) * F, hipMemcpyDeviceToHost, b->stream));
    }
    unsigned long long ctr[3];
    SKM_HIP(hipMemcpyAsync(ctr, b->d_ctr.p, sizeof(ctr), hipMemcpyDeviceToHost, b->stream));
    const bool strict = b->world > 1 ? b->g_strict : b->seqid_strict;
    std::vector<uint8_t> flags;
    if (!strict) {
        flags.resize(b->n_total);
        if (b->n_total) SKM_HIP(hipMemcpyAsync(flags.data(), b->d_flags.p, b->n_total, hipMemcpyDeviceToHost, b->stream));
    }
    SKM_HIP(hipStreamSynchronize(b->stream));
    if (!b->pool) b->pool.reset(new HostPool(HostPool::default_threads()));
    kept_handoff(src_k, src_d, n, b->stream, b->pool.get(), &out->keys, &out->data, &b->handoff,
                 (uint64_t)b->tune.handoff_index_limit, (uint64_t)b->tune.handoff_max_chunk);
    out->n = n;
    out->n_functions = F;
    out->distinct_signatures = total;
    if (strict) {
        out->n_seqs_with_signature = ctr[2];
    } else {
        const std::vector<uint32_t>& sid = b->world > 1 ? b->g_seqid : b->h_seqid;
        std::vector<uint32_t> ids;
        for (uint32_t s = 0; s < b->n_total; ++s)
            if (flags[s]) ids.push_back(sid[s]);
        std::sort(ids.begin(), ids.end());
        out->n_seqs_with_signature = (uint64_t)(std::unique(ids.begin(), ids.end()) - ids.begin());
    }
    out->n_windows = b->n_windows;
    out->n_records = b->n_local;
    SKM_API_END
}

int skm_build_finish_slice(skm_build* b, int slice_bits, uint32_t slice, skm_kept* out) {
    SKM_API_BEGIN
// ... 194 lines not shown
```

Measured before the change: 11.61 billion.

## Persistent work-stealing bucket processing and fused per-pass bucket start computation

k_bucket_process becomes a persistent kernel launched with about two blocks per CU. Blocks pull tasks from an atomic counter, and each bucket is split into eight sub-bucket parts to balance skewed buckets. A new k_pass_starts kernel computes bucket starts, cursors, slices and part order right after the pass histogram. It uses double-buffered per-pass copies, replacing the colsum/bstart/coloffs/abs_starts/stage_init chain in multi-pass mode, and join_tail is removed. Small buckets are now copied into tmp so the process kernel always reads from tmp, which adds extra memory traffic. The change also adds task and batch counters, and carries risks from atomic contention and the removed join.

Result: faster. 11.99 billion (median of 6 runs) (+3.3%).

```diff
diff --git a/signature_kmers_amd/__init__.py b/signature_kmers_amd/__init__.py
--- a/signature_kmers_amd/__init__.py
+++ b/signature_kmers_amd/__init__.py
@@ -335,8 +335,8 @@
         return self.counters()["passes"]
 
     def counters(self) -> dict:
-        v = (C.c_uint64 * 48)()
-        n = lib().skm_build_counters(self._h, v, 48)
+        v = (C.c_uint64 * 50)()
+        n = lib().skm_build_counters(self._h, v, 50)
         names = ["windows", "kept", "overflow_subbuckets", "chain_jobs", "chain_samples", "sequences", "grouped",
                  "overflow_elements", "overflow_kept", "big_groups", "big_kept", "passes", "valid", "giant_chains",
                  "giant_max", "redone", "cap_overflow_scratch", "cap_split", "cap_long_samples", "cap_long_jobs",
@@ -345,7 +345,8 @@
                  "pass_groups", "add_pack_us", "add_dma_wait_us", "finish_us", "finish_wait_us", "finish_copy_us",
                  "finish_chunks", "finish_select_dev_us", "finish_sort_dev_us", "finish_gather_dev_us",
                  "finish_d2h_dev_us", "finish_max_chunk", "finish_wide_index", "kept_cap",
-                 "free_after_prepare", "recs_rot", "overflow_light_subbuckets", "overflow_light_elements"]
+                 "free_after_prepare", "recs_rot", "overflow_light_subbuckets", "overflow_light_elements",
+                 "groupby_tasks", "groupby_batches"]
         return {names[i]: int(v[i]) for i in range(n)}
 
     def debug_jobs(self, k: int = 64) -> list:
diff --git a/signature_kmers_amd/csrc/skm_build.hip b/signature_kmers_amd/csrc/skm_build.hip
--- a/signature_kmers_amd/csrc/skm_build.hip
+++ b/signature_kmers_amd/csrc/skm_build.hip
@@ -636,6 +636,8 @@
     RUN_LONG_CUR = 1,
     RUN_LONG_N = 2,
     RUN_LONG_FLUSHED = 3,
+    RUN_ACC_BPK_TASKS = 4,
+    RUN_ACC_BPK_BATCHES = 5,
     RUN_SNAP = 28,
     RUN_DEM_TOT = 8,
     RUN_DEM_SPLIT = 9,
@@ -2708,64 +2710,90 @@
     return L;
 }
 
+constexpr uint32_t BPK_PARTS = 8;
+static_assert(BPK_PARTS >= 1 && (BPK_PARTS & (BPK_PARTS - 1)) == 0 && BPK_PARTS <= (1u << MAX_B2), "parts: a power of two");
+constexpr int CTR_BPK_TASK = 7;
+constexpr int CTR_BPK_TASKS = 13;
+constexpr int CTR_BPK_BATCHES = 15;
+
 __global__ __launch_bounds__(BPK_THREADS, BPK_WAVES_EU) void k_bucket_process(BucketArgs A) {
     static_assert(CAP % BPK_THREADS == 0, "emit assigns CAP / BPK_THREADS elements per thread");
     __shared__ SubMem s_mem;
-    __shared__ uint32_t s_sub[(1 << MAX_B2) + 1];
+    __shared__ uint32_t s_sub[(1 << MAX_B2) / BPK_PARTS + 1];
+    __shared__ uint32_t s_task;
     if (A.skip && *A.skip) return;
     SubLds L = sub_lds(s_mem);
-
-    const uint32_t bucket = blockIdx.x;
-    if (bucket >= A.nbuckets) return;
-    const uint64_t r0 = A.bstart[bucket], r1 = A.bstart[bucket + 1];
-    const uint64_t n = r1 - r0;
-    if (n == 0) return;
-    const uint64_t hprefix = (uint64_t)(A.bucket_base + bucket) << A.rem_bits;
     if (A.prio == 1) __builtin_amdgcn_s_setprio(1);
     if (A.prio == 2) __builtin_amdgcn_s_setprio(2);
     if (A.prio >= 3) __builtin_amdgcn_s_setprio(3);
-
-    const bool direct = n <= (uint64_t)CAP && A.nsrc == 1;
-    uint32_t nsub = 1;
-    if (!direct) {
-        const uint32_t* tab = A.sub_tab + (uint64_t)bucket * SUB_TAB;
-        nsub = tab[0];
-        for (uint32_t d = threadIdx.x; d <= nsub; d += blockDim.x) s_sub[d] = tab[1 + d];
+    const uint32_t ntasks = A.nbuckets * BPK_PARTS;
+    uint32_t worked = 0, batches = 0;
+    for (;;) {
+        if (threadIdx.x == 0) s_task = (uint32_t)atomicAdd(&A.ctr[CTR_BPK_TASK], 1ull);
         __syncthreads();
-        SKM_STAMP(9);
-    }
-    struct Batch {
-        uint32_t a, cnt;
-    };
-    auto next_batch = [&](uint32_t& d) -> Batch {
+        const uint32_t task = s_task;
+        __syncthreads();
+        if (task >= ntasks) break;
+        const uint32_t bucket = task / BPK_PARTS, part = task % BPK_PARTS;
+        const uint64_t r0 = A.bstart[bucket], r1 = A.bstart[bucket + 1];
+        const uint64_t n = r1 - r0;
+        if (n == 0) continue;
+        const uint64_t hprefix = (uint64_t)(A.bucket_base + bucket) << A.rem_bits;
+
+        const bool direct = n <= (uint64_t)CAP && A.nsrc == 1;
+        uint32_t nsub = 1;
         if (direct) {
-            if (d >= 1) return Batch{0, 0};
-            d = 1;
-            return Batch{0, (uint32_t)n};
-        }
-        while (d < nsub) {
-            const uint32_t a = s_sub[d];
-            if (s_sub[d + 1] - a == 0 || s_sub[d + 1] - a > (uint32_t)CAP) {
-                ++d;
-                continue;
-            }
-            uint32_t d2 = d + 1;
-            while (d2 < nsub && s_sub[d2 + 1] - a <= (uint32_t)CAP) ++d2;
-            d = d2;
-            return Batch{a, s_sub[d2] - a};
-        }
-        return Batch{0, 0};
-    };
-    const uint64_t* base_hi = direct ? A.recs_hi + r0 : A.tmp_hi + r0;
-    const uint64_t* base_lo = direct ? A.recs_lo + r0 : A.tmp_lo + r0;
-    const uint64_t sel = direct ? LENS_IN_RECS : LENS_IN_TMP;
-    uint32_t d = 0;
-    for (Batch cur = next_batch(d); cur.cnt; cur = next_batch(d)) {
-        L.lens_sel = (sel << LENS_SEL_SHIFT) | (2 * (r0 + cur.a));
-        L.lens32 = reinterpret_cast<uint32_t*>(const_cast<uint64_t*>(base_hi + cur.a));
-        process_sub(base_hi + cur.a, base_lo + cur.a, cur.cnt, A, hprefix, L);
-        __syncthreads();
-        SKM_STAMP(10);
+            if (part) continue;
+        } else {
+            const uint32_t* tab = A.sub_tab + (uint64_t)bucket * SUB_TAB;
+            const uint32_t all = tab[0];
+            const uint32_t d0 = (uint32_t)((uint64_t)part * all / BPK_PARTS), d1 = (uint32_t)((uint64_t)(part + 1) * all / BPK_PARTS);
+            if (d0 == d1) continue;
+            nsub = d1 - d0;
+            for (uint32_t d = threadIdx.x; d <= nsub; d += blockDim.x) s_sub[d] = tab[1 + d0 + d];
+            __syncthreads();
+            SKM_STAMP(9);
+        }
+        struct Batch {
+            uint32_t a, cnt;
+        };
+        auto next_batch = [&](uint32_t& d) -> Batch {
+            if (direct) {
+                if (d >= 1) return Batch{0, 0};
+                d = 1;
+                return Batch{0, (uint32_t)n};
+            }
+            while (d < nsub) {
+                const uint32_t a = s_sub[d];
+                if (s_sub[d + 1] - a == 0 || s_sub[d + 1] - a > (uint32_t)CAP) {
+                    ++d;
+                    continue;
+                }
+                uint32_t d2 = d + 1;
+                while (d2 < nsub && s_sub[d2 + 1] - a <= (uint32_t)CAP) ++d2;
+                d = d2;
+                return Batch{a, s_sub[d2] - a};
+            }
+            return Batch{0, 0};
+        };
+        const uint64_t* base_hi = A.tmp_hi + r0;
+        const uint64_t* base_lo = A.tmp_lo + r0;
+        const uint64_t sel = LENS_IN_TMP;
+        uint32_t d = 0, nb = 0;
+        for (Batch cur = next_batch(d); cur.cnt; cur = next_batch(d)) {
+            L.lens_sel = (sel << LENS_SEL_SHIFT) | (2 * (r0 + cur.a));
+            L.lens32 = reinterpret_cast<uint32_t*>(const_cast<uint64_t*>(base_hi + cur.a));
+            process_sub(base_hi + cur.a, base_lo + cur.a, cur.cnt, A, hprefix, L);
+            __syncthreads();
+            SKM_STAMP(10);
+            ++nb;
+        }
+        worked += nb ? 1u : 0u;
+        batches += nb;
+    }
+    if (threadIdx.x == 0 && worked) {
+        atomicAdd(&A.ctr[CTR_BPK_TASKS], (unsigned long long)worked);
+        atomicAdd(&A.ctr[CTR_BPK_BATCHES], (unsigned long long)batches);
     }
 }
 
@@ -3018,7 +3046,76 @@
     if (threadIdx.x == 0) order[nb] = nbig;
 }
 
+constexpr uint32_t PS_CUR0 = (1u << SC_L0_BITS) * CUR_STRIDE, PS_SLICES = 80;
+
+__global__ __launch_bounds__(1024) void k_pass_starts(const uint32_t* __restrict__ histg, uint32_t NB, int l0_shift,
+                                                      uint32_t set0, uint64_t* __restrict__ bstart,
+                                                      unsigned long long* __restrict__ cur0,
+                                                      unsigned long long* __restrict__ cur1,
+                                                      uint32_t* __restrict__ slice_base, uint32_t* __restrict__ order) {
+    __shared__ uint32_t s_wave[48];
+    __shared__ uint32_t s_n[(1 << SC_L0_BITS) + 1];
+    const uint32_t c = set0 + blockIdx.x;
+    const uint32_t* hist = histg + (uint64_t)blockIdx.x * NB;
+    bstart += (uint64_t)c * (NB + 1);
+    cur0 += (uint64_t)c * PS_CUR0;
+    cur1 += (uint64_t)c * NB * CUR_STRIDE;
+    slice_base += (uint64_t)c * PS_SLICES;
+    const uint32_t per = (NB + blockDim.x - 1) / blockDim.x;
+    const uint32_t b0 = min(NB, threadIdx.x * per), b1 = min(NB, b0 + per);
+    uint32_t loc = 0;
+    for (uint32_t b = b0; b < b1; ++b) loc += hist[b];
+    uint32_t total;
+    uint32_t run = wg_exclusive_scan(loc, s_wave, total);
+    for (uint32_t b = b0; b < b1; ++b) {
+        bstart[b] = run;
+        cur1[(uint64_t)b * CUR_STRIDE] = run;
+        run += hist[b];
+    }
+    if (threadIdx.x == 0) bstart[NB] = total;
+    __syncthreads();
+    const uint32_t n0 = 1u << SC_L0_BITS;
+    if (threadIdx.x < n0) {
+        const uint64_t a = bstart[(uint64_t)threadIdx.x << l0_shift];
+        const uint64_t e = bstart[(uint64_t)(threadIdx.x + 1) << l0_shift];
+        cur0[threadIdx.x * CUR_STRIDE] = a;
+        s_n[threadIdx.x] = (uint32_t)((e - a + SC_SLICE - 1) / SC_SLICE);
+    }
+    __syncthreads();
+    if (threadIdx.x == 0) {
+        uint32_t acc = 0;
+        for (uint32_t b = 0; b < n0; ++b) {
+            slice_base[b] = acc;
+            acc += s_n[b];
+        }
+        slice_base[n0] = acc;
+    }
+    if (!order) return;
+    order += (uint64_t)c * (NB + 1);
+    const uint64_t thr = 2 * ((uint64_t)total / max(NB, 1u));
+    loc = 0;
+    for (uint32_t b = b0; b < b1; ++b) loc += hist[b] > thr ? 1u : 0u;
+    uint32_t nbig;
+    uint32_t pos = wg_exclusive_scan(loc, s_wave, nbig);
+    uint32_t sp = b0 - pos;
+    for (uint32_t b = b0; b < b1; ++b) {
+        if (hist[b] > thr)
+            order[pos++] = b;
+        else
+            order[nbig + sp++] = b;
+    }
+    if (threadIdx.x == 0) order[NB] = nbig;
+}
+
 constexpr uint32_t PT_ROUND = 2048, PT_THREADS = BP_THREADS;
+
+__device__ __noinline__ void copy_small_bucket(const uint64_t* __restrict__ hi, const uint64_t* __restrict__ lo,
+                                               uint64_t* __restrict__ out_hi, uint64_t* __restrict__ out_lo, uint32_t n) {
+    for (uint32_t j = threadIdx.x; j < n; j += blockDim.x) {
+        out_hi[j] = hi[j];
+        out_lo[j] = lo[j];
+    }
+}
 
 __global__ __launch_bounds__(PT_THREADS, 3) void k_partition(BucketArgs A) {
     __shared__ uint32_t s_cur[(1 << MAX_B2) + 1];
@@ -3034,6 +3131,7 @@
     uint32_t* tab = A.sub_tab + (uint64_t)bucket * SUB_TAB;
     if (n == 0 || (n <= (uint64_t)CAP && A.nsrc == 1)) {
         if (threadIdx.x == 0) tab[0] = 0;
+        copy_small_bucket(A.recs_hi + r0, A.recs_lo + r0, A.tmp_hi + r0, A.tmp_lo + r0, (uint32_t)n);
         return;
     }
     const uint64_t rem_mask = (1ull << A.rem_bits) - 1;
@@ -4314,6 +4412,8 @@
     run[RUN_ACC_BIG_KEPT] += ctr[6];
     run[RUN_ACC_LIGHT_SUB] += ctr[21];
     run[RUN_ACC_LIGHT_ELEMS] += ctr[22];
+    run[RUN_ACC_BPK_TASKS] += ctr[CTR_BPK_TASKS];
+    run[RUN_ACC_BPK_BATCHES] += ctr[CTR_BPK_BATCHES];
     run[RUN_LAST_JOBS] = j;
     if (ctr[3] > jobs_cap || ctr[8 + 3] > jobs2_cap || ctr[5] > big_cap || ctr[8 + 4] > lens_cap)
         atomicOr(&run[RUN_FLAGS], RUN_F_CAP);
@@ -4526,7 +4626,7 @@
     hipEvent_t* ev_o = nullptr;
     hipEvent_t* ev_o3 = nullptr;
     float last_ms[15] = {};
-    uint64_t ovf_elems = 0, ovf_kept = 0, ovf_light_sub = 0, ovf_light_elems = 0;
+    uint64_t ovf_elems = 0, ovf_kept = 0, ovf_light_sub = 0, ovf_light_elems = 0, bpk_tasks = 0, bpk_batches = 0;
 
     uint8_t* st_pin[2] = {};
     size_t st_fill[2] = {};
@@ -4567,6 +4667,7 @@
     DevBuf d_jobs, d_lens, d_stamps, d_big_desc, d_big_out;
     uint64_t big_cap = 0, n_big = 0, big_kept = 0;
     bool stamps = false;
+    uint32_t n_cus = 0;
     uint64_t jobs_cap = 0, lens_cap = 0, n_jobs = 0, n_lens = 0;
     uint32_t n_overflow = 0, n_overflow_last = 0;
     uint32_t nwg = 0;
@@ -5027,6 +5128,11 @@
 
 void prepare_local(skm_build* b) {
     SKM_HIP(hipSetDevice(b->device));
+    if (!b->n_cus) {
+        hipDeviceProp_t prop;
+        SKM_HIP(hipGetDeviceProperties(&prop, b->device));
+        b->n_cus = (uint32_t)std::max(1, prop.multiProcessorCount);
+    }
     set_geometry(b);
     stage_flush(b);
     const uint64_t rp = b->rp_total;
@@ -5051,11 +5157,6 @@
     uint64_t nwg = std::max<uint64_t>(1, std::min<uint64_t>(EX_MAX_WG, ceil_div(rp ? rp : 1, step)));
     b->span = ceil_div(ceil_div(rp ? rp : 1, nwg), step) * step;
     b->nwg = (uint32_t)ceil_div(rp ? rp : 1, b->span);
-    const uint32_t nrb = (uint32_t)ceil_div(b->nwg, SCAN_ROWS);
-    b->d_hist.ensure(sizeof(uint32_t) * (uint64_t)b->nwg * NB);
-    b->d_offs.ensure(sizeof(uint32_t) * (uint64_t)b->nwg * NB);
-    b->d_partial.ensure(sizeof(uint32_t) * (uint64_t)nrb * NB);
-    b->d_rbbase.ensure(sizeof(uint32_t) * (uint64_t)nrb * NB);
     b->d_bstart32.ensure(sizeof(uint32_t) * (NB + 1));
     b->d_bstart.ensure(sizeof(uint64_t) * (NB + 1));
     b->d_owner_start.ensure(sizeof(uint64_t) * 80);
@@ -5152,6 +5253,19 @@
     b->d_big_desc.ensure(16 * b->big_cap);
     b->d_big_out.ensure(sizeof(BigOut) * b->big_cap);
     b->cap_local = c;
+}
+
+inline uint32_t pass_copies(const skm_build* b) { return b->pass_bits ? 2u * b->emit_g : 1u; }
+inline uint32_t pass_copy(const skm_build* b, uint32_t pass) {
+    return b->pass_bits ? ((pass / b->emit_g) & 1u) * b->emit_g + pass % b->emit_g : 0u;
+}
+void ensure_pass_copies(skm_build* b) {
+    const uint64_t NB = 1ull << (b->owner_bits + b->b1_bits), nc = pass_copies(b);
+    b->d_bstart.ensure(sizeof(uint64_t) * (NB + 1) * nc);
+    b->d_cur0.ensure(8ull * PS_CUR0 * nc);
+    b->d_cur1.ensure(8ull * NB * CUR_STRIDE * nc);
+    b->d_slices.ensure(4ull * PS_SLICES * nc);
+    b->d_part_order.ensure(4ull * (NB + 1) * nc);
 }
 
 void size_local(skm_build* b) {
@@ -5178,11 +5292,15 @@
         uint32_t nwg = (uint32_t)std::max<uint64_t>(1, std::min<uint64_t>(stage_wg, ceil_div(W, (uint64_t)SC_ROUND * 4)));
         b->pf_span = ceil_div(ceil_div(W, nwg), (uint64_t)SC_ROUND) * SC_ROUND;
         b->pf_nwg = (uint32_t)std::max<uint64_t>(1, ceil_div(W, b->pf_span));
-        b->d_hist.ensure(sizeof(uint32_t) * (uint64_t)EX_MAX_WG * NB);
-        b->d_offs.ensure(sizeof(uint32_t) * (uint64_t)EX_MAX_WG * NB);
-        b->d_partial.ensure(sizeof(uint32_t) * (uint64_t)ceil_div(EX_MAX_WG, SCAN_ROWS) * NB);
-        b->d_rbbase.ensure(sizeof(uint32_t) * (uint64_t)ceil_div(EX_MAX_WG, SCAN_ROWS) * NB);
-    }
+    } else {
+        const uint64_t NB = 1ull << (b->owner_bits + b->b1_bits);
+        const uint64_t nrb = ceil_div(b->nwg, SCAN_ROWS);
+        b->d_hist.ensure(sizeof(uint32_t) * (uint64_t)b->nwg * NB);
+        b->d_offs.ensure(sizeof(uint32_t) * (uint64_t)b->nwg * NB);
+        b->d_partial.ensure(sizeof(uint32_t) * nrb * NB);
+        b->d_rbbase.ensure(sizeof(uint32_t) * nrb * NB);
+    }
+    ensure_pass_copies(b);
 }
 
 void size_arena(skm_build* b) {
@@ -5483,6 +5601,10 @@
     SKM_HIP(hipMemsetAsync(b->d_histg.p, 0, sizeof(uint32_t) * NB * G, st));
     SKM_LAUNCH(b, k_pass_hist, dim3(256, G), dim3(PH_THREADS), 4u * NB, st, b->d_posg.as<uint64_t>(), cap,
                b->d_npos.as<unsigned long long>() + (uint64_t)g * G, NB, rem_bits, b->d_histg.as<uint32_t>());
+    SKM_LAUNCH(b, k_pass_starts, dim3(G), dim3(1024), 0, st, b->d_histg.as<uint32_t>(), NB,
+               b->owner_bits + b->b1_bits - SC_L0_BITS, (g & 1u) * G, b->d_bstart.as<uint64_t>(),
+               b->d_cur0.as<unsigned long long>(), b->d_cur1.as<unsigned long long>(), b->d_slices.as<uint32_t>(),
+               b->world == 1 && b->tune.part_order ? b->d_part_order.as<uint32_t>() : nullptr);
     SKM_HIP(hipGetLastError());
     if (st != b->stream) SKM_HIP(hipEventRecord(b->ev_emit, st));
 }
@@ -5540,23 +5662,28 @@
     }
     SKM_HIP(hipGetLastError());
     SKM_HIP(hipEventRecord(b->ev[1], st));
-    const uint32_t nrb = (uint32_t)ceil_div(hist_rows, SCAN_ROWS);
-    dim3 gsc((NB + 255) / 256, nrb);
-    SKM_LAUNCH(b, k_colsum, gsc, dim3(256), 0, st, X.hist, hist_rows, NB, b->d_partial.as<uint32_t>());
-    SKM_LAUNCH(b, k_bstart, dim3(1), dim3(1024), 0, st, b->d_partial.as<uint32_t>(), nrb, NB, b->b1_bits,
-                       b->d_rbbase.as<uint32_t>(), b->d_bstart32.as<uint32_t>(), b->d_owner_start.as<uint64_t>(), nowners);
-    SKM_LAUNCH(b, k_coloffs, gsc, dim3(256), 0, st, X.hist, b->d_rbbase.as<uint32_t>(), hist_rows,
-                       NB, b->d_offs.as<uint32_t>());
-    SKM_LAUNCH(b, k_abs_starts, dim3((NB + 1 + 255) / 256), dim3(256), 0, st, b->d_bstart32.as<uint32_t>(),
-                       b->d_owner_start.as<uint64_t>(), NB, b->b1_bits, nowners, b->d_bstart.as<uint64_t>());
-    SKM_HIP(hipGetLastError());
+    const uint32_t pc = pass_copy(b, pass);
+    uint64_t* bstart = b->d_bstart.as<uint64_t>() + (uint64_t)pc * (NB + 1);
+    unsigned long long* cur0 = b->d_cur0.as<unsigned long long>() + (uint64_t)pc * PS_CUR0;
+    unsigned long long* cur1 = b->d_cur1.as<unsigned long long>() + (uint64_t)pc * NB * CUR_STRIDE;
+    uint32_t* slices = b->d_slices.as<uint32_t>() + (uint64_t)pc * PS_SLICES;
+    if (!b->pass_bits) {
+        const uint32_t nrb = (uint32_t)ceil_div(hist_rows, SCAN_ROWS);
+        dim3 gsc((NB + 255) / 256, nrb);
+        SKM_LAUNCH(b, k_colsum, gsc, dim3(256), 0, st, X.hist, hist_rows, NB, b->d_partial.as<uint32_t>());
+        SKM_LAUNCH(b, k_bstart, dim3(1), dim3(1024), 0, st, b->d_partial.as<uint32_t>(), nrb, NB, b->b1_bits,
+                           b->d_rbbase.as<uint32_t>(), b->d_bstart32.as<uint32_t>(), b->d_owner_start.as<uint64_t>(), nowners);
+        SKM_LAUNCH(b, k_coloffs, gsc, dim3(256), 0, st, X.hist, b->d_rbbase.as<uint32_t>(), hist_rows,
+                           NB, b->d_offs.as<uint32_t>());
+        SKM_LAUNCH(b, k_abs_starts, dim3((NB + 1 + 255) / 256), dim3(256), 0, st, b->d_bstart32.as<uint32_t>(),
+                           b->d_owner_start.as<uint64_t>(), NB, b->b1_bits, nowners, bstart);
+        SKM_HIP(hipGetLastError());
+    }
     SKM_HIP(hipEventRecord(b->ev[2], st));
-    const int l0_shift = nbits - SC_L0_BITS;
-    b->d_cur0.ensure(8ull * 64 * CUR_STRIDE);
-    b->d_cur1.ensure(8ull * NB * CUR_STRIDE);
-    b->d_slices.ensure(4 * 80);
-    SKM_LAUNCH(b, k_stage_init, dim3((NB + 255) / 256), dim3(256), 0, st, b->d_bstart.as<uint64_t>(), NB, l0_shift,
-                       b->d_cur0.as<unsigned long long>(), b->d_cur1.as<unsigned long long>(), b->d_slices.as<uint32_t>());
+    if (!b->pass_bits) {
+        SKM_LAUNCH(b, k_stage_init, dim3((NB + 255) / 256), dim3(256), 0, st, bstart, NB, nbits - SC_L0_BITS, cur0, cur1,
+                   slices);
+    }
     const bool sep = tail_async_on(b);
     uint64_t* stg_hi = (sep ? b->d_stg_hi : b->d_tmp_hi).as<uint64_t>();
     uint64_t* stg_lo = (sep ? b->d_stg_lo : b->d_tmp_lo).as<uint64_t>();
@@ -5566,21 +5693,18 @@
                    b->d_posg.as<uint64_t>() + (uint64_t)(pass % b->emit_g) * std::max<uint64_t>(b->pass_max, 1),
                    b->d_npos.as<unsigned long long>() + pass,
                    b->d_seloff.as<uint64_t>() + (uint64_t)pass * (b->sel_wg + 1), b->sel_wg, b->sel_span,
-                   b->d_cur0.as<unsigned long long>(), stg_hi, stg_lo);
+                   cur0, stg_hi, stg_lo);
     else if (b->pass_bits)
         SKM_LAUNCH_AS(b, "k_extract_stage_pos", (k_extract_stage_pos<SC_ROUND, 2>), dim3(nwg), dim3(EX_THREADS), 0, st, X,
                    b->d_posg.as<uint64_t>() + (uint64_t)(pass % b->emit_g) * std::max<uint64_t>(b->pass_max, 1),
                    b->d_npos.as<unsigned long long>() + pass,
                    b->d_seloff.as<uint64_t>() + (uint64_t)pass * (b->sel_wg + 1), b->sel_wg, b->sel_span,
-                   b->d_cur0.as<unsigned long long>(), stg_hi, stg_lo);
+                   cur0, stg_hi, stg_lo);
     else
-        SKM_LAUNCH(b, k_extract_stage, dim3(nwg), dim3(EX_THREADS), 0, st, X, b->d_cur0.as<unsigned long long>(),
-                           stg_hi, stg_lo);
-    join_tail(b);
+        SKM_LAUNCH(b, k_extract_stage, dim3(nwg), dim3(EX_THREADS), 0, st, X, cur0, stg_hi, stg_lo);
     const uint32_t nsl = (uint32_t)(ceil_div(b->pass_max, SC_SLICE) + (1u << SC_L0_BITS));
     SKM_LAUNCH(b, k_split_stage, dim3(nsl), dim3(EX_THREADS), 0, st, stg_hi,
-                       stg_lo, b->d_bstart.as<uint64_t>(), nbits, b->d_slices.as<uint32_t>(),
-                       b->d_cur1.as<unsigned long long>(), b->d_recs_hi.as<uint64_t>(), b->d_recs_lo.as<uint64_t>());
+                       stg_lo, bstart, nbits, slices, cur1, b->d_recs_hi.as<uint64_t>(), b->d_recs_lo.as<uint64_t>());
     SKM_HIP(hipGetLastError());
     SKM_HIP(hipEventRecord(b->ev[3], st));
 }
@@ -5593,7 +5717,8 @@
     for (auto* b : bs) {
         b->d_cnt_send.ensure(4ull * NB);
         b->d_cnt_recv.ensure(4ull * NB);
-        SKM_LAUNCH(b, k_send_counts, dim3((NB + 255) / 256), dim3(256), 0, b->stream, b->d_bstart.as<uint64_t>(), NB, NB1,
+        SKM_LAUNCH(b, k_send_counts, dim3((NB + 255) / 256), dim3(256), 0, b->stream,
+                   b->d_bstart.as<uint64_t>() + (uint64_t)pass_copy(b, pass) * ((1ull << (b->owner_bits + b->b1_bits)) + 1), NB, NB1,
                    (uint32_t)W, b->d_xs.as<unsigned long long>() + (uint64_t)pass * W, b->d_run.as<unsigned long long>(),
                    b->d_cnt_send.as<uint32_t>());
         cx.send.push_back(b->d_cnt_send.as<uint8_t>());
@@ -5765,7 +5890,8 @@
     A.recs_lo = (multi ? b->d_rlo : b->d_recs_lo).as<uint64_t>();
     A.tmp_hi = b->d_tmp_hi.as<uint64_t>();
     A.tmp_lo = b->d_tmp_lo.as<uint64_t>();
-    A.bstart = multi ? b->d_vstart.as<uint64_t>() : b->d_bstart.as<uint64_t>();
+    const uint32_t pc = pass_copy(b, pass);
+    A.bstart = multi ? b->d_vstart.as<uint64_t>() : b->d_bstart.as<uint64_t>() + (uint64_t)pc * (NB1 + 1);
     A.seg_start = multi ? b->d_seg_start.as<uint64_t>() : nullptr;
     A.seg_len = multi ? b->d_seg_len.as<uint32_t>() : nullptr;
     A.nsrc = multi ? (uint32_t)b->world : 1u;
@@ -5797,9 +5923,8 @@
     }
     A.order = nullptr;
     if (b->tune.part_order) {
-        b->d_part_order.ensure(4ull * (NB1 + 1));
-        SKM_LAUNCH(b, k_part_order, dim3(1), dim3(1024), 0, st, A.bstart, NB1, b->d_part_order.as<uint32_t>());
-        A.order = b->d_part_order.as<uint32_t>();
+        A.order = b->d_part_order.as<uint32_t>() + (multi ? 0 : (uint64_t)pc * (NB1 + 1));
+        if (multi || !b->pass_bits) SKM_LAUNCH(b, k_part_order, dim3(1), dim3(1024), 0, st, A.bstart, NB1, b->d_part_order.as<uint32_t>());
     }
     SKM_LAUNCH(b, k_partition, dim3(NB1), dim3(BP_THREADS), 0, st, A);
     SKM_HIP(hipGetLastError());
@@ -5809,7 +5934,7 @@
     if (multi) {
         nloc_d = reinterpret_cast<const unsigned long long*>(b->d_vstart.as<uint64_t>() + NB1);
     } else {
-        nloc_d = reinterpret_cast<const unsigned long long*>(b->d_bstart.as<uint64_t>() + NB1);
+        nloc_d = reinterpret_cast<const unsigned long long*>(A.bstart + NB1);
     }
     const uint32_t split_min = (uint32_t)std::max(b->tune.split_min, CAP + 1);
     const uint32_t key_min = (uint32_t)std::max(b->tune.heavy_min, 2);
@@ -5926,7 +6051,7 @@
     BA.flags = A.flags;
     BA.out = b->d_big_out.as<BigOut>();
     SKM_HIP(hipEventRecord(b->ev[11], st));
-    SKM_LAUNCH(b, k_bucket_process, dim3(NB1), dim3(BPK_THREADS), 0, st, A);
+    SKM_LAUNCH(b, k_bucket_process, dim3(std::min<uint32_t>(NB1 * BPK_PARTS, 2u * b->n_cus)), dim3(BPK_THREADS), 0, st, A);
     SKM_HIP(hipGetLastError());
     SKM_HIP(hipEventRecord(b->ev[5], st));
     if (b->tune.serial_overflow) launch_overflow();
@@ -6218,6 +6343,8 @@
     b->big_kept = R[RUN_ACC_BIG_KEPT];
     b->ovf_light_sub = R[RUN_ACC_LIGHT_SUB];
     b->ovf_light_elems = R[RUN_ACC_LIGHT_ELEMS];
+    b->bpk_tasks = R[RUN_ACC_BPK_TASKS];
+    b->bpk_batches = R[RUN_ACC_BPK_BATCHES];
     b->n_local = R[RUN_ACC_GROUPED];
     b->ran = true;
 }
@@ -6840,7 +6967,7 @@
 int skm_build_counters(skm_build* b, uint64_t* out, int cap) {
     if (!b || !out) return SKM_E_ARG;
     auto us = [](double sec) { return (uint64_t)(sec * 1e6); };
-    const uint64_t v[48] = {b->n_windows, b->n_kept, b->n_overflow, b->n_jobs, b->n_lens, b->nseq, b->n_local,
+    const uint64_t v[50] = {b->n_windows, b->n_kept, b->n_overflow, b->n_jobs, b->n_lens, b->nseq, b->n_local,
                             b->ovf_elems, b->ovf_kept, b->n_big, b->big_kept, 1ull << b->pass_bits, b->valid_total,
                             b->giant_jobs, b->giant_max, b->n_redo, b->tot_cap, b->split_cap, b->long_cap,
                             b->long_jobs_cap, b->demand[0], b->demand[1], b->demand[2], b->demand[3],
@@ -6851,8 +6978,9 @@
                             (uint64_t)(1e3 * b->handoff.sort_ms), (uint64_t)(1e3 * b->handoff.gather_ms),
                             (uint64_t)(1e3 * b->handoff.d2h_ms), b->handoff.max_chunk,
                             (uint64_t)b->handoff.wide_index, b->kept_cap, b->free_after_prepare,
-                            0ull , b->ovf_light_sub, b->ovf_light_elems};
-    int n = std::min(cap, 48);
+                            0ull , b->ovf_light_sub, b->ovf_light_elems, b->bpk_tasks,
+                            b->bpk_batches};
+    int n = std::min(cap, 50);
     for (int i = 0; i < n; ++i) out[i] = v[i];
     return n;
 }
```
